# chenbinghui1/DSL

Measured on AMD Instinct MI355X. Metric: imgs/sec training step, FCOS R50-FPN 1333x800, higher is better.
Workload: dtype bf16; 1 GPU; FCOS R50-caffe-FPN supervised training step (BASELINE.json configs[1]), 2 x (3,800,1344) per GPU, synthetic COCO-shaped boxes, random-init weights; global_batch=2, parallelism=dp1, optimizer=SGD momentum 0.9 wd 1e-4

## Files before the change

dsl_amd/_lib.py:

```python
import ctypes as C
import os

import torch

HERE = os.path.dirname(os.path.abspath(__file__))
LIB_PATH = os.environ.get('DSL_HIP_LIB') or os.path.join(HERE, 'lib', 'libdsl_hip.so')
MAX_SEG = 5

if not os.path.exists(LIB_PATH):
    raise RuntimeError(
        f'{LIB_PATH} not found: the MI355X kernels are not built. Run `python -m dsl_amd.build` '
        '(needs hipcc); dsl_amd has no CPU or PyTorch fallback for its hot path.')
lib = C.CDLL(LIB_PATH)

I5 = C.c_int32 * MAX_SEG
F5 = C.c_float * MAX_SEG

CONV_RELU_OUT, CONV_RELU_IN, CONV_OUT_F32, CONV_MASK_FIRST, CONV_MASK_LAST, CONV_ADD_UPSAMPLE, \
    CONV_SMALL_C = 1, 2, 4, 8, 16, 32, 64
CONV_FP8 = 128
CONV_EPI_STAGED = 1 << 16
(OP_CONV, OP_WGRAD, OP_GN_FWD, OP_GN_BWD, OP_MAXPOOL, OP_SUM2X2, OP_COLSUM, OP_MEMSET, OP_PACK_IMAGE,
 OP_ASSIGN, OP_LOSS, OP_FORK, OP_JOIN, OP_WGRAD_GROUP, OP_RECORD, OP_WAIT) = range(1, 17)
OP_RLA = 17
# ... 8 lines not shown
MAX_MULTI = 16
SLOT_TAIL, SLOT_PREFIX = 13, 14
SLOT_PACKS = 15
SUMSQ_PARTS = 256
ACC_SET, ACC_ADD, ACC_FOLD = 0, 1, 2
SLOT_UPD = 8
SLOT_HEADW = 12
(RLA_AVGPOOL, RLA_AVGPOOL_BWD, RLA_BN_TANH, RLA_BN_TANH_BWD, RLA_BN_FOLD, RLA_BN_POST, RLA_REC_SUM, RLA_TAIL_FWD, RLA_TAIL_BWD) = range(2, 11)
MAX_GROUP = 8


class ConvDesc(C.Structure):
    _fields_ = [('nseg', C.c_int32), ('n', C.c_int32),
                ('gh', I5), ('gw', I5), ('sh', I5), ('sw', I5), ('dh', I5), ('dw', I5), ('ah', I5), ('aw', I5),
                ('cs', C.c_int32), ('cd', C.c_int32), ('cd_pad', C.c_int32),
                ('ldd', C.c_int32), ('lda', C.c_int32), ('ldm', C.c_int32),
                ('kh', C.c_int32), ('kw', C.c_int32), ('stride', C.c_int32), ('pad', C.c_int32),
                ('mode', C.c_int32), ('os', C.c_int32), ('flags', C.c_int32),
                ('src', C.c_void_p), ('wgt', C.c_void_p), ('dst', C.c_void_p),
                ('scale', C.c_void_p), ('bias', C.c_void_p), ('addend', C.c_void_p), ('mask', C.c_void_p),
                ('workspace', C.c_void_p), ('workspace_bytes', C.c_size_t), ('cs_real', C.c_int32), ('lds', C.c_int32),
                ('gn_ws', C.c_void_p), ('gn_x', C.c_void_p), ('gn_gamma', C.c_void_p), ('gn_beta', C.c_void_p),
                ('gn_stats', C.c_void_p)]


class WgradDesc(C.Structure):
    _fields_ = [('nseg', C.c_int32), ('n', C.c_int32),
                ('gh', I5), ('gw', I5), ('sh', I5), ('sw', I5),
                ('cs', C.c_int32), ('cy', C.c_int32), ('cd', C.c_int32),
                ('kh', C.c_int32), ('kw', C.c_int32), ('stride', C.c_int32), ('pad', C.c_int32),
                ('splits', C.c_int32),
                ('dy', C.c_void_p), ('x', C.c_void_p), ('scale', C.c_void_p), ('dw', C.c_void_p),
                ('db', C.c_void_p), ('workspace', C.c_void_p), ('workspace_bytes', C.c_size_t),
                ('ldx', C.c_int32), ('shared', C.c_int32), ('slots', C.c_int32), ('pad_', C.c_int32),
                ('pixtab', C.c_void_p), ('pixtab_bytes', C.c_size_t)]


class GnDesc(C.Structure):
    _fields_ = [('nseg', C.c_int32), ('n', C.c_int32), ('c', C.c_int32), ('groups', C.c_int32),
                ('h', I5), ('w', I5), ('eps', C.c_float),
                ('x', C.c_void_p), ('y', C.c_void_p), ('gamma', C.c_void_p), ('beta', C.c_void_p),
                ('stats', C.c_void_p), ('dy', C.c_void_p), ('dx', C.c_void_p), ('dgamma', C.c_void_p),
                ('dbeta', C.c_void_p), ('dbias', C.c_void_p), ('workspace', C.c_void_p), ('workspace_bytes', C.c_size_t),
                ('conv_stats', C.c_int32), ('pad_', C.c_int32), ('y8', C.c_void_p), ('y8_scale', C.c_void_p), ('y8_amax', C.c_void_p)]


class Fp8PrepItem(C.Structure):
    _fields_ = [('w', C.c_void_p), ('w8', C.c_void_p), ('comb', C.c_void_p), ('amax', C.c_void_p), ('scale', C.c_void_p),
                ('n_amax', C.c_int32), ('cout', C.c_int32)]


class FcosDesc(C.Structure):
    _fields_ = [('nlvl', C.c_int32), ('n', C.c_int32),
                ('h', I5), ('w', I5), ('stride', I5), ('range_lo', F5), ('range_hi', F5),
                ('radius', C.c_float), ('num_classes', C.c_int32),
                ('gt_boxes', C.c_void_p), ('gt_labels', C.c_void_p), ('gt_off', C.c_void_p),
                ('ig_boxes', C.c_void_p), ('ig_off', C.c_void_p),
                ('labels', C.c_void_p), ('bbox_targets', C.c_void_p), ('assign_idx', C.c_void_p),
                ('cls_weight', C.c_void_p), ('pos_weight', C.c_void_p), ('stats', C.c_void_p),
                ('loss_weight', C.c_float),
                ('cls_logits', C.c_void_p), ('regctr', C.c_void_p),
                ('ld_cls', C.c_int32), ('ld_rc', C.c_int32),
                ('scales', C.c_void_p), ('norm', C.c_void_p),
                ('g_cls', C.c_void_p), ('ld_gcls', C.c_int32), ('g_rc', C.c_void_p), ('ld_grc', C.c_int32),
                ('g_scales', C.c_void_p), ('losses', C.c_void_p),
                ('soft_weight', C.c_float), ('grad_scale', C.c_float), ('inv_world', C.c_float),
                ('workspace', C.c_void_p), ('workspace_bytes', C.c_size_t), ('logvec', C.c_void_p),
                ('head_flags', C.c_int32), ('ld_ctr', C.c_int32), ('ctr', C.c_void_p), ('g_ctr', C.c_void_p), ('ld_gctr', C.c_int32),
                ('box_kind', C.c_int32), ('box_eps', C.c_float), ('focal_gamma', C.c_float), ('focal_alpha', C.c_float),
                ('w_cls', C.c_float), ('w_bbox', C.c_float), ('w_ctr', C.c_float)]


HEAD_INSIDE_BOX, HEAD_RAW_TARGETS, HEAD_EXP_DECODE, HEAD_IOU_LOSS = 1, 2, 4, 8
HEAD_LOSS_EXT = 16
BOX_GIOU, BOX_IOU_LOG, BOX_IOU_LINEAR, BOX_DIOU, BOX_CIOU = range(5)
NMS_HARD, NMS_LINEAR, NMS_GAUSSIAN, NMS_NAIVE = range(4)
EVAL_COCO, EVAL_VOC, EVAL_MAX_THRS, EVAL_MAX_RANGES = 0, 1, 16, 4
MAX_AUG = 16


class DetDesc(C.Structure):
    _fields_ = [('nlvl', C.c_int32), ('n', C.c_int32),
                ('h', I5), ('w', I5), ('stride', I5),
                ('num_classes', C.c_int32), ('nms_pre', C.c_int32), ('max_per_img', C.c_int32),
                ('score_thr', C.c_float), ('iou_thr', C.c_float),
                ('cls_logits', C.c_void_p), ('ld_cls', C.c_int32),
                ('regctr', C.c_void_p), ('ld_rc', C.c_int32),
                ('scales', C.c_void_p), ('img_shapes', C.c_void_p), ('scale_factors', C.c_void_p),
                ('dets', C.c_void_p), ('det_labels', C.c_void_p), ('det_count', C.c_void_p),
                ('workspace', C.c_void_p), ('workspace_bytes', C.c_size_t),
                ('head_flags', C.c_int32), ('ld_ctr', C.c_int32), ('ctr', C.c_void_p),
                ('nms_method', C.c_int32), ('soft_sigma', C.c_float), ('soft_min_score', C.c_float)]


class PackItem(C.Structure):
    _fields_ = [('w', C.c_void_p), ('scale', C.c_void_p), ('out', C.c_void_p),
                ('cout', C.c_int32), ('cout_pad', C.c_int32), ('taps', C.c_int32), ('cin', C.c_int32),
                ('block_start', C.c_int32), ('tiles_ci', C.c_int32), ('tiles_co', C.c_int32), ('tapmap', C.c_int32)]


class BneckDesc(C.Structure):
    _fields_ = [('x', C.c_void_p), ('w1', C.c_void_p), ('w2', C.c_void_p), ('w3', C.c_void_p), ('idt', C.c_void_p),
                ('s1', C.c_void_p), ('b1', C.c_void_p), ('s2', C.c_void_p), ('b2', C.c_void_p), ('s3', C.c_void_p), ('b3', C.c_void_p),
                ('a1', C.c_void_p), ('a2', C.c_void_p), ('out', C.c_void_p),
                ('n', C.c_int32), ('hin', C.c_int32), ('win', C.c_int32), ('h', C.c_int32), ('w', C.c_int32),
                ('planes', C.c_int32), ('cin', C.c_int32), ('ldx', C.c_int32), ('stride', C.c_int32), ('ldi', C.c_int32), ('ldo', C.c_int32)]


class RlaDesc(C.Structure):
    _fields_ = [('kind', C.c_int32), ('i', C.c_int32 * 8), ('f', C.c_float * 2), ('rows', C.c_int64), ('p', C.c_void_p * 12)]


class BnPostItem(C.Structure):
    _fields_ = [('w', C.c_void_p), ('dw', C.c_void_p), ('dgamma', C.c_void_p), ('dbeta', C.c_void_p), ('gamma', C.c_void_p),
                ('mean', C.c_void_p), ('var', C.c_void_p), ('rows', C.c_int32), ('k', C.c_int32), ('row_start', C.c_int32),
                ('pad_', C.c_int32)]


class RecSumItem(C.Structure):
    _fields_ = [('rec', C.c_void_p), ('out_a', C.c_void_p), ('out_b', C.c_void_p), ('nrec', C.c_int32), ('pad_', C.c_int32)]


class ImagePrepItem(C.Structure):
    _fields_ = [('src', C.c_void_p), ('src_h', C.c_int32), ('src_w', C.c_int32), ('new_h', C.c_int32), ('new_w', C.c_int32),
                ('flip', C.c_int32), ('ps_mode', C.c_int32), ('ps_crop', C.c_int32), ('to_rgb', C.c_int32),
                ('mean', C.c_float * 3), ('inv_std', C.c_float * 3)]


class AugItem(C.Structure):
    _fields_ = [('h', C.c_int32), ('w', C.c_int32), ('kind', C.c_int32), ('order', C.c_int32), ('m', C.c_float * 6),
                ('roi', C.c_int32 * 4), ('cval', C.c_int32), ('f', C.c_float * 3), ('rect', (C.c_int32 * 4) * 3), ('seed', C.c_uint32)]


(AUG_COPY, AUG_AFFINE, AUG_BRIGHTNESS, AUG_CONTRAST, AUG_SATURATION, AUG_HUE, AUG_GRAY, AUG_BLUR_H, AUG_BLUR_V, AUG_ERASE,
 AUG_AUTOCONTRAST, AUG_EQUALIZE, AUG_SOLARIZE, AUG_POSTERIZE, AUG_SHARPNESS) = range(15)


class Op(C.Structure):
    _fields_ = [('kind', C.c_int32), ('i', C.c_int32 * 7), ('desc', C.c_void_p),
                ('p', C.c_void_p * 4), ('l', C.c_int64 * 2)]


lib.dsl_last_error.restype = C.c_char_p
lib.dsl_wgrad_workspace_bytes.restype = C.c_size_t
if hasattr(lib, 'dsl_wgrad_pixtab_bytes'):
    lib.dsl_wgrad_pixtab_bytes.restype = C.c_size_t
if hasattr(lib, 'dsl_wgrad_group_workspace_bytes'):
    lib.dsl_wgrad_group_workspace_bytes.restype = C.c_size_t
lib.dsl_conv2d_workspace_bytes.restype = C.c_size_t
if hasattr(lib, 'dsl_image_aug_scratch_bytes'):
    lib.dsl_image_aug_scratch_bytes.restype = C.c_size_t
if hasattr(lib, 'dsl_rla_tail_bwd_workspace_bytes'):
    lib.dsl_rla_tail_bwd_workspace_bytes.restype = C.c_size_t
for _n in ('dsl_wgrad_multi_table_bytes', 'dsl_wgrad_multi_workspace_bytes'):
    if hasattr(lib, _n):
        getattr(lib, _n).restype = C.c_size_t
if hasattr(lib, 'dsl_bn_tanh_bwd_workspace_bytes'):
    lib.dsl_bn_tanh_bwd_workspace_bytes.restype = C.c_size_t
if hasattr(lib, 'dsl_fcos_workspace_bytes'):
    lib.dsl_fcos_workspace_bytes.restype = C.c_size_t
if hasattr(lib, 'dsl_groupnorm_workspace_bytes'):
    lib.dsl_groupnorm_workspace_bytes.restype = C.c_size_t
if hasattr(lib, 'dsl_detect_workspace_bytes'):
    lib.dsl_detect_workspace_bytes.restype = C.c_size_t
if hasattr(lib, 'dsl_detect_aug_workspace_bytes'):
    lib.dsl_detect_aug_workspace_bytes.restype = C.c_size_t
if hasattr(lib, 'dsl_eval_match_workspace_bytes'):
    lib.dsl_eval_match_workspace_bytes.restype = C.c_size_t
_vp, _i, _l, _f = C.c_void_p, C.c_int, C.c_long, C.c_float
_SIGS = {
    'dsl_conv2d': [_vp, _vp], 'dsl_conv2d_workspace_bytes': [_vp], 'dsl_conv2d_gn_fusable': [_vp], 'dsl_conv2d_wgrad': [_vp, _vp], 'dsl_wgrad_splits': [_vp],
    'dsl_wgrad_workspace_bytes': [_vp], 'dsl_wgrad_pixtab_bytes': [_vp], 'dsl_wgrad_pixtab_fill': [_vp, _vp, C.c_size_t, _vp], 'dsl_wgrad_group_workspace_bytes': [_vp, _i], 'dsl_conv2d_wgrad_group': [_vp, _i, _vp],
    'dsl_wgrad_multi_config': [_vp], 'dsl_wgrad_multi_table_bytes': [], 'dsl_wgrad_multi_workspace_bytes': [_vp, _vp, _i],
    'dsl_wgrad_multi_build': [_vp, _vp, _i, _vp, C.c_size_t, _vp, C.c_size_t], 'dsl_conv2d_wgrad_multi': [_vp, _vp, _vp], 'dsl_wgrad_multi_info': [_vp, _vp, _vp, _vp, _vp, _vp],
    'dsl_wgrad_plan_probe': [_vp, _vp, _vp, _i, _i, _i, _vp, _vp],
    'dsl_image_prep': [_vp, _i, _vp, _i, _i, _vp],
    'dsl_pack_image': [_vp, _vp, _i, _i, _i, _vp], 'dsl_stem_pool': [_vp, _vp, _vp, _vp, _vp, _i, _i, _i, _i, _vp], 'dsl_stem_pool_half': [_vp, _vp, _vp, _vp, _vp, _i, _i, _i, _i, _i, _vp], 'dsl_maxpool3x3s2': [_vp, _vp, _i, _i, _i, _i, _vp],
    'dsl_maxpool3x3s2_ld': [_vp, _vp, _i, _i, _i, _i, _i, _vp],
    'dsl_avgpool2x2': [_vp, _i, _vp, _i, _i, _i, _i, _i, _vp],
    'dsl_avgpool2x2_bwd': [_vp, _i, _vp, _i, _i, _i, _i, _i, _vp],
    'dsl_bn_tanh_fwd': [_vp, _i, _vp, _vp, _vp, _i, _l, _i, _vp],
    'dsl_rla_tail_bwd': [_vp, _i, _vp, _i, _vp, _i, _vp, _vp, _vp, _vp, _f, _vp, _i, _vp, _vp, _vp, _i, _i, _i, _vp], 'dsl_rla_tail_bwd_workspace_bytes': [_i, _i, _i],
    'dsl_rla_tail_fwd': [_vp, _i, _vp, _i, _vp, _i, _vp, _vp, _vp, _i, _vp, _vp, _vp, _i, _i, _i, _i, _vp], 'dsl_bn_tanh_bwd_workspace_bytes': [_l, _i],
    'dsl_bn_tanh_bwd': [_vp, _i, _vp, _i, _vp, _i, _vp, _vp, _vp, _f, _vp, _i, _vp, _vp, _vp, _l, _i, _vp],
    'dsl_image_prep_u8': [_vp, _i, _vp, _i, _i, _vp], 'dsl_image_aug': [_vp, _i, _vp, _vp, _i, _i, _vp, _i, _vp], 'dsl_image_aug_scratch_bytes': [_i],
    'dsl_image_normalize': [_vp, _vp, _i, _vp, _i, _i, _vp],
    'dsl_quant_fp8': [_vp, _vp, _l, _i, _i, _f, _vp], 'dsl_absmax': [_vp, _l, _i, _i, _vp, _i, _vp],
    'dsl_quant_fp8_dyn': [_vp, _vp, _l, _i, _i, _vp, _i, _vp], 'dsl_fp8_comb': [_vp, _vp, _i, _vp, _i, _vp], 'dsl_fp8_prep': [_vp, _i, _i, _i, _f, _vp],
    'dsl_quant_fp8_delayed': [_vp, _vp, _l, _i, _i, _vp, _vp, _i, _vp], 'dsl_quant_fp8_weights': [_vp, _vp, _vp, _vp, _i, _i, _i, _f, _vp],
    'dsl_bn_fold': [_vp, _vp, _vp, _vp, _f, _vp, _vp, _i, _vp], 'dsl_bn_wgrad_post': [_vp, _i, _i, _f, _vp], 'dsl_rla_op': [_vp, _vp],
    'dsl_rec_sum_multi': [_vp, _i, _i, _vp],
    'dsl_groupnorm_relu_fwd': [_vp, _vp], 'dsl_groupnorm_relu_bwd': [_vp, _vp], 'dsl_groupnorm_workspace_bytes': [_vp],
    'dsl_sum2x2': [_vp, _vp, _i, _i, _i, _i, _i, _i, _vp], 'dsl_colsum': [_vp, _vp, _l, _i, _i, _vp],
    'dsl_fcos_points': [_vp, _vp, _vp], 'dsl_fcos_workspace_bytes': [_vp], 'dsl_fcos_assign': [_vp, _vp], 'dsl_fcos_loss': [_vp, _vp],
    'dsl_sumsq': [_vp, _l, _vp, _vp], 'dsl_sumsq_det': [_vp, _l, _vp, _vp, _vp],
    'dsl_sgd_step': [_vp, _vp, _vp, _vp, _vp, _l, _f, _f, _f, _f, _f, _vp, _f, _i, _vp],
    'dsl_grad_accumulate': [_vp, _vp, _l, _i, _vp],
    'dsl_ema_lerp': [_vp, _vp, _l, _f, _vp], 'dsl_ema_lerp_bf16': [_vp, _vp, _vp, _l, _f, _vp], 'dsl_cast_bf16': [_vp, _vp, _l, _vp],
    'dsl_pack_dgrad': [_vp, _vp, _vp, _i, _i, _i, _i, _vp], 'dsl_pack_dgrad_batched': [_vp, _i, _i, _vp],
    'dsl_detect_workspace_bytes': [_vp], 'dsl_fcos_detect': [_vp, _vp],
    'dsl_detect_aug_workspace_bytes': [_vp, _i], 'dsl_fcos_detect_collect': [_vp, _vp, _i, _i, _i, _vp, C.c_size_t, _vp],
    'dsl_fcos_detect_finish': [_vp, _i, _i, _vp, C.c_size_t, _vp],
    'dsl_pseudo_label_fuse': [_vp, _vp, _vp, _i, _i, _i, _f, _f, _f, _vp, _vp, _vp, _vp, _vp],
    'dsl_eval_match_workspace_bytes': [_i, _i],
    'dsl_eval_match': [_i, _i, _i, _i, _i, _i, _vp, _vp, _vp, _vp, _vp, _vp, _vp, _vp, _i, _vp, _i, _vp, _vp, _vp, _vp, C.c_size_t, _vp],
    'dsl_eval_accumulate': [_i, _i, _i, _i, _i, _i, _vp, _vp, _vp, _vp, _vp, _vp, _vp, _vp],
    'dsl_comm_unique_id': [_vp],
    'dsl_comm_init_rank': [_vp, _i, _vp, _i],
    'dsl_comm_size': [_vp],
    'dsl_comm_destroy': [_vp],
    'dsl_allreduce_bucket': [_vp, _vp, C.c_size_t, _vp],
    'dsl_allreduce_buckets': [_vp, _vp, _vp, _i, _vp],
    'dsl_allreduce_bucket_bf16': [_vp, _vp, C.c_size_t, _vp],
    'dsl_cast_f32': [_vp, _vp, _l, _vp], 'dsl_sumsq_partial': [_vp, _l, _vp, _vp], 'dsl_sumsq_fold': [_vp, _i, _vp, _vp],
    'dsl_pseudo_label_fuse_history': [_vp, _vp, _vp, _i, _i, _vp, _vp, _vp, _vp, _i, _i, _f, _f, _f, _vp, _vp, _vp, _vp, _i, _vp],
    'dsl_bottleneck_fwd': [_vp, _vp], 'dsl_bottleneck_fwd_supported': [_vp],
    'dsl_set_option': [C.c_char_p, _i], 'dsl_get_option': [C.c_char_p, _vp],
    'dsl_run_ops': [_vp, _i, _vp], 'dsl_stream_wait_slot': [_i, _vp], 'dsl_stream_record_slot': [_i, _vp], 'dsl_side_stream': [_i, _vp], 'dsl_streams_init': [_vp, _vp], 'dsl_comm_stream_queue': [], 'dsl_comm_proxy': [_vp, C.c_longlong, _i, _i, _vp], 'dsl_prof_enable': [_i], 'dsl_prof_reset': [], 'dsl_prof_read': [_vp, _vp, _vp], 'dsl_prof_read2': [_vp, _vp, _vp, _vp], 'dsl_probe_tr16': [_vp, _vp, _vp, _vp], 'dsl_probe_xcc': [_vp, _vp, _i, _vp], 'dsl_probe_cu_mask': [_vp, _i, _vp, _i],
}
MISSING = []
for _name, _args in _SIGS.items():
    try:
        getattr(lib, _name).argtypes = _args
    except AttributeError:
        MISSING.append(_name)


if 'dsl_set_option' not in MISSING:
    from . import tuning as _tuning
    _tuning.push_lib_options(lib)


def check(rc, what=''):
    if rc != 0:
        raise RuntimeError(f'libdsl_hip {what} failed ({rc}): {lib.dsl_last_error().decode()}')


def seg5(vals):
    a = I5()
    for i, v in enumerate(vals):
        a[i] = int(v)
    return a


def stream_ptr():
    import torch
    return C.c_void_p(torch.cuda.current_stream().cuda_stream)


def ptr(t):
    if t is None:
        return C.c_void_p(0)
    if isinstance(t, int):
        return C.c_void_p(t)
    return C.c_void_p(t.data_ptr())
```

dsl_amd/csrc/api.hip:

```cpp
#include <stdarg.h>
#include <stdlib.h>

#include <stdio.h>
#include <string.h>
#include <stdlib.h>

#include "common.hpp"

static thread_local char g_err[512] = "";

void dsl_set_error(const char* fmt, ...) {
  va_list ap;
  va_start(ap, fmt);
  vsnprintf(g_err, sizeof(g_err), fmt, ap);
  va_end(ap);
}

extern "C" const char* dsl_last_error(void) { return g_err; }
extern "C" int dsl_version(void) { return 100; }

namespace {
struct Option { const char* name; int value; };
Option g_options[] = {
    {"wgrad_slots", 128},
    {"stream_probe", 1},
    {"debug_sync", 0},
    {"skip_kinds", 0},
    {"rla_tail_form", 0},
    {"comm_queue", 1},
};
}
int dsl_option(const char* name) {
  for (const Option& o : g_options)
    if (!strcmp(o.name, name)) return o.value;
  return 0;
}
extern "C" int dsl_set_option(const char* name, int value) {
  DSL_CHECK(name != nullptr, "dsl_set_option: null name");
  for (Option& o : g_options)
    if (!strcmp(o.name, name)) { o.value = value; return 0; }
  dsl_set_error("dsl_set_option: unknown option '%s'", name);
  return -1;
}
extern "C" int dsl_get_option(const char* name, int* value) {
  DSL_CHECK(name != nullptr && value != nullptr, "dsl_get_option: null argument");
  for (const Option& o : g_options)
    if (!strcmp(o.name, name)) { *value = o.value; return 0; }
  dsl_set_error("dsl_get_option: unknown option '%s'", name);
  return -1;
}

namespace {
constexpr int kEvRing = 256, kSide = 3, kStreams = 6;
hipStream_t g_side[16][kStreams] = {};
hipEvent_t g_ev[16][kEvRing] = {};
int g_evpos[16] = {};
bool g_init[16] = {};
int g_probe_result[16] = {};
int g_comm_queue[16] = {};
hipEvent_t g_named[16][16] = {};
bool g_named_set[16][16] = {};

__global__ void spin_kernel(long long ticks) {
  const long long t0 = (long long)wall_clock64();
  while ((long long)wall_clock64() - t0 < ticks) __builtin_amdgcn_s_sleep(8);
}
bool streams_concurrent(hipStream_t a, hipStream_t b, hipEvent_t ea, hipEvent_t eb) {
  hipLaunchKernelGGL(spin_kernel, dim3(1), dim3(64), 0, a, 30000LL);
  hipEventRecord(ea, a);
  hipLaunchKernelGGL(spin_kernel, dim3(1), dim3(64), 0, b, 0LL);
  hipEventRecord(eb, b);
  hipEventSynchronize(eb);
  const bool a_running = hipEventQuery(ea) == hipErrorNotReady;
  hipEventSynchronize(ea);
  (void)hipGetLastError();
  return a_running;
}
void side_init(int dev, hipStream_t caller) {
  if (g_init[dev]) return;
  for (int i = 0; i < kEvRing; ++i) hipEventCreateWithFlags(&g_ev[dev][i], hipEventDisableTiming);
  for (int i = 0; i < 16; ++i) hipEventCreateWithFlags(&g_named[dev][i], hipEventDisableTiming);
  constexpr int kCand = 12, kNeed = 3;
  hipStream_t cand[kCand] = {};
  bool used[kCand] = {};
  for (int i = 0; i < kCand; ++i) {
    hipStreamCreateWithFlags(&cand[i], hipStreamNonBlocking);
    hipEventRecord(g_ev[dev][i], cand[i]);
  }
  hipStream_t chosen[kNeed] = {};
  int n = 0;
  if (dsl_option("stream_probe") != 0) {
    hipEvent_t ea = g_ev[dev][kEvRing - 1], eb = g_ev[dev][kEvRing - 2];
    for (int i = 0; i < kCand && n < kNeed; ++i) {
      bool ok = streams_concurrent(caller, cand[i], ea, eb);
      for (int j = 0; j < n && ok; ++j) ok = streams_concurrent(chosen[j], cand[i], ea, eb);
      if (ok) { chosen[n++] = cand[i]; used[i] = true; }
    }
    g_probe_result[dev] = n;
    if (n < kNeed)
      fprintf(stderr, "[libdsl_hip] stream probe: only %d of %d side streams found a hardware queue of their own (device %d); "
                      "dsl_streams_init reports the count\n", n, kNeed, dev);
  } else {
    g_probe_result[dev] = -1;
  }
  auto take = [&]() -> hipStream_t {
    for (int i = 0; i < kCand; ++i)
      if (!used[i]) { used[i] = true; return cand[i]; }
    return cand[0];
  };
  while (n < kNeed) chosen[n++] = take();
  g_side[dev][0] = chosen[0];
  g_side[dev][1] = chosen[1];
  g_side[dev][2] = chosen[1];
  g_side[dev][3] = chosen[2];
  hipStream_t comm = nullptr;
  g_comm_queue[dev] = 0;
  const int want = dsl_option("comm_queue");
  if (g_probe_result[dev] == kNeed && want >= 1 && want <= 4) {
    hipEvent_t ea = g_ev[dev][kEvRing - 1], eb = g_ev[dev][kEvRing - 2];
    hipStream_t owner = want == 4 ? caller : chosen[want - 1];
    for (int i = 0; i < kCand && !comm; ++i)
      if (!used[i] && !streams_concurrent(owner, cand[i], ea, eb)) { comm = cand[i]; used[i] = true; g_comm_queue[dev] = want; }
  }
  g_side[dev][4] = comm ? comm : take();
  g_side[dev][5] = take();
  for (int i = 0; i < kCand; ++i)
    if (!used[i]) hipStreamDestroy(cand[i]);
  g_init[dev] = true;
}
hipEvent_t next_event(int dev) {
  g_evpos[dev] = (g_evpos[dev] + 1) % kEvRing;
  return g_ev[dev][g_evpos[dev]];
}
}

void dsl_prof_phase(int cls, int end, long long flops_bits, long long bytes_bits, hipStream_t st);

extern "C" int dsl_run_ops(const dsl_op* ops, int n_ops, void* stream) {
  DSL_CHECK(ops || n_ops == 0, "dsl_run_ops: null op list");
  hipStream_t main_st = (hipStream_t)stream;
  int dev = 0;
  hipGetDevice(&dev);
  DSL_CHECK(dev >= 0 && dev < 16, "dsl_run_ops: device index %d out of range", dev);
  auto pick = [&](int id) -> hipStream_t { return id <= 0 ? main_st : g_side[dev][(id - 1) % kSide]; };
  for (int k = 0; k < n_ops; ++k) {
    const dsl_op& o = ops[k];
    int rc = 0;
    hipStream_t st = main_st;
    const bool dbg_pre = dsl_option("debug_sync") == 1;
    if (dbg_pre) {
      fprintf(stderr, "[dsl_run_ops] start op %d/%d kind %d stream %d desc %p p0 %p p1 %p\n", k, n_ops, o.kind, o.i[6], o.desc, o.p[0], o.p[1]);
      if (o.kind == DSL_OP_CONV && o.desc) {
        const dsl_conv_desc* d = (const dsl_conv_desc*)o.desc;
        fprintf(stderr, "    conv src %p wgt %p dst %p addend %p mask %p n %d nseg %d g %dx%d s %dx%d cs %d cd %d lds %d ldd %d lda %d k %d stride %d mode %d flags %d ws %p\n",
                d->src, d->wgt, d->dst, d->addend, d->mask, d->n, d->nseg, d->gh[0], d->gw[0], d->sh[0], d->sw[0], d->cs, d->cd, d->lds, d->ldd, d->lda, d->kh, d->stride, d->mode, d->flags, d->workspace);
      }
      fflush(stderr);
    }
    if (o.kind == DSL_OP_PROF) {
      dsl_prof_phase(o.i[0], o.i[1], o.l[0], o.l[1], pick(o.i[6]));
      continue;
    }
    static const unsigned skip_kinds = (unsigned)dsl_option("skip_kinds");
    if (skip_kinds && o.kind < 30 && (skip_kinds >> o.kind & 1u) && o.kind != DSL_OP_FORK && o.kind != DSL_OP_JOIN &&
        o.kind != DSL_OP_RECORD && o.kind != DSL_OP_WAIT && (!(skip_kinds >> 30 & 1u) || o.i[6] == 1))
      continue;
    if (o.kind == DSL_OP_RECORD || o.kind == DSL_OP_WAIT) {
      side_init(dev, main_st);
      DSL_CHECK(o.i[1] >= 0 && o.i[1] < 16, "dsl_run_ops: event slot %d out of range", o.i[1]);
      if (o.kind == DSL_OP_RECORD) {
        hipEventRecord(g_named[dev][o.i[1]], pick(o.i[0]));
        g_named_set[dev][o.i[1]] = true;
      } else if (g_named_set[dev][o.i[1]]) {
        hipStreamWaitEvent(pick(o.i[0]), g_named[dev][o.i[1]], 0);
      }
      continue;
    }
// ... 281 lines not shown
```

dsl_amd/csrc/wgrad.hip:

```cpp
#include <stdlib.h>
#include <algorithm>

#include <mutex>
#include <type_traits>
#include <vector>

#include "common.hpp"

namespace {
typedef __attribute__((address_space(1))) const void* gptr_t;
typedef __attribute__((address_space(3))) void* lptr_t;
__device__ __attribute__((aligned(16))) unsigned int g_zero_line[4] = {0u, 0u, 0u, 0u};

template <int N>
__device__ __forceinline__ void wait_vmcnt() {
  asm volatile("s_waitcnt vmcnt(%0)" ::"n"(N) : "memory");
}

struct WgTile {
  int bco, bci, wco, wci, ks, nst;
  bool pipe;
};
constexpr WgTile kWgTiles[] = {
    {256, 256, 2, 4, 64, 2, false}, {256, 128, 4, 2, 64, 3, false}, {128, 256, 2, 4, 64, 3, false}, {128, 128, 2, 2, 64, 2, false},
    {256, 256, 2, 4, 32, 4, true},  {256, 128, 4, 2, 32, 5, true},  {128, 256, 2, 4, 32, 5, true},
};
constexpr int kWgDescRing = 16;
constexpr bool wgrad_cfg_ok(int cfg, bool pipe) { return cfg >= 1 && cfg <= (pipe ? 3 : 4); }
constexpr int wgrad_row(int cfg, bool pipe) { return (pipe ? 4 : 0) + cfg - 1; }
constexpr const WgTile& wgrad_tile(int cfg, bool pipe) { return kWgTiles[wgrad_row(cfg, pipe)]; }
constexpr size_t wgrad_lds_bytes(int bco, int bci, int ks, int nst, bool pipe) {
  return (size_t)nst * ks * 2 * (bco + bci) + (pipe ? (size_t)kWgDescRing * ks * 8 : 0);
}
constexpr size_t wgrad_lds_bytes(const WgTile& t) { return wgrad_lds_bytes(t.bco, t.bci, t.ks, t.nst, t.pipe); }

struct WgK {
  int nseg, n;
  int gh[DSL_MAX_SEG], gw[DSL_MAX_SEG], sh[DSL_MAX_SEG], sw[DSL_MAX_SEG];
  int pxstart[DSL_MAX_SEG + 1];
  long long xoff[DSL_MAX_SEG];
  FastDiv dhw[DSL_MAX_SEG], dwd[DSL_MAX_SEG];
  int cs, cy, kh, kw, stride, pad;
  int ktiles, tiles_per_split, ctiles_per_tap;
  int dbg;
  int gx, gy, splits;
  int chunk;
  int group;
  int ldx;
  int cyp;
  const uint16_t* dyv[DSL_MAX_GROUP];
  const uint16_t* xv[DSL_MAX_GROUP];
  long long krow;
  const uint16_t* dy;
  const uint16_t* x;
  float* ws;
  int direct, cd;
  int totpx;
  float* dwv[DSL_MAX_GROUP];
  const float* scalev[DSL_MAX_GROUP];
  int dbmask;
  float* dbws;
  float* dbv[DSL_MAX_GROUP];
  const void* pixtab;
  unsigned pixtab_bytes;
  unsigned ybytes;
};

__device__ __forceinline__ u32x2 lds_tr_read_b64(unsigned addr) {
  u32x2 v;
  asm volatile("ds_read_b64_tr_b16 %0, %1" : "=v"(v) : "v"(addr) : "memory");
  return v;
}
template <int OFF>
__device__ __forceinline__ u32x2 lds_tr_read_b64_o(unsigned addr) {
  static_assert(OFF >= 0 && OFF < 65536, "DS offset field");
  u32x2 v;
  asm volatile("ds_read_b64_tr_b16 %0, %1 offset:%2" : "=v"(v) : "v"(addr), "n"(OFF) : "memory");
  return v;
}
template <int ROWB, int KK>
__device__ __forceinline__ u32x2 lds_tr_read_kh(unsigned base, int kk, int hi) {
  static_assert(KK <= 4, "k-steps per stage");
  switch (kk * 2 + hi) {
    case 0: return lds_tr_read_b64_o<0>(base);
    case 1: return lds_tr_read_b64_o<4 * ROWB>(base);
    case 2: return lds_tr_read_b64_o<16 * ROWB>(base);
    case 3: return lds_tr_read_b64_o<20 * ROWB>(base);
    case 4: return lds_tr_read_b64_o<32 * ROWB>(base);
    case 5: return lds_tr_read_b64_o<36 * ROWB>(base);
    case 6: return lds_tr_read_b64_o<48 * ROWB>(base);
    default: return lds_tr_read_b64_o<52 * ROWB>(base);
  }
}
struct Frag {
  u32x2 lo, hi;
};
__device__ __forceinline__ unsigned lds_read_b32_asm(unsigned addr) {
  unsigned v;
  asm volatile("ds_read_b32 %0, %1" : "=v"(v) : "v"(addr) : "memory");
  return v;
}
__device__ __forceinline__ void wait_lds4(unsigned& a, unsigned& b, unsigned& c, unsigned& d) {
  asm volatile("s_waitcnt lgkmcnt(0)" : "+v"(a), "+v"(b), "+v"(c), "+v"(d) : : "memory");
}
template <int CT, int IT>
__device__ __forceinline__ void wait_frags(Frag (&fa)[CT], Frag (&fb)[IT]) {
  static_assert(IT == 2 && (CT == 2 || CT == 4), "fragment shapes used by the wgrad tiles");
  if constexpr (CT == 4) {
    asm volatile("s_waitcnt lgkmcnt(0)"
                 : "+v"(fa[0].lo), "+v"(fa[0].hi), "+v"(fa[1].lo), "+v"(fa[1].hi), "+v"(fa[2].lo), "+v"(fa[2].hi),
                   "+v"(fa[3].lo), "+v"(fa[3].hi), "+v"(fb[0].lo), "+v"(fb[0].hi), "+v"(fb[1].lo), "+v"(fb[1].hi)
                 :
                 : "memory");
  } else {
    asm volatile("s_waitcnt lgkmcnt(0)"
                 : "+v"(fa[0].lo), "+v"(fa[0].hi), "+v"(fa[1].lo), "+v"(fa[1].hi), "+v"(fb[0].lo), "+v"(fb[0].hi),
                   "+v"(fb[1].lo), "+v"(fb[1].hi)
                 :
                 : "memory");
  }
  __builtin_amdgcn_sched_barrier(0);
}

struct SegSel {
  int px0;
  uint32_t m1lo, m1hi, d1, m2lo, m2hi, d2;
  int sh, sw;
  long long xoff;
};
__device__ __forceinline__ SegSel seg_select(const WgK& p, int gp) {
  SegSel r;
  r.px0 = p.pxstart[0];
  r.m1lo = (uint32_t)p.dhw[0].m; r.m1hi = (uint32_t)(p.dhw[0].m >> 32); r.d1 = p.dhw[0].d;
  r.m2lo = (uint32_t)p.dwd[0].m; r.m2hi = (uint32_t)(p.dwd[0].m >> 32); r.d2 = p.dwd[0].d;
  r.sh = p.sh[0]; r.sw = p.sw[0]; r.xoff = p.xoff[0];
#pragma unroll
  for (int s = 1; s < DSL_MAX_SEG; ++s) {
    const bool in = s < p.nseg && gp >= p.pxstart[s];
    r.px0 = in ? p.pxstart[s] : r.px0;
    r.m1lo = in ? (uint32_t)p.dhw[s].m : r.m1lo; r.m1hi = in ? (uint32_t)(p.dhw[s].m >> 32) : r.m1hi;
    r.d1 = in ? p.dhw[s].d : r.d1;
    r.m2lo = in ? (uint32_t)p.dwd[s].m : r.m2lo; r.m2hi = in ? (uint32_t)(p.dwd[s].m >> 32) : r.m2hi;
    r.d2 = in ? p.dwd[s].d : r.d2;
    r.sh = in ? p.sh[s] : r.sh; r.sw = in ? p.sw[s] : r.sw;
    r.xoff = in ? p.xoff[s] : r.xoff;
  }
  return r;
}

template <int BCO, int BCI, int WCO, int WCI, int KS, int NST>
__device__ __forceinline__ void wgrad_glds_body(const WgK& p, const int bid, unsigned char* smem) {
  constexpr int NW = WCO * WCI;
  constexpr int YB = BCO * 2, XB = BCI * 2;
  constexpr int TILE_Y = KS * YB, TILE_X = KS * XB, STAGE = TILE_Y + TILE_X;
  constexpr int NY = TILE_Y / 1024, NX = TILE_X / 1024;
  constexpr int LY = NY / NW, LX = NX / NW;
  constexpr int LPT = LY + LX;
  constexpr int CT = BCO / WCO / 32, IT = BCI / WCI / 32;
  constexpr int KK = KS / 16;
  static_assert(NY % NW == 0 && NX % NW == 0 && LY >= 1 && LX >= 1, "tile / wave mismatch");
  static_assert(YB >= 256 && XB >= 256, "64-byte-chunk swizzle needs >= 4 chunks per row");
  static_assert(KK == 2 || KK == 4, "stage depth");
  static_assert((NST - 2) * LPT <= 63 && NST >= 2 && NST <= 4, "vmcnt range");
  static_assert(wgrad_lds_bytes(BCO, BCI, KS, NST, false) == (size_t)NST * STAGE, "the host sizes the launch's LDS with wgrad_lds_bytes");

  const int tid = threadIdx.x, lane = tid & 63;
  const int wave = __builtin_amdgcn_readfirstlane(tid >> 6);
  const int wave_co = wave / WCI, wave_ci = wave % WCI;
  const int tiles_per_member = p.gx * p.gy;
  const int tiles_per_split_wg = tiles_per_member * p.group;
  const int xcd = bid & 7, jj = bid >> 3;
  const int witem = xcd * p.chunk + jj;
  if (jj >= p.chunk || witem >= tiles_per_split_wg * p.splits) return;
  const int sp = witem / tiles_per_split_wg;
  const int rem_sp = witem - sp * tiles_per_split_wg;
  const int member = rem_sp / tiles_per_member;
  const int rem_wg = rem_sp - member * tiles_per_member;
  const uint16_t* dy_p = p.dyv[0];
  const uint16_t* x_p = p.xv[0];
  float* db_p = p.dbv[0];
#pragma unroll
  for (int g = 1; g < DSL_MAX_GROUP; ++g) {
    dy_p = member == g ? p.dyv[g] : dy_p;
// ... 157 lines not shown
      for (int i = 0; i < LX; ++i) {
        const gptr_t g = gx[i] >= 0 ? (gptr_t)(x_p + gx[i] + xch[i]) : zero;
        __builtin_amdgcn_global_load_lds(g, (lptr_t)(stage + TILE_Y + (wave + NW * i) * 1024), 16, 0, 0);
      }
    }
    if (kl >= kt0) slot_i = (slot_i + 1 == NST) ? 0 : slot_i + 1;
    if (kc >= kt0) {
#ifdef DSL_ABLATE_BUILD
      if (!(p.dbg & 2))
#endif
      compute(slot_c);
      if (do_db) {
        const unsigned st = lds_base + slot_c * STAGE;
#pragma unroll
        for (int r4 = 0; r4 < DB_ROWS; r4 += 4) {
          unsigned v[4];
#pragma unroll
          for (int j = 0; j < 4; ++j) {
            const int row = db_rg * DB_ROWS + r4 + j;
            v[j] = lds_read_b32_asm(st + row * YB + ((((db_cp * 4) >> 6) ^ (row & 3)) << 6) + ((db_cp * 4) & 63));
          }
          wait_lds4(v[0], v[1], v[2], v[3]);
#pragma unroll
          for (int j = 0; j < 4; ++j) {
            db_lo += __uint_as_float(v[j] << 16);
            db_hi += __uint_as_float(v[j] & 0xffff0000u);
          }
        }
      }
      slot_c = (slot_c + 1 == NST) ? 0 : slot_c + 1;
    }
  }
#ifdef DSL_ABLATE_BUILD
  if (p.dbg & 4) return;
#endif

  if (do_db) {
    __syncthreads();
    float* red = reinterpret_cast<float*>(smem);
    red[(db_rg * DB_PAIRS + db_cp) * 2] = db_lo;
    red[(db_rg * DB_PAIRS + db_cp) * 2 + 1] = db_hi;
    __syncthreads();
    if (tid < BCO) {
      float sacc = 0.f;
#pragma unroll
      for (int r = 0; r < DB_RG; ++r) sacc += red[(r * DB_PAIRS + (tid >> 1)) * 2 + (tid & 1)];
      const int co = co0 + tid;
      if (p.direct) {
        if (co < p.cd) db_p[co] = sacc;
      } else {
        p.dbws[((long long)sp * p.group + member) * p.cyp + co] = sacc;
      }
    }
  }
  const int frow = lane & 31, fhalf = lane >> 5;
  if (p.direct) {
    float* dw_p = p.dwv[0];
    const float* sc_p = p.scalev[0];
#pragma unroll
    for (int g = 1; g < DSL_MAX_GROUP; ++g) {
      dw_p = member == g ? p.dwv[g] : dw_p;
      sc_p = member == g ? p.scalev[g] : sc_p;
    }
#pragma unroll
    for (int ct = 0; ct < CT; ++ct)
#pragma unroll
      for (int it = 0; it < IT; ++it) {
        const long long col = (long long)tap * p.cs + ci0 + wave_ci * (32 * IT) + it * 32 + frow;
#pragma unroll
        for (int j = 0; j < 16; ++j) {
          const int co = co0 + wave_co * (32 * CT) + ct * 32 + (j & 3) + 8 * (j >> 2) + 4 * fhalf;
          if (co < p.cd) dw_p[(long long)co * p.krow + col] = sc_p ? acc[ct][it][j] * sc_p[co] : acc[ct][it][j];
        }
      }
    return;
  }
#pragma unroll
  for (int ct = 0; ct < CT; ++ct)
#pragma unroll
    for (int it = 0; it < IT; ++it) {
      const long long col = (long long)tap * p.cs + ci0 + wave_ci * (32 * IT) + it * 32 + frow;
#pragma unroll
      for (int j = 0; j < 16; ++j) {
        const int co = co0 + wave_co * (32 * CT) + ct * 32 + (j & 3) + 8 * (j >> 2) + 4 * fhalf;
        p.ws[(((long long)sp * p.group + member) * p.cyp + co) * p.krow + col] = acc[ct][it][j];
      }
    }
}

template <int BCO, int BCI, int WCO, int WCI, int KS, int NST>
__global__ __launch_bounds__(64 * WCO * WCI) void wgrad_glds_kernel(const WgK p) {
  extern __shared__ __attribute__((aligned(16))) unsigned char smem[];
  wgrad_glds_body<BCO, BCI, WCO, WCI, KS, NST>(p, (int)blockIdx.x, smem);
}

struct PixDesc {
  int32_t base;
  uint32_t info;
};

__device__ __forceinline__ u32x2 lds_read_b64_asm(unsigned addr) {
  u32x2 v;
  asm volatile("ds_read_b64 %0, %1" : "=v"(v) : "v"(addr) : "memory");
  return v;
}
__device__ __forceinline__ void pin2(u32x2& a) { asm volatile("" : "+v"(a)); }
__device__ __forceinline__ void pin1(unsigned& a) { asm volatile("" : "+v"(a)); }

template <int BCO, int BCI, int WCO, int WCI, int KS, int NST>
__device__ __forceinline__ void wgrad_pipe_body(const WgK& p, const int bid, unsigned char* smem) {
  constexpr int NW = WCO * WCI;
  constexpr int YB = BCO * 2, XB = BCI * 2;
  constexpr int TILE_Y = KS * YB, TILE_X = KS * XB, STAGE = TILE_Y + TILE_X;
  constexpr int NY = TILE_Y / 1024, NX = TILE_X / 1024;
  constexpr int LY = NY / NW, LX = NX / NW;
  constexpr int NDSC = KS * 8 / 256;
  constexpr int P = NDSC + LY + LX;
  constexpr int CT = BCO / WCO / 32, IT = BCI / WCI / 32, NM = CT * IT;
  constexpr int KK = KS / 16;
  constexpr int DR = kWgDescRing;
  constexpr int DESC_BASE = NST * STAGE;
  constexpr int DLEAD = 2 * NST - 2;
  static_assert(NY % NW == 0 && NX % NW == 0 && LY >= 1 && LX >= 1, "tile / wave mismatch");
  static_assert(YB >= 256 && XB >= 256, "64-byte-chunk swizzle needs >= 4 chunks per row");
  static_assert(KK == 2 || KK == 4, "stage depth");
  static_assert(NST >= 3 && DLEAD < DR && NDSC >= 1, "ring depths");
  static_assert((NST - 1) * P + DLEAD * NDSC <= 63, "vmcnt range");
  static_assert(wgrad_lds_bytes(BCO, BCI, KS, NST, true) == (size_t)DESC_BASE + DR * KS * 8, "the host sizes the launch's LDS with wgrad_lds_bytes");

  const int tid = threadIdx.x, lane = tid & 63;
  const int wave = __builtin_amdgcn_readfirstlane(tid >> 6);
  const int wave_co = wave / WCI, wave_ci = wave % WCI;
  const int tiles_per_member = p.gx * p.gy;
  const int tiles_per_split_wg = tiles_per_member * p.group;
  const int xcd = bid & 7, jj = bid >> 3;
  const int witem = xcd * p.chunk + jj;
  if (jj >= p.chunk || witem >= tiles_per_split_wg * p.splits) return;
  const int sp = witem / tiles_per_split_wg;
  const int rem_sp = witem - sp * tiles_per_split_wg;
  const int member = rem_sp / tiles_per_member;
  const int rem_wg = rem_sp - member * tiles_per_member;
  const uint16_t* dy_p = p.dyv[0];
  const uint16_t* x_p = p.xv[0];
  float* db_p = p.dbv[0];
#pragma unroll
  for (int g = 1; g < DSL_MAX_GROUP; ++g) {
    dy_p = member == g ? p.dyv[g] : dy_p;
    x_p = member == g ? p.xv[g] : x_p;
    db_p = member == g ? p.dbv[g] : db_p;
  }
  const int co0 = (rem_wg % p.gx) * BCO;
  const int colt = rem_wg / p.gx;
  const bool do_db = colt == 0 && ((p.dbmask >> member) & 1);
  constexpr int DB_PAIRS = BCO / 2, DB_RG = 64 * NW / DB_PAIRS, DB_ROWS = KS / DB_RG;
  static_assert(DB_ROWS >= 1 && DB_ROWS <= 8 && DB_RG * DB_PAIRS == 64 * NW, "bias-gradient thread mapping");
  const int db_cp = tid % DB_PAIRS, db_rg = tid / DB_PAIRS;
  float db_lo = 0.f, db_hi = 0.f;
  const int ctiles = p.cs / BCI;
  const int tap = colt / ctiles;
  const int ci0 = (colt - tap * ctiles) * BCI;
  const int tr = tap / p.kw, ts = tap - tr * p.kw;
  const int kt0 = sp * p.tiles_per_split;
  const int kt1 = min(kt0 + p.tiles_per_split, p.ktiles);
  if (kt0 >= kt1) return;

  const __amdgpu_buffer_rsrc_t rs_y = __builtin_amdgcn_make_buffer_rsrc((void*)dy_p, 0, (int)p.ybytes, 0x00020000);
  const __amdgpu_buffer_rsrc_t rs_x = __builtin_amdgcn_make_buffer_rsrc((void*)x_p, 0, 0x7fffffff, 0x00020000);
  const __amdgpu_buffer_rsrc_t rs_t = __builtin_amdgcn_make_buffer_rsrc((void*)p.pixtab, 0, (int)p.pixtab_bytes, 0x00020000);

  unsigned yv[LY];
  unsigned xcol[LX], xdaddr[LX];
#pragma unroll
  for (int i = 0; i < LY; ++i) {
    const int off = (wave + NW * i) * 1024 + lane * 16;
    const int row = off / YB, inrow = off % YB;
    const int ch = (((inrow >> 6) ^ (row & 3)) << 5) + ((inrow & 63) >> 1);
    yv[i] = co0 + ch < p.cy ? (unsigned)(((kt0 * KS + row) * p.cy + co0 + ch) * 2) : 0x80000000u;
  }
#pragma unroll
  for (int i = 0; i < LX; ++i) {
    const int off = (wave + NW * i) * 1024 + lane * 16;
    const int row = off / XB, inrow = off % XB;
    const int ch = (((inrow >> 6) ^ (row & 3)) << 5) + ((inrow & 63) >> 1);
    xcol[i] = (unsigned)(ci0 + ch) * 2u;
    xdaddr[i] = (unsigned)(DESC_BASE + row * 8);
  }
  const unsigned y_step = (unsigned)(KS * p.cy * 2);
  const unsigned ldx2 = (unsigned)(p.ldx * 2);
  const unsigned sel = (1u << tr) | (0x100u << ts);

  f32x16 acc[CT][IT];
#pragma unroll
  for (int a = 0; a < CT; ++a)
#pragma unroll
    for (int b = 0; b < IT; ++b)
#pragma unroll
      for (int j = 0; j < 16; ++j) acc[a][b][j] = 0.f;

  const int g16 = lane >> 4, l16 = lane & 15;
  const int iblk = (g16 & 1) * 16, kblk = (g16 >> 1) * 8;
  const int krow_l = kblk + (l16 >> 2);
  const int ccol_l = iblk + 4 * (l16 & 3);
  const unsigned lds_base = (unsigned)(size_t)smem;
  unsigned a_off[CT], b_off[IT];
#pragma unroll
  for (int ct = 0; ct < CT; ++ct) {
    const int col = wave_co * (32 * CT) + ct * 32 + ccol_l;
    a_off[ct] = krow_l * YB + ((((col * 2) >> 6) ^ (krow_l & 3)) << 6) + ((col * 2) & 63);
  }
#pragma unroll
  for (int it = 0; it < IT; ++it) {
    const int col = wave_ci * (32 * IT) + it * 32 + ccol_l;
    b_off[it] = TILE_Y + krow_l * XB + ((((col * 2) >> 6) ^ (krow_l & 3)) << 6) + ((col * 2) & 63);
  }
  Frag fa[2][CT], fb[2][IT];
  constexpr int NR = 2 * (CT + IT);
  unsigned ra[CT], rb[IT];
  auto set_read_stage = [&](unsigned stage_addr) {
#pragma unroll
    for (int ct = 0; ct < CT; ++ct) ra[ct] = stage_addr + a_off[ct];
#pragma unroll
    for (int it = 0; it < IT; ++it) rb[it] = stage_addr + b_off[it];
  };
  auto rd = [&](int kk, int f, int j) {
#ifdef DSL_ABLATE_BUILD
    if (p.dbg & 8) return;
#endif
    if (j < 2 * CT) {
      const int ct = j >> 1;
      if (j & 1) fa[f][ct].hi = lds_tr_read_kh<YB, KK>(ra[ct], kk, 1); else fa[f][ct].lo = lds_tr_read_kh<YB, KK>(ra[ct], kk, 0);
    } else {
      const int it = (j - 2 * CT) >> 1;
      if (j & 1) fb[f][it].hi = lds_tr_read_kh<XB, KK>(rb[it], kk, 1); else fb[f][it].lo = lds_tr_read_kh<XB, KK>(rb[it], kk, 0);
    }
  };
  auto issue = [&](int kk, int f) {
#pragma unroll
    for (int j = 0; j < NR; ++j) rd(kk, f, j);
  };
  auto wait_lds = [&](int f) {
    asm volatile("s_waitcnt lgkmcnt(0)" ::: "memory");
#pragma unroll
    for (int ct = 0; ct < CT; ++ct) { pin2(fa[f][ct].lo); pin2(fa[f][ct].hi); }
#pragma unroll
    for (int it = 0; it < IT; ++it) { pin2(fb[f][it].lo); pin2(fb[f][it].hi); }
  };

  int t_data = kt0, t_desc = kt0, ld_slot = 0;
  unsigned xv[LX];
  u32x2 dreg[LX];
  auto piece = [&](int k) {
#ifdef DSL_ABLATE_BUILD
    if ((p.dbg & 1) && t_data >= kt0 + NST) return;
#endif
    if (k < NDSC) {
      const unsigned v = (unsigned)(t_desc * (KS * 8) + k * 256 + lane * 4);
      __builtin_amdgcn_raw_ptr_buffer_load_lds(rs_t, (lptr_t)(smem + DESC_BASE + (t_desc & (DR - 1)) * (KS * 8) + k * 256), 4, v, 0, 0, 0);
    } else if (k < NDSC + LY) {
      const int i = k - NDSC;
      const unsigned v = t_data < kt1 ? yv[i] : 0x80000000u;
      __builtin_amdgcn_raw_ptr_buffer_load_lds(rs_y, (lptr_t)(smem + ld_slot * STAGE + (wave + NW * i) * 1024), 16, v, 0, 0, 0);
    } else {
      const int i = k - NDSC - LY;
      const unsigned v = t_data < kt1 ? xv[i] : 0x80000000u;
      __builtin_amdgcn_raw_ptr_buffer_load_lds(rs_x, (lptr_t)(smem + ld_slot * STAGE + TILE_Y + (wave + NW * i) * 1024), 16, v, 0, 0, 0);
    }
  };
  auto desc_read = [&]() {
#pragma unroll
    for (int i = 0; i < LX; ++i) dreg[i] = lds_read_b64_asm(lds_base + xdaddr[i] + (unsigned)((t_data & (DR - 1)) * (KS * 8)));
  };
  auto desc_use = [&]() {
#pragma unroll
    for (int i = 0; i < LX; ++i) {
      pin2(dreg[i]);
      const unsigned info = dreg[i][1];
      const unsigned px = (unsigned)((int)dreg[i][0] + tr * (int)(info >> 16) + ts);
      xv[i] = (info & sel) == sel ? px * ldx2 + xcol[i] : 0x80000000u;
    }
  };
  auto advance = [&]() {
    ++t_data;
    ++t_desc;
    ld_slot = (ld_slot + 1 == NST) ? 0 : ld_slot + 1;
#pragma unroll
    for (int i = 0; i < LY; ++i) yv[i] += y_step;
  };
  auto block = [&](int f, int lo, int hi, int rd_kk) {
    bf16x8 a[CT], b[IT];
#pragma unroll
    for (int ct = 0; ct < CT; ++ct) {
      union { struct { u32x2 l, h; } s; bf16x8 v; } u;
      u.s.l = fa[f][ct].lo;
      u.s.h = fa[f][ct].hi;
      a[ct] = u.v;
    }
#pragma unroll
    for (int it = 0; it < IT; ++it) {
      union { struct { u32x2 l, h; } s; bf16x8 v; } u;
      u.s.l = fb[f][it].lo;
      u.s.h = fb[f][it].hi;
      b[it] = u.v;
    }
    __builtin_amdgcn_sched_barrier(0);
    int k = lo;
#pragma unroll
    for (int m = 0; m < NM; ++m) {
#ifdef DSL_ABLATE_BUILD
      if (!(p.dbg & 2))
#endif
      acc[m / IT][m % IT] = __builtin_amdgcn_mfma_f32_32x32x16_bf16(a[m / IT], b[m % IT], acc[m / IT][m % IT], 0, 0, 0);
      __builtin_amdgcn_sched_barrier(0);
#pragma unroll
      for (int j = 0; j < NR; ++j)
        if (j >= m * NR / NM && j < (m + 1) * NR / NM) rd(rd_kk, f ^ 1, j);
      if ((m & 1) == 1 && k < hi) {
        piece(k);
        ++k;
      }
      __builtin_amdgcn_sched_barrier(0);
    }
#pragma unroll
    for (int j = 0; j < P; ++j)
      if (k + j < hi) piece(k + j);
    __builtin_amdgcn_sched_barrier(0);
  };
  constexpr int PA = (KK - 1) * P / KK;

#pragma unroll
  for (int j = 0; j < NST - 1; ++j) {
#pragma unroll
    for (int k = 0; k < NDSC; ++k) piece(k);
    ++t_desc;
  }
  wait_vmcnt<0>();
  __builtin_amdgcn_s_barrier();
#pragma unroll
  for (int j = 0; j < NST - 1; ++j) {
    desc_read();
    asm volatile("s_waitcnt lgkmcnt(0)" ::: "memory");
    desc_use();
#pragma unroll
    for (int k = 0; k < P; ++k) piece(k);
    advance();
  }
  wait_vmcnt<(NST - 2) * P>();
  __builtin_amdgcn_s_barrier();
  desc_read();
  set_read_stage(lds_base);
  issue(0, 0);

  unsigned dbr[8];
  int slot_c = 0;
  for (int s = kt0; s < kt1; ++s) {
    const unsigned st = lds_base + slot_c * STAGE;
    const int nslot = (slot_c + 1 == NST) ? 0 : slot_c + 1;
#pragma unroll
    for (int kk = 0; kk < KK; ++kk) {
      const int f = kk & 1;
      wait_lds(f);
      if (kk == 0) desc_use();
      if (kk == 1 && do_db) {
#pragma unroll
        for (int j = 0; j < DB_ROWS; ++j) {
          pin1(dbr[j]);
          db_lo += __uint_as_float(dbr[j] << 16);
          db_hi += __uint_as_float(dbr[j] & 0xffff0000u);
        }
      }
      if (kk == 0 && do_db) {
#pragma unroll
        for (int j = 0; j < DB_ROWS; ++j) {
          const int row = db_rg * DB_ROWS + j;
          dbr[j] = lds_read_b32_asm(st + row * YB + ((((db_cp * 4) >> 6) ^ (row & 3)) << 6) + ((db_cp * 4) & 63));
        }
      }
      if (kk == KK - 1) {
        wait_vmcnt<(NST - 3) * P + PA>();
#ifdef DSL_ABLATE_BUILD
        if (!(p.dbg & 16))
#endif
        __builtin_amdgcn_s_barrier();
      }
      __builtin_amdgcn_sched_barrier(0);
      if (kk < KK - 1) {
        block(f, kk * P / KK, (kk + 1) * P / KK, kk + 1);
      } else {
        set_read_stage(lds_base + nslot * STAGE);
        block(f, kk * P / KK, P, 0);
      }
      if (kk == KK - 1) {
        advance();
        desc_read();
      }
    }
    slot_c = nslot;
  }
  wait_vmcnt<0>();
  asm volatile("s_waitcnt lgkmcnt(0)" ::: "memory");
#ifdef DSL_ABLATE_BUILD
  if (p.dbg & 4) return;
#endif

  if (do_db) {
    __syncthreads();
    float* red = reinterpret_cast<float*>(smem);
    red[(db_rg * DB_PAIRS + db_cp) * 2] = db_lo;
    red[(db_rg * DB_PAIRS + db_cp) * 2 + 1] = db_hi;
    __syncthreads();
    if (tid < BCO) {
      float sacc = 0.f;
#pragma unroll
      for (int r = 0; r < DB_RG; ++r) sacc += red[(r * DB_PAIRS + (tid >> 1)) * 2 + (tid & 1)];
      const int co = co0 + tid;
      if (p.direct) {
        if (co < p.cd) db_p[co] = sacc;
      } else {
        p.dbws[((long long)sp * p.group + member) * p.cyp + co] = sacc;
      }
    }
  }
  const int frow = lane & 31, fhalf = lane >> 5;
  if (p.direct) {
    float* dw_p = p.dwv[0];
    const float* sc_p = p.scalev[0];
#pragma unroll
    for (int g = 1; g < DSL_MAX_GROUP; ++g) {
      dw_p = member == g ? p.dwv[g] : dw_p;
      sc_p = member == g ? p.scalev[g] : sc_p;
    }
#pragma unroll
    for (int ct = 0; ct < CT; ++ct)
#pragma unroll
      for (int it = 0; it < IT; ++it) {
        const long long col = (long long)tap * p.cs + ci0 + wave_ci * (32 * IT) + it * 32 + frow;
#pragma unroll
        for (int j = 0; j < 16; ++j) {
          const int co = co0 + wave_co * (32 * CT) + ct * 32 + (j & 3) + 8 * (j >> 2) + 4 * fhalf;
          if (co < p.cd) dw_p[(long long)co * p.krow + col] = sc_p ? acc[ct][it][j] * sc_p[co] : acc[ct][it][j];
        }
      }
    return;
  }
#pragma unroll
  for (int ct = 0; ct < CT; ++ct)
#pragma unroll
    for (int it = 0; it < IT; ++it) {
      const long long col = (long long)tap * p.cs + ci0 + wave_ci * (32 * IT) + it * 32 + frow;
#pragma unroll
      for (int j = 0; j < 16; ++j) {
        const int co = co0 + wave_co * (32 * CT) + ct * 32 + (j & 3) + 8 * (j >> 2) + 4 * fhalf;
        p.ws[(((long long)sp * p.group + member) * p.cyp + co) * p.krow + col] = acc[ct][it][j];
      }
    }
}

template <int BCO, int BCI, int WCO, int WCI, int KS, int NST>
__global__ __launch_bounds__(64 * WCO * WCI) void wgrad_pipe_kernel(const WgK p) {
  extern __shared__ __attribute__((aligned(16))) unsigned char smem[];
  const int total = p.chunk * 8;
  for (int vb = (int)blockIdx.x; vb < total; vb += (int)gridDim.x) {
    wgrad_pipe_body<BCO, BCI, WCO, WCI, KS, NST>(p, vb, smem);
    __syncthreads();
  }
}

constexpr int kMaxMulti = DSL_MAX_MULTI;
struct WgMultiHdr {
  int nsub;
  int wg_end[kMaxMulti];
};
#define WG_MULTI_SUB(h, vb)                                    \
  int sub = 0, start = 0;                                      \
  _Pragma("unroll") for (int s = 1; s < kMaxMulti; ++s) {      \
    const bool in = s < (h).nsub && (vb) >= (h).wg_end[s - 1]; \
    sub = in ? s : sub;                                        \
    start = in ? (h).wg_end[s - 1] : start;                    \
  }

template <int BCO, int BCI, int WCO, int WCI, int KS, int NST>
__global__ __launch_bounds__(64 * WCO * WCI) void wgrad_glds_multi_kernel(const WgMultiHdr h, const WgK* __restrict__ tab) {
  extern __shared__ __attribute__((aligned(16))) unsigned char smem[];
  WG_MULTI_SUB(h, (int)blockIdx.x)
  const WgK p = tab[sub];
  wgrad_glds_body<BCO, BCI, WCO, WCI, KS, NST>(p, (int)blockIdx.x - start, smem);
}

template <int BCO, int BCI, int WCO, int WCI, int KS, int NST>
__global__ __launch_bounds__(64 * WCO * WCI) void wgrad_pipe_multi_kernel(const WgMultiHdr h, const WgK* __restrict__ tab, int total) {
  extern __shared__ __attribute__((aligned(16))) unsigned char smem[];
  for (int vb = (int)blockIdx.x; vb < total; vb += (int)gridDim.x) {
    WG_MULTI_SUB(h, vb)
    const WgK p = tab[sub];
    wgrad_pipe_body<BCO, BCI, WCO, WCI, KS, NST>(p, vb - start, smem);
    __syncthreads();
  }
}

template <int BCO, int BCI, int WCO, int WCI, int KS, int NST>
__global__ __launch_bounds__(64 * WCO * WCI) void wgrad_pipe_multi_sched_kernel(const WgMultiHdr h, const WgK* __restrict__ tab,
                                                                               const short* __restrict__ sched, int rounds) {
  extern __shared__ __attribute__((aligned(16))) unsigned char smem[];
  for (int r = 0; r < rounds; ++r) {
    const int vb = __builtin_amdgcn_readfirstlane((int)sched[r * (int)gridDim.x + (int)blockIdx.x]);
    if (vb < 0) break;
    WG_MULTI_SUB(h, vb)
    const WgK p = tab[sub];
    wgrad_pipe_body<BCO, BCI, WCO, WCI, KS, NST>(p, vb - start, smem);
    __syncthreads();
  }
}

#undef WG_MULTI_SUB

struct RedEnt {
  const float* ws;
  float* dw;
  const float* scale;
  float* db;
  const float* dbws;
  long long dbstride;
  long long krow, sstride;
  int splits, cd, blk_start, nblk;
};
__global__ void wgrad_reduce_multi_kernel(const RedEnt* __restrict__ tab, int n) {
  int e = 0;
  for (int i = 1; i < n; ++i) e = (int)blockIdx.x >= tab[i].blk_start ? i : e;
  const RedEnt r = tab[e];
  const int lb = (int)blockIdx.x - r.blk_start;
  if (lb == 0 && r.db)
    for (int c = threadIdx.x; c < r.cd; c += blockDim.x) {
      float sacc = 0.f;
      for (int sp = 0; sp < r.splits; ++sp) sacc += r.dbws[sp * r.dbstride + c];
      r.db[c] = sacc;
    }
  const long long total4 = (long long)r.cd * r.krow / 4;
  for (long long i = (long long)lb * blockDim.x + threadIdx.x; i < total4; i += (long long)r.nblk * blockDim.x) {
    const long long el = i * 4;
    const int co = (int)(el / r.krow);
    f32x4 s = {0.f, 0.f, 0.f, 0.f};
    const float* base = r.ws + el;
    int sp = 0;
    for (; sp + 4 <= r.splits; sp += 4) {
      const f32x4 a = *reinterpret_cast<const f32x4*>(base + sp * r.sstride);
      const f32x4 b = *reinterpret_cast<const f32x4*>(base + (sp + 1) * r.sstride);
      const f32x4 c = *reinterpret_cast<const f32x4*>(base + (sp + 2) * r.sstride);
      const f32x4 d = *reinterpret_cast<const f32x4*>(base + (sp + 3) * r.sstride);
      s += (a + b) + (c + d);
    }
    for (; sp < r.splits; ++sp) s += *reinterpret_cast<const f32x4*>(base + sp * r.sstride);
    if (r.scale) s *= r.scale[co];
    *reinterpret_cast<f32x4*>(r.dw + el) = s;
  }
}

struct RedK {
  float* dw[DSL_MAX_GROUP];
  const float* scale[DSL_MAX_GROUP];
  float* db[DSL_MAX_GROUP];
  const float* dbws;
};

__global__ void wgrad_reduce_kernel(const float* __restrict__ ws, const RedK r, int splits, int group, int cy, int cd,
                                    long long krow) {
  const int member = blockIdx.y;
  float* __restrict__ dw = r.dw[0];
  const float* __restrict__ scale = r.scale[0];
#pragma unroll
  for (int g = 1; g < DSL_MAX_GROUP; ++g) {
    dw = member == g ? r.dw[g] : dw;
    scale = member == g ? r.scale[g] : scale;
  }
  if (blockIdx.x == 0) {
    float* db = r.db[0];
#pragma unroll
    for (int g = 1; g < DSL_MAX_GROUP; ++g) db = member == g ? r.db[g] : db;
    if (db)
      for (int c = threadIdx.x; c < cd; c += blockDim.x) {
        float sacc = 0.f;
        if (r.dbws)
          for (int sp = 0; sp < splits; ++sp) sacc += r.dbws[((long long)sp * group + member) * cy + c];
        db[c] = sacc;
      }
  }
  const long long total4 = (long long)cd * krow / 4;
  const long long sstride = (long long)group * cy * krow;
  for (long long i = (long long)blockIdx.x * blockDim.x + threadIdx.x; i < total4;
       i += (long long)gridDim.x * blockDim.x) {
    const long long e = i * 4;
    const int co = (int)(e / krow);
    const long long k = e - (long long)co * krow;
    f32x4 s = {0.f, 0.f, 0.f, 0.f};
    const float* base = ws + ((long long)member * cy + co) * krow + k;
    int sp = 0;
    for (; sp + 4 <= splits; sp += 4) {
      const f32x4 a = *reinterpret_cast<const f32x4*>(base + sp * sstride);
      const f32x4 b = *reinterpret_cast<const f32x4*>(base + (sp + 1) * sstride);
      const f32x4 c = *reinterpret_cast<const f32x4*>(base + (sp + 2) * sstride);
      const f32x4 d = *reinterpret_cast<const f32x4*>(base + (sp + 3) * sstride);
      s += (a + b) + (c + d);
    }
    for (; sp < splits; ++sp) s += *reinterpret_cast<const f32x4*>(base + sp * sstride);
    if (scale) s *= scale[co];
    *reinterpret_cast<f32x4*>(dw + e) = s;
  }
}

}

namespace {
struct PixGeo {
  int nseg, n, stride, pad, kh, kw;
  int gh[DSL_MAX_SEG], gw[DSL_MAX_SEG], sh[DSL_MAX_SEG], sw[DSL_MAX_SEG];
  int pxstart[DSL_MAX_SEG + 1];
  long long xoff[DSL_MAX_SEG];
};
__global__ void pixtab_fill_kernel(PixDesc* __restrict__ out, PixGeo g) {
  const int i = blockIdx.x * blockDim.x + threadIdx.x;
  if (i >= g.pxstart[g.nseg]) return;
  int s = 0;
#pragma unroll
  for (int t = 1; t < DSL_MAX_SEG; ++t)
    if (t < g.nseg && i >= g.pxstart[t]) s = t;
  const int gh = g.gh[s], gw = g.gw[s], sh = g.sh[s], sw = g.sw[s];
  int r = i - g.pxstart[s];
  const int img = r / (gh * gw);
  r -= img * gh * gw;
  const int y = r / gw, x = r - y * gw;
  const int y0 = y * g.stride - g.pad, x0 = x * g.stride - g.pad;
  unsigned ym = 0, xm = 0;
  for (int a = 0; a < g.kh; ++a) if ((unsigned)(y0 + a) < (unsigned)sh) ym |= 1u << a;
  for (int c = 0; c < g.kw; ++c) if ((unsigned)(x0 + c) < (unsigned)sw) xm |= 1u << c;
  PixDesc e;
  e.base = (int32_t)(g.xoff[s] + ((long long)img * sh + y0) * sw + x0);
  e.info = ((unsigned)sw << 16) | (xm << 8) | ym;
  out[i] = e;
}

int wgrad_slots() {
  const int v = dsl_option("wgrad_slots");
  return v > 0 ? v : 128;
}
long long wgrad_px(const dsl_wgrad_desc* d) {
  long long px = 0;
  for (int s = 0; s < d->nseg; ++s) px += (long long)d->n * d->gh[s] * d->gw[s];
  return px;
}
bool wgrad_v3_ok(const dsl_wgrad_desc* d, int cfg) {
  if (!wgrad_cfg_ok(cfg, true) || d->kh > 8 || d->kw > 8) return false;
  long long xo = 0;
  for (int s = 0; s < d->nseg; ++s) {
    xo += (long long)d->n * d->sh[s] * d->sw[s];
    if (d->sw[s] >= 65536) return false;
  }
  const long long px = wgrad_px(d), ldx = d->ldx > 0 ? d->ldx : d->cs;
  return px * d->cy * 2 < 0x7fff0000LL && xo * ldx * 2 < 0x7fff0000LL && px < (1 << 20);
}
int wgrad_v3_fill(const dsl_wgrad_desc* d, WgK& k, long long px) {
  const size_t need = (size_t)px * sizeof(PixDesc);
  DSL_CHECK(d->pixtab != nullptr && d->pixtab_bytes >= need,
            "dsl_conv2d_wgrad: this geometry runs the pipelined kernel and needs dsl_wgrad_desc.pixtab (%zu bytes given, %zu needed: "
            "dsl_wgrad_pixtab_bytes / dsl_wgrad_pixtab_fill)", d->pixtab ? d->pixtab_bytes : (size_t)0, need);
  k.pixtab = d->pixtab;
  k.pixtab_bytes = (unsigned)need;
  k.ybytes = (unsigned)(px * d->cy * 2);
  return 0;
}

template <class F>
bool wgrad_dispatch(int cfg, bool pipe, F&& f) {
  if (!wgrad_cfg_ok(cfg, pipe)) return false;
  switch (wgrad_row(cfg, pipe)) {
    case 0: f(std::integral_constant<int, 0>{}); break;
    case 1: f(std::integral_constant<int, 1>{}); break;
    case 2: f(std::integral_constant<int, 2>{}); break;
    case 3: f(std::integral_constant<int, 3>{}); break;
    case 4: f(std::integral_constant<int, 4>{}); break;
    case 5: f(std::integral_constant<int, 5>{}); break;
    default: f(std::integral_constant<int, 6>{}); break;
  }
  return true;
}
static_assert(sizeof(kWgTiles) / sizeof(kWgTiles[0]) == 7, "wgrad_dispatch lists every row");
#define WG_TILE_ARGS(T) T.bco, T.bci, T.wco, T.wci, T.ks, T.nst
template <auto KERNEL, class... Args>
void wgrad_run(const WgTile& T, dim3 grid, hipStream_t st, const Args&... args) {
  const size_t lds = wgrad_lds_bytes(T);
  static bool attr_set = false;
  if (!attr_set) {
    hipFuncSetAttribute((const void*)KERNEL, hipFuncAttributeMaxDynamicSharedMemorySize, (int)lds);
    attr_set = true;
  }
  hipLaunchKernelGGL(KERNEL, grid, dim3(64 * T.wco * T.wci), lds, st, args...);
}
}

static int wgrad_pick(const dsl_wgrad_desc* d) {
  const int force = d->splits < 0 ? -d->splits : 0;
  if (force) return force - 1;
  if (d->cy % 128) return d->cs % 256 == 0 ? 3 : 4;
  if (d->cy % 256 == 0 && d->cs % 256 == 0) return 1;
  if (d->cy % 256 == 0) return 2;
  if (d->cs % 256 == 0) return 3;
  return 4;
}
static int wgrad_geometry(const dsl_wgrad_desc* d, int* ktiles, int* tiles, int* bco) {
  const int cfg = wgrad_pick(d);
  *ktiles = *tiles = *bco = 0;
  if (!wgrad_cfg_ok(cfg, false)) return cfg;
  const WgTile& t = wgrad_tile(cfg, false);
  *ktiles = (int)((wgrad_px(d) + t.ks - 1) / t.ks);
  *bco = t.bco;
  *tiles = ((d->cy + t.bco - 1) / t.bco) * (d->kh * d->kw * d->cs / t.bci);
  return cfg;
}

static int wgrad_splits_for(const dsl_wgrad_desc* d, int count) {
  int ktiles, tiles, bco;
  const int cfg = wgrad_geometry(d, &ktiles, &tiles, &bco);
  if (tiles == 0) return 0;
  tiles *= count;
  const int max_by_k = ktiles / 4 > 0 ? ktiles / 4 : 1;
  const int per_cu = cfg == 4 ? 2 : 1;
  const int slots = d->slots > 0 ? d->slots : wgrad_slots();
  int splits = slots * per_cu / tiles;
  if (splits > max_by_k) splits = max_by_k;
  if (splits < 1) splits = 1;
  if (splits > 256) splits = 256;
  {
    const int ks = wgrad_tile(cfg, wgrad_v3_ok(d, cfg)).ks;
    const int stages = (int)((wgrad_px(d) + ks - 1) / ks);
    const int tps = (stages + splits - 1) / splits;
    splits = (stages + tps - 1) / tps;
  }
  return splits;
}

extern "C" int dsl_wgrad_splits(const dsl_wgrad_desc* d) { return wgrad_splits_for(d, 1); }

extern "C" size_t dsl_wgrad_pixtab_bytes(const dsl_wgrad_desc* d) {
  if (d == nullptr || d->nseg < 1 || d->nseg > DSL_MAX_SEG) return 0;
  if (!wgrad_v3_ok(d, wgrad_pick(d))) return 0;
  return (size_t)wgrad_px(d) * sizeof(PixDesc);
}
extern "C" int dsl_wgrad_pixtab_fill(const dsl_wgrad_desc* d, void* table, size_t bytes, void* stream) {
  DSL_CHECK(d != nullptr && d->nseg >= 1 && d->nseg <= DSL_MAX_SEG, "dsl_wgrad_pixtab_fill: bad descriptor");
  const size_t need = dsl_wgrad_pixtab_bytes(d);
  if (need == 0) return 0;
  DSL_CHECK(table != nullptr && bytes >= need, "dsl_wgrad_pixtab_fill: table too small (%zu < %zu)", bytes, need);
  PixGeo g;
  memset(&g, 0, sizeof(g));
  g.nseg = d->nseg; g.n = d->n; g.stride = d->stride; g.pad = d->pad; g.kh = d->kh; g.kw = d->kw;
  int px = 0;
  long long xo = 0;
  for (int s = 0; s < d->nseg; ++s) {
    g.gh[s] = d->gh[s]; g.gw[s] = d->gw[s]; g.sh[s] = d->sh[s]; g.sw[s] = d->sw[s];
    g.pxstart[s] = px;
    g.xoff[s] = xo;
    px += d->n * d->gh[s] * d->gw[s];
    xo += (long long)d->n * d->sh[s] * d->sw[s];
  }
  for (int s = d->nseg; s <= DSL_MAX_SEG; ++s) g.pxstart[s] = px;
  hipLaunchKernelGGL(pixtab_fill_kernel, dim3((px + 255) / 256), dim3(256), 0, (hipStream_t)stream, (PixDesc*)table, g);
  DSL_CHECK(hipGetLastError() == hipSuccess, "dsl_wgrad_pixtab_fill: launch failed");
  return 0;
}

static size_t wgrad_cy_pad(const dsl_wgrad_desc* d) {
  int ktiles, tiles, bco;
  wgrad_geometry(d, &ktiles, &tiles, &bco);
  return bco ? (size_t)(d->cy + bco - 1) / bco * bco : 0;
}

extern "C" size_t dsl_wgrad_workspace_bytes(const dsl_wgrad_desc* d) {
  const int splits = d->splits > 0 ? d->splits : dsl_wgrad_splits(d);
  return (size_t)splits * wgrad_cy_pad(d) * ((size_t)d->kh * d->kw * d->cs + 1) * sizeof(float);
}

extern "C" size_t dsl_wgrad_group_workspace_bytes(const dsl_wgrad_desc* descs, int count) {
  if (!descs || count < 1) return 0;
  if (count == 1) return dsl_wgrad_workspace_bytes(descs);
  return (size_t)wgrad_splits_for(descs, count) * count * wgrad_cy_pad(descs) * ((size_t)descs->kh * descs->kw * descs->cs + 1) * sizeof(float);
}

static bool wgrad_same_geometry(const dsl_wgrad_desc* a, const dsl_wgrad_desc* b) {
  if (a->ldx != b->ldx || a->shared != b->shared) return false;
  if (a->nseg != b->nseg || a->n != b->n || a->cs != b->cs || a->cy != b->cy || a->cd != b->cd || a->kh != b->kh ||
      a->kw != b->kw || a->stride != b->stride || a->pad != b->pad)
    return false;
  for (int s = 0; s < a->nseg; ++s)
    if (a->gh[s] != b->gh[s] || a->gw[s] != b->gw[s] || a->sh[s] != b->sh[s] || a->sw[s] != b->sw[s]) return false;
  return true;
}

static int wgrad_fill_k(const dsl_wgrad_desc* descs, int count, int splits, int cfg, bool v3, WgK& k, long long* px_out, long long* xo_out) {
  const dsl_wgrad_desc* d = descs;
  memset(&k, 0, sizeof(k));
  k.nseg = d->nseg; k.n = d->n;
  int px = 0;
  long long xo = 0;
  for (int s = 0; s < d->nseg; ++s) {
    k.gh[s] = d->gh[s]; k.gw[s] = d->gw[s]; k.sh[s] = d->sh[s]; k.sw[s] = d->sw[s];
    k.pxstart[s] = px;
    k.xoff[s] = xo;
    k.dhw[s] = make_fastdiv((uint32_t)(d->gh[s] * d->gw[s]));
    k.dwd[s] = make_fastdiv((uint32_t)d->gw[s]);
    px += d->n * d->gh[s] * d->gw[s];
    xo += (long long)d->n * d->sh[s] * d->sw[s];
  }
  DSL_CHECK(px < (1 << 20), "dsl_conv2d_wgrad: %d pixels exceed the 2^20 fast-division range", px);
  const int ldx = d->ldx > 0 ? d->ldx : d->cs;
  DSL_CHECK(ldx >= d->cs && ldx % 8 == 0, "dsl_conv2d_wgrad: ldx=%d must be >= cs=%d and a multiple of 8", ldx, d->cs);
  DSL_CHECK(xo * ldx < (1LL << 31), "dsl_conv2d_wgrad: X has more than 2^31 elements");
  k.pxstart[d->nseg] = px;
  k.totpx = px;
  k.cs = d->cs; k.cy = d->cy; k.kh = d->kh; k.kw = d->kw; k.stride = d->stride; k.pad = d->pad;
  k.ctiles_per_tap = d->cs / 128;
  k.krow = (long long)d->kh * d->kw * d->cs;
  k.group = count;
  k.ldx = ldx;
  k.cyp = (int)wgrad_cy_pad(d);
  k.cd = d->cd;
  for (int g = 0; g < DSL_MAX_GROUP; ++g) {
    const dsl_wgrad_desc& m = descs[g < count ? g : 0];
    k.dyv[g] = (const uint16_t*)m.dy;
    k.xv[g] = (const uint16_t*)m.x;
    k.dwv[g] = m.dw;
    k.scalev[g] = m.scale;
    k.dbv[g] = m.db;
    if (g < count && m.db) k.dbmask |= 1 << g;
  }
  k.dy = k.dyv[0]; k.x = k.xv[0];
  const WgTile& t = wgrad_tile(cfg, v3);
  DSL_CHECK(k.cyp % t.bco == 0 && d->cs % t.bci == 0, "dsl_conv2d_wgrad: tile config %d does not divide cy=%d / cs=%d", cfg, d->cy, d->cs);
  k.gx = k.cyp / t.bco;
  k.gy = d->kh * d->kw * d->cs / t.bci;
  k.splits = splits;
  k.chunk = (k.gx * k.gy * count * splits + 7) / 8;
  k.ktiles = (px + t.ks - 1) / t.ks;
  k.tiles_per_split = (k.ktiles + splits - 1) / splits;
  if (v3)
    if (int rc = wgrad_v3_fill(d, k, px)) return rc;
  *px_out = px;
  *xo_out = xo;
  return 0;
}

static int wgrad_launch(const dsl_wgrad_desc* descs, int count, void* stream) {
  const dsl_wgrad_desc* d = descs;
  DSL_CHECK(d != nullptr && count >= 1 && count <= DSL_MAX_GROUP, "dsl_conv2d_wgrad: bad group (count=%d)", count);
  DSL_CHECK(d->nseg >= 1 && d->nseg <= DSL_MAX_SEG, "dsl_conv2d_wgrad: nseg=%d", d->nseg);
  DSL_CHECK(d->cs % 128 == 0, "dsl_conv2d_wgrad: Cin=%d must be a multiple of 128", d->cs);
  DSL_CHECK(d->cy % 64 == 0 && d->cd <= d->cy, "dsl_conv2d_wgrad: bad cy=%d cd=%d", d->cy, d->cd);
  for (int g = 0; g < count; ++g) {
    DSL_CHECK(descs[g].dy && descs[g].x && descs[g].dw, "dsl_conv2d_wgrad: null pointer (member %d)", g);
    DSL_CHECK(wgrad_same_geometry(d, &descs[g]), "dsl_conv2d_wgrad_group: member %d has a different geometry", g);
  }
  DSL_CHECK(d->workspace, "dsl_conv2d_wgrad: null workspace");
  const int cfg = wgrad_pick(d);
  DSL_CHECK(wgrad_cfg_ok(cfg, false), "dsl_conv2d_wgrad: there is no tile configuration %d (1 .. 4; the register-staged configuration 0 is gone)", cfg);
  const int splits = count == 1 ? (d->splits > 0 ? d->splits : dsl_wgrad_splits(d)) : wgrad_splits_for(d, count);
  const int cyp = (int)wgrad_cy_pad(d);
  const size_t need = (size_t)splits * count * cyp * ((size_t)d->kh * d->kw * d->cs + 1) * sizeof(float);
  DSL_CHECK(d->workspace_bytes >= need, "dsl_conv2d_wgrad: workspace too small (%zu < %zu)", d->workspace_bytes, need);
  const bool v3 = wgrad_v3_ok(d, cfg);
  WgK k;
  long long px, xo;
  if (int rc = wgrad_fill_k(descs, count, splits, cfg, v3, k, &px, &xo)) return rc;
  k.ws = (float*)d->workspace;
  k.dbws = k.ws + (size_t)splits * count * cyp * k.krow;
#ifdef DSL_ABLATE_BUILD
  { const char* e = getenv("DSL_ABLATE"); k.dbg = e ? atoi(e) : 0; }
#endif
  hipStream_t st = (hipStream_t)stream;
  const int prof = dsl_prof_active()
                       ? dsl_prof_begin(3, 2.0 * count * px * (double)d->cd * d->kh * d->kw * d->cs, st,
                                        count * ((double)px * d->cd * 2.0 + (double)xo * d->cs * 2.0 + (double)d->cd * d->kh * d->kw * d->cs * 4.0))
                       : -1;
  dim3 grid(k.chunk * 8);
  if (v3) {
    const int cap = ((d->slots > 0 ? d->slots : wgrad_slots()) + 7) / 8 * 8;
    if ((int)grid.x > cap) grid.x = cap;
  }
  wgrad_dispatch(cfg, v3, [&](auto row) {
    constexpr WgTile T = kWgTiles[decltype(row)::value];
    if constexpr (T.pipe) wgrad_run<wgrad_pipe_kernel<WG_TILE_ARGS(T)>>(T, grid, st, k);
    else wgrad_run<wgrad_glds_kernel<WG_TILE_ARGS(T)>>(T, grid, st, k);
  });
  dsl_prof_end(prof, st);
  DSL_LAUNCH_CHECK(v3 ? "wgrad_pipe_kernel" : "wgrad_glds_kernel");
  const long long total4 = (long long)d->cd * k.krow / 4;
  int rb = (int)((total4 + 255) / 256);
  if (rb > 4096 / count) rb = 4096 / count;
  RedK r;
  for (int g = 0; g < DSL_MAX_GROUP; ++g) {
    r.dw[g] = descs[g < count ? g : 0].dw;
    r.scale[g] = descs[g < count ? g : 0].scale;
    r.db[g] = g < count ? descs[g].db : nullptr;
  }
  r.dbws = k.dbws;
  if (d->shared && count > 1) {
    for (int g = 1; g < count; ++g)
      DSL_CHECK(descs[g].dw == d->dw && descs[g].scale == d->scale && !descs[g].db, "dsl_conv2d_wgrad_group: shared members must share dw / scale and have no db");
    hipLaunchKernelGGL(wgrad_reduce_kernel, dim3(rb * count, 1), dim3(256), 0, st, (const float*)d->workspace, r, splits * count, 1,
                       cyp, d->cd, k.krow);
    DSL_LAUNCH_CHECK("wgrad_reduce_kernel");
    return 0;
  }
  hipLaunchKernelGGL(wgrad_reduce_kernel, dim3(rb, count), dim3(256), 0, st, (const float*)d->workspace, r, splits, count,
                     cyp, d->cd, k.krow);
  DSL_LAUNCH_CHECK("wgrad_reduce_kernel");
  return 0;
}

namespace {
constexpr int kMaxRed = 128, kSchedMax = 8192;
struct WgMultiTable {
  int magic, cfg, nsub, total_blocks;
  WgMultiHdr hdr;
  int n_red, red_blocks, v3;
  double flops, bytes;
  WgK k[kMaxMulti];
  RedEnt red[kMaxRed];
  int sched_grid, sched_rounds;
  int plan_makespan, plan_items;
  short sched[kSchedMax];
};
constexpr int kMultiMagic = 0x574d5431;

struct PlanSub { int stages, tiles, max_sp; long long tile_elems; };
inline int plan_norm_splits(int stages, int sp) {
  if (sp < 1) sp = 1;
  const int tps = (stages + sp - 1) / sp;
  return (stages + tps - 1) / tps;
}
long long plan_simulate(const PlanSub* subs, const int* splits, int nsub, int G, int ovh, short* sched, int sched_cap, int* rounds_out,
                        int* items_out) {
  struct It { int cost, vb; };
  std::vector<It> cls[8];
  int base = 0, items = 0;
  for (int i = 0; i < nsub; ++i) {
    const int witems = subs[i].tiles * splits[i];
    const int chunk = (witems + 7) / 8;
    const int tps = (subs[i].stages + splits[i] - 1) / splits[i];
    for (int bid = 0; bid < chunk * 8; ++bid) {
      const int xcd = bid & 7, jj = bid >> 3, w = xcd * chunk + jj;
      if (jj >= chunk || w >= witems) continue;
      const int sp = w / subs[i].tiles;
      const int k0 = sp * tps, k1 = std::min(k0 + tps, subs[i].stages);
      if (k1 <= k0) continue;
      cls[xcd].push_back({ovh + (k1 - k0), base + bid});
      ++items;
    }
    base += chunk * 8;
  }
  const int per = G / 8;
  long long makespan = 0;
  int rounds = 0;
  std::vector<long long> load(G, 0);
  std::vector<std::vector<int>> mine(G);
  for (int x = 0; x < 8; ++x) {
    std::stable_sort(cls[x].begin(), cls[x].end(), [](const It& a, const It& b) { return a.cost > b.cost; });
    for (const It& it : cls[x]) {
      int best = x;
      for (int j = 1; j < per; ++j)
        if (load[x + 8 * j] < load[best]) best = x + 8 * j;
      load[best] += it.cost;
      mine[best].push_back(it.vb);
    }
  }
  for (int b = 0; b < G; ++b) {
    makespan = std::max(makespan, load[b]);
    rounds = std::max(rounds, (int)mine[b].size());
  }
  if (sched) {
    if ((long long)rounds * G > sched_cap) { rounds = 0; }
    else {
      for (int i = 0; i < rounds * G; ++i) sched[i] = -1;
      for (int b = 0; b < G; ++b)
        for (size_t r = 0; r < mine[b].size(); ++r) sched[r * G + b] = (short)mine[b][r];
    }
  }
  if (rounds_out) *rounds_out = rounds;
  if (items_out) *items_out = items;
  return makespan;
}
inline double plan_stage_us(int cfg) { return cfg == 1 ? 0.62 : 0.43; }
constexpr int kPlanOvh = 8;
struct PlanOut { int splits[kMaxMulti]; int grid, makespan, items; double us; };
void wgrad_plan(const PlanSub* subs, int nsub, int cfg, int cap, PlanOut* out) {
  long long total = 0;
  int smax = 1;
  for (int i = 0; i < nsub; ++i) { total += (long long)subs[i].stages * subs[i].tiles; smax = std::max(smax, subs[i].stages); }
  const long long bal = std::max<long long>(8, (total + cap - 1) / cap);
  std::vector<int> cand;
  cand.push_back(smax);
  for (int i = 0; i < nsub; ++i)
    for (int j = 1; j <= subs[i].max_sp; ++j) {
      const int l = (subs[i].stages + j - 1) / j;
      if (l >= bal / 3 && l <= bal * 4) cand.push_back(l);
    }
  std::sort(cand.begin(), cand.end());
  cand.erase(std::unique(cand.begin(), cand.end()), cand.end());
  double best = 1e30;
  std::vector<std::vector<int>> seen;
  for (int l : cand) {
    std::vector<int> sp(nsub);
    long long items = 0;
    for (int i = 0; i < nsub; ++i) {
      int v = (subs[i].stages + l - 1) / l;
      if (v > subs[i].max_sp) v = subs[i].max_sp;
      sp[i] = plan_norm_splits(subs[i].stages, v);
      items += (long long)sp[i] * subs[i].tiles;
    }
    if (std::find(seen.begin(), seen.end(), sp) != seen.end()) continue;
    seen.push_back(sp);
    int G = (int)std::min<long long>(cap, (items + 7) / 8 * 8);
    if (G < 8) G = 8;
    int n_items = 0;
    long long ms = plan_simulate(subs, sp.data(), nsub, cap, kPlanOvh, nullptr, 0, nullptr, &n_items);
    {
      int g = G;
      for (; g < cap; g += 8)
        if (plan_simulate(subs, sp.data(), nsub, g, kPlanOvh, nullptr, 0, nullptr, nullptr) <= ms) break;
      G = g;
    }
    double red_bytes = 0;
    for (int i = 0; i < nsub; ++i)
      if (sp[i] > 1) red_bytes += (double)(sp[i] + 1) * subs[i].tile_elems * 4.0;
    const double us = ms * plan_stage_us(cfg) + (red_bytes > 0 ? 6.0 + red_bytes / 3.0e6 : 0.0);
    if (us < best) {
      best = us;
      for (int i = 0; i < nsub; ++i) out->splits[i] = sp[i];
      out->grid = G; out->makespan = (int)ms; out->items = n_items; out->us = us;
    }
  }
}
bool wgrad_multi_v3(const dsl_wgrad_desc* descs, const int* counts, int nsub, int cfg) {
  bool v3 = true;
  int off = 0;
  for (int s = 0; s < nsub; ++s) { v3 = v3 && wgrad_v3_ok(&descs[off], cfg); off += counts[s]; }
  return v3;
}
int wgrad_multi_cap(const dsl_wgrad_desc* descs, const int* counts, int nsub) {
  int n = 0, cap = 0;
  for (int s = 0; s < nsub; ++s) n += counts[s];
  for (int i = 0; i < n; ++i) cap = std::max(cap, descs[i].slots);
  if (cap <= 0) cap = wgrad_slots();
  return (std::min(cap, 256) + 7) / 8 * 8;
}

void wgrad_plan_subs(const dsl_wgrad_desc* descs, const int* counts, int nsub, int ks, PlanSub* subs) {
  int off = 0;
  for (int s = 0; s < nsub; ++s) {
    int ktiles, tiles, bco;
    wgrad_geometry(&descs[off], &ktiles, &tiles, &bco);
    const long long px = wgrad_px(&descs[off]);
    subs[s].stages = (int)((px + ks - 1) / ks);
    subs[s].tiles = tiles * counts[s];
    subs[s].max_sp = std::max(1, subs[s].stages / (256 / ks));
    subs[s].tile_elems = (long long)counts[s] * (long long)wgrad_cy_pad(&descs[off]) * ((long long)descs[off].kh * descs[off].kw * descs[off].cs);
    off += counts[s];
  }
}

int wgrad_multi_splits(const dsl_wgrad_desc* descs, const int* counts, int nsub, int* splits) {
  const int cfg = wgrad_pick(descs);
  if (wgrad_multi_v3(descs, counts, nsub, cfg)) {
    PlanSub subs[kMaxMulti];
    wgrad_plan_subs(descs, counts, nsub, wgrad_tile(cfg, true).ks, subs);
    PlanOut po;
    wgrad_plan(subs, nsub, cfg, wgrad_multi_cap(descs, counts, nsub), &po);
    for (int s = 0; s < nsub; ++s) splits[s] = po.splits[s];
    return 0;
  }
  long long total = 0;
  int off = 0;
  for (int s = 0; s < nsub; ++s) {
    int ktiles, tiles, bco;
    wgrad_geometry(&descs[off], &ktiles, &tiles, &bco);
    total += (long long)ktiles * tiles * counts[s];
    off += counts[s];
  }
  const int slots = wgrad_multi_cap(descs, counts, nsub) * (cfg == 4 ? 2 : 1);
  long long lmax = (total + slots - 1) / slots;
  if (lmax < 4) lmax = 4;
  off = 0;
  for (int s = 0; s < nsub; ++s) {
    int ktiles, tiles, bco;
    wgrad_geometry(&descs[off], &ktiles, &tiles, &bco);
    int sp = (int)((ktiles + lmax - 1) / lmax);
    const int max_by_k = ktiles / 4 > 0 ? ktiles / 4 : 1;
    if (sp > max_by_k) sp = max_by_k;
    if (sp < 1) sp = 1;
    splits[s] = sp;
    off += counts[s];
  }
  return 0;
}

int wgrad_multi_check(const dsl_wgrad_desc* descs, const int* counts, int nsub) {
  DSL_CHECK(descs && counts && nsub >= 1 && nsub <= kMaxMulti, "dsl_wgrad_multi: bad sub-launch list (n=%d)", nsub);
  const int cfg = wgrad_pick(descs);
  DSL_CHECK(cfg >= 1 && cfg <= 4, "dsl_wgrad_multi: tile configuration %d has no multi form", cfg);
  int off = 0;
  for (int s = 0; s < nsub; ++s) {
    DSL_CHECK(counts[s] >= 1 && counts[s] <= DSL_MAX_GROUP, "dsl_wgrad_multi: sub-launch %d has %d members", s, counts[s]);
    const dsl_wgrad_desc* d = &descs[off];
    DSL_CHECK(d->nseg >= 1 && d->nseg <= DSL_MAX_SEG && d->cs % 128 == 0 && d->cy % 64 == 0 && d->cd <= d->cy,
              "dsl_wgrad_multi: bad geometry in sub-launch %d", s);
    DSL_CHECK(wgrad_pick(d) == cfg, "dsl_wgrad_multi: sub-launch %d needs tile configuration %d, the launch uses %d", s, wgrad_pick(d), cfg);
    for (int g = 0; g < counts[s]; ++g) {
      DSL_CHECK(d[g].dy && d[g].x && d[g].dw, "dsl_wgrad_multi: null pointer (sub-launch %d member %d)", s, g);
      DSL_CHECK(!d[g].shared, "dsl_wgrad_multi: shared-weight groups use dsl_conv2d_wgrad_group");
      DSL_CHECK(wgrad_same_geometry(d, &d[g]), "dsl_wgrad_multi: sub-launch %d member %d has a different geometry", s, g);
    }
    off += counts[s];
  }
  return 0;
}
}

extern "C" int dsl_wgrad_multi_config(const dsl_wgrad_desc* d) {
  DSL_CHECK(d != nullptr, "dsl_wgrad_multi_config: null descriptor");
  return d->shared ? 0 : wgrad_pick(d);
}

extern "C" size_t dsl_wgrad_multi_table_bytes(void) { return sizeof(WgMultiTable); }

extern "C" size_t dsl_wgrad_multi_workspace_bytes(const dsl_wgrad_desc* descs, const int* counts, int nsub) {
  if (wgrad_multi_check(descs, counts, nsub)) return 0;
  int splits[kMaxMulti];
  wgrad_multi_splits(descs, counts, nsub, splits);
  size_t need = 0;
  int off = 0;
  for (int s = 0; s < nsub; ++s) {
    const dsl_wgrad_desc* d = &descs[off];
    if (splits[s] > 1) need += (size_t)splits[s] * counts[s] * wgrad_cy_pad(d) * ((size_t)d->kh * d->kw * d->cs + 1) * sizeof(float);
    off += counts[s];
  }
  return need ? need : 16;
}

extern "C" int dsl_wgrad_multi_build(const dsl_wgrad_desc* descs, const int* counts, int nsub, void* workspace, size_t ws_bytes,
                                     void* table_host, size_t table_bytes) {
  if (int rc = wgrad_multi_check(descs, counts, nsub)) return rc;
  DSL_CHECK(table_host && table_bytes >= sizeof(WgMultiTable), "dsl_wgrad_multi_build: table buffer too small");
  DSL_CHECK(workspace && ws_bytes >= dsl_wgrad_multi_workspace_bytes(descs, counts, nsub), "dsl_wgrad_multi_build: workspace too small");
  WgMultiTable* t = (WgMultiTable*)table_host;
  memset(t, 0, sizeof(*t));
  t->magic = kMultiMagic;
  t->cfg = wgrad_pick(descs);
  t->nsub = nsub;
  int splits[kMaxMulti], first[kMaxMulti], order[kMaxMulti];
  wgrad_multi_splits(descs, counts, nsub, splits);
  t->v3 = wgrad_multi_v3(descs, counts, nsub, t->cfg) ? 1 : 0;
  long long per_wg[kMaxMulti];
  {
    int off = 0;
    for (int s = 0; s < nsub; ++s) {
      int ktiles, tiles, bco;
      wgrad_geometry(&descs[off], &ktiles, &tiles, &bco);
      per_wg[s] = (ktiles + splits[s] - 1) / splits[s];
      first[s] = off;
      order[s] = s;
      off += counts[s];
    }
  }
  for (int i = 1; i < nsub; ++i)
    for (int j = i; j > 0 && per_wg[order[j]] > per_wg[order[j - 1]]; --j) { const int tmp = order[j]; order[j] = order[j - 1]; order[j - 1] = tmp; }
  unsigned char* ws = (unsigned char*)workspace;
  int blocks = 0, red_blocks = 0;
  for (int i = 0; i < nsub; ++i) {
    const int s = order[i];
    const dsl_wgrad_desc* d = &descs[first[s]];
    WgK& k = t->k[i];
    long long px, xo;
    if (int rc = wgrad_fill_k(d, counts[s], splits[s], t->cfg, t->v3 != 0, k, &px, &xo)) return rc;
    k.direct = splits[s] == 1 ? 1 : 0;
    k.ws = (float*)ws;
    blocks += k.chunk * 8;
    t->hdr.wg_end[i] = blocks;
    t->flops += 2.0 * counts[s] * px * (double)d->cd * d->kh * d->kw * d->cs;
    t->bytes += counts[s] * ((double)px * d->cd * 2.0 + (double)xo * d->cs * 2.0 + (double)d->cd * d->kh * d->kw * d->cs * 4.0);
    const long long sub_elems = (long long)counts[s] * k.cyp * k.krow;
    k.dbws = (float*)ws + (size_t)splits[s] * sub_elems;
    for (int g = 0; g < counts[s]; ++g) {
      if (!k.direct) {
        DSL_CHECK(t->n_red < kMaxRed, "dsl_wgrad_multi_build: more than %d reduce entries", kMaxRed);
        RedEnt& r = t->red[t->n_red++];
        r.ws = (const float*)ws + (long long)g * k.cyp * k.krow;
        r.dw = d[g].dw; r.scale = d[g].scale; r.db = d[g].db;
        r.dbws = k.dbws + (long long)g * k.cyp; r.dbstride = (long long)counts[s] * k.cyp;
        r.krow = k.krow; r.sstride = sub_elems; r.splits = splits[s]; r.cd = d->cd;
        const long long total4 = (long long)d->cd * k.krow / 4;
        int nb = (int)((total4 + 1023) / 1024);
        if (nb > 512) nb = 512;
        if (nb < 1) nb = 1;
        r.blk_start = red_blocks; r.nblk = nb;
        red_blocks += nb;
      }
    }
    if (!k.direct) ws += (size_t)splits[s] * (sub_elems + (long long)counts[s] * k.cyp) * sizeof(float);
  }
  t->hdr.nsub = nsub;
  t->total_blocks = blocks;
  t->red_blocks = red_blocks;
  if (t->v3) {
    PlanSub subs[kMaxMulti], tsubs[kMaxMulti];
    int tsplits[kMaxMulti];
    wgrad_plan_subs(descs, counts, nsub, wgrad_tile(t->cfg, true).ks, subs);
    long long items = 0;
    for (int i = 0; i < nsub; ++i) { tsubs[i] = subs[order[i]]; tsplits[i] = splits[order[i]]; items += (long long)tsplits[i] * tsubs[i].tiles; }
    const int cap_ = wgrad_multi_cap(descs, counts, nsub);
    int G = (int)std::min<long long>(cap_, (items + 7) / 8 * 8);
    if (G < 8) G = 8;
    {
      const long long ms_cap = plan_simulate(tsubs, tsplits, nsub, cap_, kPlanOvh, nullptr, 0, nullptr, nullptr);
      for (; G < cap_; G += 8)
        if (plan_simulate(tsubs, tsplits, nsub, G, kPlanOvh, nullptr, 0, nullptr, nullptr) <= ms_cap) break;
    }
    int rounds = 0, n_items = 0;
    const long long ms = plan_simulate(tsubs, tsplits, nsub, G, kPlanOvh, t->sched, kSchedMax, &rounds, &n_items);
    if (blocks < 32767 && rounds > 0) { t->sched_grid = G; t->sched_rounds = rounds; }
    t->plan_makespan = (int)ms; t->plan_items = n_items;
  }
  return 0;
}

extern "C" int dsl_wgrad_plan_probe(const int* stages, const int* tiles, const long long* tile_elems, int nsub, int cfg, int cap,
                                    int* splits_out, int* info) {
  DSL_CHECK(stages && tiles && nsub >= 1 && nsub <= kMaxMulti && cfg >= 1 && cfg <= 3 && cap >= 8 && cap % 8 == 0, "dsl_wgrad_plan_probe: bad arguments");
  PlanSub subs[kMaxMulti];
  for (int s = 0; s < nsub; ++s) {
    subs[s].stages = stages[s]; subs[s].tiles = tiles[s]; subs[s].max_sp = std::max(1, stages[s] / 8);
    subs[s].tile_elems = tile_elems ? tile_elems[s] : 0;
  }
  PlanOut po;
  wgrad_plan(subs, nsub, cfg, cap, &po);
  for (int s = 0; s < nsub; ++s) splits_out[s] = po.splits[s];
  info[0] = po.grid; info[1] = po.makespan; info[2] = po.items;
  {
    std::vector<short> sched(kSchedMax);
    int rounds = 0, n_items = 0, total_blocks = 0;
    plan_simulate(subs, po.splits, nsub, po.grid, kPlanOvh, sched.data(), kSchedMax, &rounds, &n_items);
    for (int s = 0; s < nsub; ++s) total_blocks += (subs[s].tiles * po.splits[s] + 7) / 8 * 8;
    if (rounds > 0) {
      std::vector<int> hit(total_blocks, 0);
      int seen_items = 0;
      for (int b = 0; b < po.grid; ++b) {
        bool ended = false;
        for (int r = 0; r < rounds; ++r) {
          const int vb = sched[r * po.grid + b];
          if (vb < 0) { ended = true; continue; }
          DSL_CHECK(!ended && vb < total_blocks && (vb & 7) == (b & 7) && hit[vb]++ == 0, "dsl_wgrad_plan_probe: bad schedule entry (workgroup %d round %d block %d)", b, r, vb);
          ++seen_items;
        }
      }
      DSL_CHECK(seen_items == n_items && n_items == po.items, "dsl_wgrad_plan_probe: schedule holds %d of %d items", seen_items, n_items);
    }
  }
  long long total = 0;
  for (int s = 0; s < nsub; ++s) total += (long long)((stages[s] + 1) / 2) * tiles[s];
  long long lmax = std::max<long long>(4, (total + cap - 1) / cap);
  int osp[kMaxMulti], ord[kMaxMulti];
  for (int s = 0; s < nsub; ++s) {
    const int kt = (stages[s] + 1) / 2;
    int sp = (int)((kt + lmax - 1) / lmax);
    sp = std::max(1, std::min(sp, std::max(1, kt / 4)));
    osp[s] = sp; ord[s] = s;
  }
  for (int i = 1; i < nsub; ++i)
    for (int j = i; j > 0 && (stages[ord[j]] + osp[ord[j]] - 1) / osp[ord[j]] > (stages[ord[j - 1]] + osp[ord[j - 1]] - 1) / osp[ord[j - 1]]; --j) std::swap(ord[j], ord[j - 1]);
  std::vector<long long> load(cap, 0);
  int base = 0, oitems = 0;
  for (int i = 0; i < nsub; ++i) {
    const int s = ord[i], witems = tiles[s] * osp[s], chunk = (witems + 7) / 8, tps = (stages[s] + osp[s] - 1) / osp[s];
    for (int bid = 0; bid < chunk * 8; ++bid) {
      const int xcd = bid & 7, jj = bid >> 3, w = xcd * chunk + jj;
      if (jj >= chunk || w >= witems) continue;
      const int sp = w / tiles[s], k0 = sp * tps, k1 = std::min(k0 + tps, stages[s]);
      if (k1 > k0) { load[(base + bid) % cap] += kPlanOvh + k1 - k0; ++oitems; }
    }
    base += chunk * 8;
  }
  info[3] = (int)*std::max_element(load.begin(), load.end());
  info[4] = oitems;
  return 0;
}

extern "C" int dsl_wgrad_multi_info(const void* table_host, double* flops, double* bytes, int* blocks, int* red_blocks, int* nsub) {
  const WgMultiTable* t = (const WgMultiTable*)table_host;
  DSL_CHECK(t && t->magic == kMultiMagic, "dsl_wgrad_multi_info: not a table of dsl_wgrad_multi_build");
  if (flops) *flops = t->flops;
  if (bytes) *bytes = t->bytes;
  if (blocks) *blocks = t->total_blocks;
  if (red_blocks) *red_blocks = t->red_blocks;
  if (nsub) *nsub = t->nsub;
  return 0;
}

extern "C" int dsl_conv2d_wgrad_multi(const void* table_host, const void* table_dev, void* stream) {
  const WgMultiTable* t = (const WgMultiTable*)table_host;
  DSL_CHECK(t && table_dev && t->magic == kMultiMagic, "dsl_conv2d_wgrad_multi: not a table of dsl_wgrad_multi_build");
  const unsigned char* dev = (const unsigned char*)table_dev;
  const WgK* ktab = (const WgK*)(dev + offsetof(WgMultiTable, k));
  const RedEnt* rtab = (const RedEnt*)(dev + offsetof(WgMultiTable, red));
  const short* sched = (const short*)(dev + offsetof(WgMultiTable, sched));
  hipStream_t st = (hipStream_t)stream;
  const int prof = dsl_prof_active() ? dsl_prof_begin(3, t->flops, st, t->bytes) : -1;
  const char* name = "wgrad_glds_multi_kernel";
  const bool known = wgrad_dispatch(t->cfg, t->v3 != 0, [&](auto row) {
    constexpr WgTile T = kWgTiles[decltype(row)::value];
    if constexpr (!T.pipe) {
      wgrad_run<wgrad_glds_multi_kernel<WG_TILE_ARGS(T)>>(T, dim3(t->total_blocks), st, t->hdr, ktab);
    } else if (t->sched_rounds > 0) {
      name = "wgrad_pipe_multi_sched_kernel";
      wgrad_run<wgrad_pipe_multi_sched_kernel<WG_TILE_ARGS(T)>>(T, dim3(t->sched_grid), st, t->hdr, ktab, sched, t->sched_rounds);
    } else {
      name = "wgrad_pipe_multi_kernel";
      const int cap = (wgrad_slots() + 7) / 8 * 8;
      wgrad_run<wgrad_pipe_multi_kernel<WG_TILE_ARGS(T)>>(T, dim3(std::min(t->total_blocks, cap)), st, t->hdr, ktab, t->total_blocks);
    }
  });
  dsl_prof_end(prof, st);
  DSL_CHECK(known, "dsl_conv2d_wgrad_multi: the table names tile configuration %d, which does not exist", t->cfg);
  DSL_LAUNCH_CHECK(name);
  if (t->n_red > 0) {
    hipLaunchKernelGGL(wgrad_reduce_multi_kernel, dim3(t->red_blocks), dim3(256), 0, st, rtab, t->n_red);
    DSL_LAUNCH_CHECK("wgrad_reduce_multi_kernel");
  }
  return 0;
}
#undef WG_TILE_ARGS

extern "C" int dsl_conv2d_wgrad(const dsl_wgrad_desc* d, void* stream) {
  DSL_CHECK(d != nullptr, "dsl_conv2d_wgrad: null descriptor");
  return wgrad_launch(d, 1, stream);
}

extern "C" int dsl_conv2d_wgrad_group(const dsl_wgrad_desc* descs, int count, void* stream) {
  DSL_CHECK(descs != nullptr, "dsl_conv2d_wgrad_group: null descriptors");
  return wgrad_launch(descs, count, stream);
}
```

dsl_amd/engine.py:

```python
import ctypes as C
import os

import torch

from . import _lib as L
from . import ops
from .head_loss import FcosLossPlan
from .params import STAGE_BLOCKS, STAGE_PLANES
from .tuning import skip_items, tune, tune_int

DEFER_SLOTS = 144

BF = torch.bfloat16


class OpList:
    def __init__(self):
        self.items, self.keep, self.arr = [], [], None

    def _add(self, kind, desc=None, i=(), p=(), l=()):
        o = L.Op()
        o.kind = kind
        for k, v in enumerate(i):
            o.i[k] = int(v)
# ... 391 lines not shown
                    x, h, w = out, oh, ow
                    continue
                use_br = self.BR
                bd = None
                if fuse:
                    bd = ops.bneck_desc(x, st.w16_ptr(c1), st.w16_ptr(c2), st.w16_ptr(c3), idt, st.bn_ptrs(c1.bn), st.bn_ptrs(c2.bn),
                                        st.bn_ptrs(c3.bn), a1, a2, out, n=N, hin=h, win=w, h=oh, w=ow, planes=planes, cin=c1.cin_store,
                                        ldx=int(x.shape[-1]), stride=s)
                    if not L.lib.dsl_bottleneck_fwd_supported(C.byref(bd)):
                        bd = None
                if bd is not None:
                    if b == 0:
                        dd = self._conv(cv[p + '.downsample.0'], x, idt, N, [(h, w)], [(oh, ow)])
                        f.conv(dd)
                        if li == 1:
                            self._pp['ds'] = [(dd, 0)]
                            self._pp['c1'] = [(bd, 0)]
                    f.bneck(bd)
                    self.blocks.append(dict(prefix=p, xin=x, a1=a1, a2=a2, out=out, in_hw=(h, w), out_hw=(oh, ow), stride=s,
                                            stage=li, b=b, planes=planes))
                    x, h, w = out, oh, ow
                    continue
                if b == 0:
                    dd = self._conv(cv[p + '.downsample.0'], x, idt, N, [(h, w)], [(oh, ow)])
                    if use_br:
                        dd.workspace, dd.workspace_bytes = L.ptr(self.conv_ws_br), self.conv_ws_br.numel()
                        f.fork(self.BR)
                    f.conv(dd, side=use_br)
                if li == 1 and b == 0:
                    self._pp['ds'] = [(dd, 0)]
                d1 = self._conv(c1, x, a1, N, [(h, w)], [(oh, ow)], relu=True)
                if li == 1 and b == 0:
                    self._pp['c1'] = [(d1, 0)]
                f.conv(d1)
                f.conv(self._conv(c2, a1, a2, N, [(oh, ow)], [(oh, ow)], relu=True))
                if b == 0 and use_br:
                    f.join(self.BR)
                d3 = self._conv(c3, a2, out, N, [(oh, ow)], [(oh, ow)], relu=True, addend=idt)
                if li == 0 and b == nb - 1:
                    self._pp['c3'], self._pp['out'] = d3, out
                f.conv(d3)
                self.blocks.append(dict(prefix=p, xin=x, a1=a1, a2=a2, out=out, in_hw=(h, w), out_hw=(oh, ow), stride=s,
                                        stage=li, b=b, planes=planes))
                x, h, w = out, oh, ow
            self.stage_out.append((x, (h, w)))
            self.stage_ld.append(planes * 4)
            if li == 0:
                self._prefix_end = len(f.items)
        if split_open:
            f.join(self.BR)

    def _gn_workspace(self, key):
        ws = self._gn_ws.get(key)
        if ws is None:
            d = L.GnDesc()
            d.nseg, d.n, d.c, d.groups = len(self.level_sizes), self.N, 256, 32
            d.h, d.w = ops._segs(self.level_sizes)
            ws = torch.empty((L.lib.dsl_groupnorm_workspace_bytes(C.byref(d)) + 3) // 4, dtype=torch.float32, device=self.dev)
            self._gn_ws[key] = ws
        return ws

    def _wgrad(self, ol, spec, dy, x, n, out_hw, in_hw, cy=None, cd=None, wregion=None, bregion=None, side=False,
               emit=True, no_db=False, ldx=0, shared=0, raw=False, db_ptr=None, slots=0):
        st = self.store
        scale = st.bn_ptrs(spec.bn)[0] if (spec is not None and spec.bn and not raw) else None
        name = wregion or (spec.name + '.weight')
        db = db_ptr
        if bregion is not None:
            db = st.t32_ptr(bregion, st.grad)
        elif spec is not None and spec.bias and not no_db:
            db = st.t32_ptr(spec.name + '.bias', st.grad)
        k = 3 if spec is None else spec.k
        cs = 256 if spec is None else spec.cin_store
        d = ops.wgrad_desc(dy, x, st.t32_ptr(name, st.grad), n=n, grid=out_hw, src_hw=in_hw,
                           cs=cs, cy=cy or spec.cout_pad, cd=cd or spec.cout,
                           kh=k, kw=k, stride=1 if spec is None else spec.stride, pad=1 if spec is None else spec.pad,
                           scale=scale, db=db, workspace=self._wg_ws(n, out_hw, in_hw, spec, cy), ldx=ldx, shared=shared, slots=slots)
        if emit:
            if side and self._multi_on:
                self._wg_pending.append([d])
            else:
                ol.wgrad(d, side=side)
        return d

    def _wgrad_group(self, ol, descs, side=True, ws_name='wg_ws'):
        if not descs:
            return
        if side and self._multi_on:
            self._wg_pending.append(list(descs))
            return
        if len(descs) == 1:
            if ws_name != 'wg_ws':
                need = L.lib.dsl_wgrad_workspace_bytes(C.byref(descs[0]))
                ws = self._wg_buf(need, ws_name)
                descs[0].workspace, descs[0].workspace_bytes = L.ptr(ws), ws.numel()
            ol.wgrad(descs[0], side=side)
            return
        arr0 = (L.WgradDesc * len(descs))()
        for i, d in enumerate(descs):
            C.memmove(C.addressof(arr0[i]), C.addressof(d), C.sizeof(L.WgradDesc))
        need = L.lib.dsl_wgrad_group_workspace_bytes(arr0, len(descs))
        ol.wgrad_group(ops.wgrad_group(descs, workspace=self._wg_buf(need, ws_name)), side=side)

    def _flush_wgrads(self, ol, side=True, ws_name='wg_ws'):
        pending, self._wg_pending = self._wg_pending, []
        if not pending:
            return
        by_cfg = {}
        for sub in pending:
            by_cfg.setdefault(L.lib.dsl_wgrad_multi_config(C.byref(sub[0])), []).append(sub)
        on, self._multi_on = self._multi_on, False
        for cfg, subs in by_cfg.items():
            for lo in range(0, len(subs), L.MAX_MULTI):
                chunk = subs[lo:lo + L.MAX_MULTI]
                if cfg == 0 or len(chunk) == 1:
                    for sub in chunk:
                        self._wgrad_group(ol, sub, side=side, ws_name=ws_name)
                else:
                    ol.wgrad_multi(ops.WgradMulti(chunk, workspace=lambda need: self._wg_buf(need, ws_name)), side=side)
        self._multi_on = on

    def _wg_ws(self, n, out_hw, in_hw, spec, cy):
        need = ops.wgrad_workspace_bytes(n=n, grid=out_hw, src_hw=in_hw, cs=256 if spec is None else spec.cin_store,
                                         cy=cy or spec.cout_pad, cd=1, kh=3 if spec is None else spec.k,
                                         kw=3 if spec is None else spec.k, stride=1 if spec is None else spec.stride,
                                         pad=1 if spec is None else spec.pad)
        return self._wg_buf(need)

    def _wg_buf(self, need, name='wg_ws'):
        ws = self.bufs.get(name)
        if ws is None or ws.numel() < need:
            ws = torch.empty(max(need, 96 << 20), dtype=torch.uint8, device=self.dev)
            self.bufs.setdefault(name + '_old', []).append(self.bufs.get(name))
            self.bufs[name] = ws
        return ws

    def _dgrad(self, name, dy, dst, n, dy_hw, dst_hw, *, cs, cd, k, stride, pad, os=1, addend=None, mask=None,
               mask_first=False, mask_last=False, cs_real=0, wptr=None, cd_pad=None, ldd=None, lda=None, ldm=None):
        st = self.store
        f = (L.CONV_MASK_FIRST if mask_first else 0) | (L.CONV_MASK_LAST if mask_last else 0)
        grid = dy_hw if os > 1 else dst_hw
        return ops.conv_desc(dy, wptr if wptr is not None else st.wT_ptr(name), dst, n=n, grid=grid, src_hw=dy_hw, dst_hw=dst_hw,
                             cs=cs, cd=cd, cd_pad=cd_pad or cd, ldd=ldd or cd, kh=k, kw=k, stride=stride, pad=pad, mode=1, os=os,
                             flags=f, addend=addend, lda=lda or cd, mask=mask, ldm=ldm or cd, workspace=self.conv_ws,
                             cs_real=cs_real)

    def _build_backward(self):
        st, N, ls = self.store, self.N, self.level_sizes
        lp = self.lossplan
        reg = st.train_regions
        M = self.M
        SIDE = tune('side') != '0'
        GROUP_LAST = True
        TAIL_SLOTS = tune_int('tail_slots')
        GROUP = True
        self._multi_on = SIDE
        self._wg_pending = []
        g_feats = self.buf('g_feats', M, 256)
        PREFIX_LI = 2
        ol = OpList()
        ol.tag = 'bwd.head'
        ol.wait(L.SLOT_PACKS, stream=0)
        if PREFIX_LI == 0:
            ol.record(L.SLOT_TAIL, stream=0)
        ol.prof(5, 0, self._head_flops, self.M * 256 * 2.0 * (8 * 2 + 8 * 5 + 2))
        tower_group = []
        BT = 2 if SIDE else 0
        if BT:
            ol.fork(BT)

        def side_ws(cd_):
            cd_.workspace, cd_.workspace_bytes = L.ptr(self.conv_ws_side), self.conv_ws_side.numel()
            return cd_
        towers = (('reg_convs', BT), ('cls_convs', 0)) if BT else (('cls_convs', 0), ('reg_convs', 0))
        self._wgrad(ol, None, lp.g_cls, self.tower['cls_convs'][3]['act'], N, ls, ls, cy=st.cls_pad, cd=st.cls_rows, wregion='head.cls_w',
                    bregion='head.cls_b', side=SIDE)
        self._wgrad(ol, None, lp.g_rc, self.tower['reg_convs'][3]['act'], N, ls, ls, cy=64, cd=4 if st.ctr_on_cls else 5, wregion='head.regctr_w',
                    bregion='head.regctr_b', side=SIDE)
        g_act = {}
        gn_from_conv = set()

        def gn_records(cd_, tower, j, sd):
            lay = self.tower[tower][j]
            cd_.gn_x = L.ptr(lay['pre'])
            if L.lib.dsl_conv2d_gn_fusable(C.byref(cd_)):
                cd_.gn_ws = L.ptr(self._gn_workspace('bwd.' + tower))
                cd_.gn_gamma, cd_.gn_beta = L.ptr(st.t32_ptr(lay['gn'] + '.weight')), L.ptr(st.t32_ptr(lay['gn'] + '.bias'))
                cd_.gn_stats = L.ptr(lay['stats'])
                gn_from_conv.add((tower, j))
            else:
                cd_.gn_x = None
            return cd_
        for tower, sd in towers:
            wsf = side_ws if sd else (lambda c: c)
            g_act[tower] = self.buf(f'g_{tower}_act3', M, 256)
            if tower == 'cls_convs':
                ol.conv(gn_records(wsf(self._dgrad('head.cls', lp.g_cls, g_act[tower], N, ls, ls, cs=st.cls_pad, cd=256, k=3, stride=1, pad=1,
                                                         cs_real=st.cls_rows)),
                                   tower, 3, sd), side=sd)
            else:
                ol.conv(gn_records(wsf(self._dgrad('head.regctr', lp.g_rc, g_act[tower], N, ls, ls, cs=64, cd=256, k=3, stride=1, pad=1, cs_real=4 if st.ctr_on_cls else 5)),
                                   tower, 3, sd), side=sd)
        for i in (3, 2, 1, 0):
            g_pre = {}
            for tower, sd in towers:
                lay = self.tower[tower][i]
                base = lay['gn']
                g_pre[tower] = self.buf(f'g_{tower}_pre{i}', M, 256)
                gd = ops.gn_desc(lay['pre'], lay['act'], st.t32_ptr(base + '.weight'), st.t32_ptr(base + '.bias'),
                                 lay['stats'], self._gn_workspace('bwd.' + tower), n=N, hw=ls, dy=g_act[tower], dx=g_pre[tower],
                                 dgamma=st.t32_ptr(base + '.weight', st.grad), dbeta=st.t32_ptr(base + '.bias', st.grad),
                                 dbias=st.t32_ptr(lay['spec'].name + '.bias', st.grad) if lay['spec'].bias else None)
                gd.conv_stats = 1 if (tower, i) in gn_from_conv else 0
                ol.gn_bwd(gd, side=sd)
                tower_group.append(self._wgrad(ol, lay['spec'], g_pre[tower], lay['xin'], N, ls, ls, side=SIDE, emit=False, no_db=True,
                                               slots=DEFER_SLOTS if self.defer else tune_int('tower_slots')))
            if i == 0:
                if BT and SIDE:
                    ol.fork(1, other=BT)
                if self.defer:
                    self._deferred_towers = list(tower_group)
                else:
                    self._wgrad_group(ol, tower_group, side=SIDE)
                self._flush_wgrads(ol, side=SIDE)
                tower_group = []
            if i > 0:
                for tower, sd in towers:
                    wsf = side_ws if sd else (lambda c: c)
                    lay = self.tower[tower][i]
                    g_act[tower] = self.buf(f'g_{tower}_act{i - 1}', M, 256)
                    ol.conv(gn_records(wsf(self._dgrad(lay['spec'].name, g_pre[tower], g_act[tower], N, ls, ls, cs=256, cd=256, k=3, stride=1, pad=1)),
                                       tower, i - 1, sd), side=sd)
            else:
                cl, rl = self.tower['cls_convs'][0], self.tower['reg_convs'][0]
                ol.conv(self._dgrad(cl['spec'].name, g_pre['cls_convs'], g_feats, N, ls, ls, cs=256, cd=256, k=3, stride=1, pad=1))
                if BT:
                    ol.join(BT)
                ol.conv(self._dgrad(rl['spec'].name, g_pre['reg_convs'], g_feats, N, ls, ls, cs=256, cd=256, k=3, stride=1, pad=1, addend=g_feats))
                ol.prof(5, 1)
        self._flush_wgrads(ol, side=SIDE)
        ol.tag = 'bwd.fpn'
        cv = st.convs
        fc = [cv[f'neck.fpn_convs.{i}.conv'] for i in range(5)]
        lc = [cv[f'neck.lateral_convs.{i}.conv'] for i in range(3)]
        hw3, hw4, hw5, hw6, hw7 = ls
        gseg = [g_feats.data_ptr() + self.seg_off[i] * 256 * 2 for i in range(5)]
        lat = [self.bufs[f'lat{i}'] for i in range(3)]
        p6r = self.bufs['p6r']
        g_p6 = self.buf('g_p6', N, hw6[0], hw6[1], 256)
        g_p5 = self.buf('g_p5', N, hw5[0], hw5[1], 256)
        g_lat = [self.buf(f'g_lat{i}', N, hw[0], hw[1], 256) for i, hw in enumerate((hw3, hw4, hw5))]
        s0 = self.buf('s0', N, hw4[0], hw4[1], 256)
        s1 = self.buf('s1', N, hw5[0], hw5[1], 256)
        rla = st.backbone == 'rla'
        BB = 3 if (SIDE and not rla) else 0

        def br_ws(cd_):
            if BB:
                cd_.workspace, cd_.workspace_bytes = L.ptr(self.conv_ws_br), self.conv_ws_br.numel()
            return cd_
        if BB:
            ol.fork(BB)
        ol.conv(br_ws(self._dgrad(fc[0].name, gseg[0], g_lat[0], N, [hw3], [hw3], cs=256, cd=256, k=3, stride=1, pad=1)), side=BB)
        ol.sum2x2(g_lat[0], s0, N, hw4[0], hw4[1], hw3[0], hw3[1], 256, side=BB)
        ol.conv(br_ws(self._dgrad(fc[1].name, gseg[1], g_lat[1], N, [hw4], [hw4], cs=256, cd=256, k=3, stride=1, pad=1,
                                  addend=s0)), side=BB)
        ol.sum2x2(g_lat[1], s1, N, hw5[0], hw5[1], hw4[0], hw4[1], 256, side=BB)
        ol.conv(self._dgrad(fc[4].name, gseg[4], g_p6, N, [hw7], [hw6], cs=256, cd=256, k=3, stride=2, pad=1,
                            addend=gseg[3], mask=p6r, mask_first=True))
        ol.conv(self._dgrad(fc[3].name, g_p6, g_p5, N, [hw6], [hw5], cs=256, cd=256, k=3, stride=2, pad=1,
                            addend=gseg[2]))
        if BB:
            ol.join(BB)
        ol.conv(self._dgrad(fc[2].name, g_p5, g_lat[2], N, [hw5], [hw5], cs=256, cd=256, k=3, stride=1, pad=1,
                            addend=s1))
        self._wgrad(ol, fc[4], gseg[4], p6r, N, [hw7], [hw6], side=SIDE)
        self._wgrad(ol, fc[3], g_p6, self.feat_seg[2], N, [hw6], [hw5], side=SIDE)
        self._wgrad(ol, fc[2], g_p5, lat[2], N, [hw5], [hw5], side=SIDE)
        self._wgrad(ol, fc[1], gseg[1], lat[1], N, [hw4], [hw4], side=SIDE)
        self._wgrad(ol, fc[0], gseg[0], lat[0], N, [hw3], [hw3], side=SIDE)
        self.g_stage = {}
        self._br_pending = False
        for i, (li, hw) in ((2, (3, hw5)), (1, (2, hw4)), (0, (1, hw3))):
            cfeat = self.stage_out[li][0]
            cch = STAGE_PLANES[li] * 4
            ldc = self.stage_ld[li]
            self._wgrad(ol, lc[i], g_lat[i], cfeat, N, [hw], [hw], side=SIDE, ldx=ldc if ldc != cch else 0)
            g0b = self.buf(f'g_stage{li}_last', N, hw[0], hw[1], cch)
            self.g_stage[li] = g0b
            masked = not rla or li == 3
            sd = BB if li < 3 else 0
            if sd and not self._br_pending:
                ol.fork(BB)
                self._br_pending = True
            ol.conv(br_ws(self._dgrad(lc[i].name, g_lat[i], g0b, N, [hw], [hw], cs=256, cd=cch, k=1, stride=1, pad=0,
                                      mask=cfeat if masked else None, mask_first=masked, ldm=ldc)) if sd else
                    self._dgrad(lc[i].name, g_lat[i], g0b, N, [hw], [hw], cs=256, cd=cch, k=1, stride=1, pad=0,
                                mask=cfeat if masked else None, mask_first=masked, ldm=ldc), side=sd)
        buckets = st.grad_buckets()
        self._flush_wgrads(ol, side=SIDE)
        if self.defer:
            self.bwd_segments.append((ol, dict(bucket=None, slot=None, main=False)))
        else:
            ol.record(0)
            self.bwd_segments.append((ol, dict(bucket=buckets[0], slot=0, main=False)))
        if rla:
            from . import engine_rla
            self._multi_on = SIDE
            engine_rla.build_backward(self, buckets, SIDE)
            return
        blocks_by_stage = {li: [b for b in self.blocks if b['stage'] == li] for li in (1, 2, 3)}
        BSPLIT = tune('img_split_bwd')
        for li in (3, 2, 1):
            ol = OpList()
            ol.tag = f'bwd.l{li + 1}'
            if li == 1:
                self._multi_on = False
            blks = blocks_by_stage[li]
            hw = blks[0]['out_hw']
            planes = blks[0]['planes']
            g_pre = self.g_stage[li]
            g3, g2, g1 = [], [], []
            grp_all = GROUP and (li > 1 or GROUP_LAST)
            bsplit = bool(BB) and N >= 2 and grp_all and str(li + 1) in BSPLIT
            groups = [(0, (N + 1) // 2, 0), ((N + 1) // 2, N, BB)] if bsplit else [(0, N, 0)]
            if bsplit:
                ol.join(BB)
                ol.fork(BB)
                self._br_pending = False
            for blk in reversed(blks):
                p = blk['prefix']
                c1, c2, c3 = cv[p + '.conv1'], cv[p + '.conv2'], cv[p + '.conv3']
                gA2 = self.buf(p + '.g_a2', N, hw[0], hw[1], planes)
                gA1 = self.buf(p + '.g_a1', N, hw[0], hw[1], planes)
                grp = GROUP and (li > 1 or GROUP_LAST)
                tsl = TAIL_SLOTS if li == 1 else 0
                if bsplit:
                    g3.append(self._wgrad(ol, c3, g_pre, blk['a2'], N, [hw], [hw], side=SIDE, emit=False, slots=tsl))
                    g2.append(self._wgrad(ol, c2, gA2, blk['a1'], N, [hw], [hw], side=SIDE, emit=False, slots=tsl))
                    g_prev = self.buf(p + '.g_in', N, hw[0], hw[1], planes * 4) if blk['b'] > 0 else None
                    for g0, g1_, sd in groups:
                        wsf = br_ws if sd else (lambda d_: d_)
                        n_ = g1_ - g0
                        ol.conv(wsf(self._dgrad(c3.name, g_pre[g0:g1_], gA2[g0:g1_], n_, [hw], [hw], cs=c3.cout, cd=c3.cin, k=1, stride=1, pad=0,
                                                mask=blk['a2'][g0:g1_], mask_last=True)), side=sd)
                        ol.conv(wsf(self._dgrad(c2.name, gA2[g0:g1_], gA1[g0:g1_], n_, [hw], [hw], cs=c2.cout, cd=c2.cin, k=3, stride=1, pad=1,
                                                mask=blk['a1'][g0:g1_], mask_last=True)), side=sd)
                        if blk['b'] > 0:
                            ol.conv(wsf(self._dgrad(c1.name, gA1[g0:g1_], g_prev[g0:g1_], n_, [hw], [hw], cs=c1.cout, cd=c1.cin, k=1, stride=1,
                                                    pad=0, addend=g_pre[g0:g1_], mask=blk['xin'][g0:g1_], mask_last=True)), side=sd)
                        elif li > 1:
                            ds = cv[p + '.downsample.0']
                            tgt, ihw = self.g_stage[li - 1], blk['in_hw']
                            for spec, dy in ((ds, g_pre), (c1, gA1)):
                                ol.conv(wsf(self._dgrad(spec.name, dy[g0:g1_], tgt[g0:g1_], n_, [hw], [ihw], cs=spec.cout, cd=spec.cin, k=1,
                                                        stride=1, pad=0, os=2, addend=tgt[g0:g1_], mask=blk['xin'][g0:g1_], mask_first=True)), side=sd)
                    if blk['b'] > 0:
                        g1.append(self._wgrad(ol, c1, gA1, blk['xin'], N, [hw], [blk['in_hw']], side=SIDE, emit=False, slots=tsl))
                        g_pre = g_prev
                    else:
                        ol.join(BB)
                        d1 = self._wgrad(ol, c1, gA1, blk['xin'], N, [hw], [blk['in_hw']], side=SIDE, emit=True, slots=tsl)
                        dwd = self._wgrad(ol, cv[p + '.downsample.0'], g_pre, blk['xin'], N, [hw], [blk['in_hw']], side=SIDE, slots=tsl)
                        if li == 1:
                            self._pp['wg_c1'], self._pp['wg_ds'] = d1, dwd
                    continue
                ds_early = BB and blk['b'] == 0 and li > 1
                if ds_early:
                    ds = cv[p + '.downsample.0']
                    tgt, ihw = self.g_stage[li - 1], blk['in_hw']
                    ol.fork(BB)
                    ol.conv(br_ws(self._dgrad(ds.name, g_pre, tgt, N, [hw], [ihw], cs=ds.cout, cd=ds.cin, k=1, stride=1, pad=0,
                                              os=2, addend=tgt, mask=blk['xin'], mask_first=True)), side=BB)
                g3.append(self._wgrad(ol, c3, g_pre, blk['a2'], N, [hw], [hw], side=SIDE, emit=not grp, slots=tsl))
                ol.conv(self._dgrad(c3.name, g_pre, gA2, N, [hw], [hw], cs=c3.cout, cd=c3.cin, k=1, stride=1, pad=0,
                                    mask=blk['a2'], mask_last=True))
                g2.append(self._wgrad(ol, c2, gA2, blk['a1'], N, [hw], [hw], side=SIDE, emit=not grp, slots=tsl))
                ol.conv(self._dgrad(c2.name, gA2, gA1, N, [hw], [hw], cs=c2.cout, cd=c2.cin, k=3, stride=1, pad=1,
                                    mask=blk['a1'], mask_last=True))
                d1 = self._wgrad(ol, c1, gA1, blk['xin'], N, [hw], [blk['in_hw']], side=SIDE,
                                 emit=not (grp and blk['b'] > 0), slots=tsl)
                if li == 1 and blk['b'] == 0:
                    self._pp['wg_c1'] = d1
                if blk['b'] > 0:
                    g1.append(d1)
                if blk['b'] > 0:
                    g_prev = self.buf(p + '.g_in', N, hw[0], hw[1], planes * 4)
                    ol.conv(self._dgrad(c1.name, gA1, g_prev, N, [hw], [hw], cs=c1.cout, cd=c1.cin, k=1, stride=1,
                                        pad=0, addend=g_pre, mask=blk['xin'], mask_last=True))
                    g_pre = g_prev
                else:
                    ds = cv[p + '.downsample.0']
                    dwd = self._wgrad(ol, ds, g_pre, blk['xin'], N, [hw], [blk['in_hw']], side=SIDE, slots=tsl)
                    if li == 1:
                        self._pp['wg_ds'] = dwd
                    if li > 1:
                        tgt = self.g_stage[li - 1]
                        ihw = blk['in_hw']
                        if BB:
                            ol.join(BB)
                        for spec, dy in ((c1, gA1),) if ds_early else ((ds, g_pre), (c1, gA1)):
                            ol.conv(self._dgrad(spec.name, dy, tgt, N, [hw], [ihw], cs=spec.cout, cd=spec.cin, k=1,
                                                stride=1, pad=0, os=2, addend=tgt, mask=blk['xin'], mask_first=True))
            if li == PREFIX_LI:
                ol.record(L.SLOT_TAIL, stream=0)
            if GROUP and (li > 1 or GROUP_LAST):
                on_main = '2' if li == 1 else '0'
                order = sorted(((3, g3), (2, g2), (1, g1)), key=lambda t: str(t[0]) in on_main)
                for gi, grp_descs in order:
                    mine = str(gi) in on_main
                    self._wgrad_group(ol, grp_descs, side=SIDE and not mine, ws_name='wg_ws_main' if mine else 'wg_ws')
            self._flush_wgrads(ol, side=SIDE)
            seg = 4 - li
            ol.record(seg)
            if li == 1:
                ol.join()
            self.bwd_segments.append((ol, dict(bucket=buckets[seg], slot=seg, main=(li == 1))))
            if li == 1 and self.defer:
                dl = OpList()
                on, self._multi_on = self._multi_on, False
                self._wgrad_group(dl, self._deferred_towers, side=True)
                self._multi_on = on
                dl.record(0)
                self.bwd_segments.append((dl, dict(bucket=buckets[0], slot=0, main=False, deferred=True)))

    def _split_prefix(self):
        f, end = self.fwd, self._prefix_end
        pre, rest = OpList(), OpList()
        pre.items, rest.items = f.items[:end], f.items[end:]
        if 'prefix' in skip_items():
            pre.items = [o for o in pre.items if o.kind != L.OP_CONV]
        pre.keep = rest.keep = f.keep
        ws = torch.empty(32 << 20, dtype=torch.uint8, device=self.dev)
        for o in pre.items:
            if o.kind == L.OP_CONV and o.i[6] == 0:
                d = C.cast(o.desc, C.POINTER(L.ConvDesc)).contents
                if d.workspace:
                    d.workspace, d.workspace_bytes = ws.data_ptr(), ws.numel()
        pre.keep.append(ws)
        w0 = L.Op()
        w0.kind, w0.i[0], w0.i[1] = L.OP_WAIT, 0, L.SLOT_TAIL
        r0 = L.Op()
        r0.kind, r0.i[0], r0.i[1] = L.OP_RECORD, 0, L.SLOT_PREFIX
        pre.items = [w0] + pre.items + [r0]
        self._img_op += 1
        w1 = L.Op()
        w1.kind, w1.i[0], w1.i[1] = L.OP_WAIT, 0, L.SLOT_PREFIX
        self.fwd_inline = f
        self.fwd_rest = rest
        rest.items = [w1] + rest.items
        self.prefix = pre
        out = self._pp['out']
        self._l1out = [out, torch.empty_like(out)]
        self._parity = 0

    def set_parity(self, p):
        ptr = self._l1out[p].data_ptr()
        self._pp['c3'].dst = ptr
        for d_, off in self._pp['c1'] + self._pp['ds']:
            if isinstance(d_, L.BneckDesc):
                d_.x = ptr + off
            else:
                d_.src = ptr + off
        self._pp['wg_c1'].x = ptr
        self._pp['wg_ds'].x = ptr
        self._parity = p

    def bind_image(self, img, half_last=False):
        assert img.shape[0] == self.N - (1 if half_last else 0), (tuple(img.shape), self.N, half_last)
        if half_last and self._stem_fused is False:
            raise RuntimeError('half_last needs the fused stem kernel (DSL_STEM_FUSED=0 is set)')
        direct = img.is_cuda and img.dtype == torch.float32 and img.is_contiguous() and img.device == self.img.device
        if not direct:
            self.img[:img.shape[0]].copy_(img, non_blocking=True)
        ptr = img.data_ptr() if direct else self.img.data_ptr()
        self._img_ref = img if direct else None
        lists = [(self.fwd, self._img_op - (1 if self.prefix is not None else 0))]
        if self.prefix is not None:
            lists.append((self.prefix, self._img_op))
        for f, idx in lists:
            if f.arr is None:
                f.arr = (L.Op * len(f.items))(*f.items)
            f.arr[idx].p[0] = ptr
            if self._stem_fused:
                f.arr[idx].i[4] = 1 if half_last else 0

    def fp8_warm(self, fwd):
        if getattr(self, 'fp8_cold', False):
            self.fp8_cold = False
            fwd.run()
            fwd.run()

    def forward(self, img=None):
        if img is not None:
            self.bind_image(img)
        self.fp8_warm(self.fwd)
        self.fwd.run()


class Engine:

    MAX_PLANS = 12

    def __init__(self):
        self.plans = {}

    def plan(self, store, N, H, W, training=True, single_stream=False):
        if store.dirty:
            store.refresh()
        key = (id(store), getattr(store, 'generation', 0), bool(getattr(store, 'defer_head', False)), single_stream, N, H, W, training)
        p = self.plans.pop(key, None)
        if p is None:
            stale = [k for k in self.plans if k[0] == id(store) and k[1] != key[1]]
            while stale or len(self.plans) >= self.MAX_PLANS:
                torch.cuda.synchronize()
                self.plans.pop(stale.pop() if stale else next(iter(self.plans)))
            p = Plan(store, N, H, W, training, single_stream=single_stream)
        self.plans[key] = p
        return p
```

dsl_amd/ops.py:

```python
import ctypes as C

import torch

from . import _lib as L

lib = L.lib


def _segs(shapes):
    return L.seg5([s[0] for s in shapes]), L.seg5([s[1] for s in shapes])


def conv_desc(src, wgt, dst, *, n, grid, src_hw, dst_hw, cs, cd, cd_pad, ldd, kh, kw, stride=1, pad=0,
              mode=0, os=1, flags=0, scale=None, bias=None, addend=None, lda=0, add_hw=None, mask=None,
              ldm=0, workspace=None, cs_real=0, lds=0):
    d = L.ConvDesc()
    d.nseg, d.n = len(grid), n
    d.gh, d.gw = _segs(grid)
    d.sh, d.sw = _segs(src_hw)
    d.dh, d.dw = _segs(dst_hw)
    if add_hw is not None:
        d.ah, d.aw = _segs(add_hw)
    d.cs, d.cd, d.cd_pad, d.ldd, d.lda, d.ldm = cs, cd, cd_pad, ldd, lda, ldm
    d.kh, d.kw, d.stride, d.pad, d.mode, d.os, d.flags = kh, kw, stride, pad, mode, os, flags
# ... 25 lines not shown
    raw = lambda t: 0 if t is None else (t if isinstance(t, int) else t.data_ptr())
    out = []
    for py in (0, 1):
        for px in (0, 1):
            gh, gw = (h - py + 1) // 2, (w - px + 1) // 2
            if gh <= 0 or gw <= 0:
                continue
            k, pad, _ = s2_class(py, px)
            off = py * w + px
            d = conv_desc(dy, packs[(py, px)], raw(dst) + off * ldd * 2, n=n, grid=[(gh, gw)], src_hw=[(oh, ow)], dst_hw=[(h, w)], cs=cs, cd=cd,
                          cd_pad=cd_pad or cd, ldd=ldd, kh=k, kw=k, stride=1, pad=pad, mode=1, os=2, flags=flags,
                          addend=(raw(addend) + off * (lda or cd) * 2) if addend is not None else None, lda=lda or cd,
                          mask=(raw(mask) + off * (ldm or cd) * 2) if mask is not None else None, ldm=ldm or cd, workspace=workspace,
                          cs_real=cs_real)
            d._keep = d._keep + (dy, dst, mask, addend)
            out.append(d)
    return out


def bneck_desc(x, w1, w2, w3, idt, bn1, bn2, bn3, a1, a2, out, *, n, hin, win, h, w, planes, cin, ldx=None, stride=1, ldi=None, ldo=None):
    d = L.BneckDesc()
    raw = lambda t: 0 if t is None else (t if isinstance(t, int) else t.data_ptr())
    d.x, d.w1, d.w2, d.w3, d.idt = raw(x), raw(w1), raw(w2), raw(w3), raw(idt)
    (d.s1, d.b1), (d.s2, d.b2), (d.s3, d.b3) = [(raw(s_), raw(b_)) for s_, b_ in (bn1, bn2, bn3)]
    d.a1, d.a2, d.out = raw(a1), raw(a2), raw(out)
    d.n, d.hin, d.win, d.h, d.w = n, hin, win, h, w
    d.planes, d.cin, d.ldx, d.stride = planes, cin, ldx or cin, stride
    d.ldi, d.ldo = ldi or 4 * planes, ldo or 4 * planes
    d._keep = (x, w1, w2, w3, idt, bn1, bn2, bn3, a1, a2, out)
    return d


def bottleneck_fwd(*a, **k):
    d = bneck_desc(*a, **k)
    L.check(lib.dsl_bottleneck_fwd(C.byref(d), L.stream_ptr()), 'dsl_bottleneck_fwd')
    return d


def conv_workspace_bytes(d):
    return lib.dsl_conv2d_workspace_bytes(C.byref(d))


def conv2d(*a, **k):
    d = conv_desc(*a, **k)
    L.check(lib.dsl_conv2d(C.byref(d), L.stream_ptr()), 'dsl_conv2d')
    return d


def wgrad_desc(dy, x, dw, *, n, grid, src_hw, cs, cy, cd, kh, kw, stride=1, pad=0, scale=None, db=None,
               workspace=None, force_cfg=None, ldx=0, shared=0, slots=0):
    d = L.WgradDesc()
    d.nseg, d.n = len(grid), n
    d.gh, d.gw = _segs(grid)
    d.sh, d.sw = _segs(src_hw)
    d.cs, d.cy, d.cd, d.kh, d.kw, d.stride, d.pad = cs, cy, cd, kh, kw, stride, pad
    d.ldx, d.shared, d.slots = ldx, shared, slots
    d.splits = 0 if force_cfg is None else -(force_cfg + 1)
    if force_cfg is None:
        d.splits = lib.dsl_wgrad_splits(C.byref(d))
    d.dy, d.x, d.scale, d.dw, d.db = L.ptr(dy), L.ptr(x), L.ptr(scale), L.ptr(dw), L.ptr(db)
    need = lib.dsl_wgrad_workspace_bytes(C.byref(d))
    if workspace is None:
        workspace = torch.empty(need, dtype=torch.uint8, device=dy.device)
    assert workspace.numel() * workspace.element_size() >= need, (workspace.numel(), need)
    d.workspace, d.workspace_bytes = L.ptr(workspace), workspace.numel() * workspace.element_size()
    tab = pixtab(d, dy.device if hasattr(dy, 'device') else 'cuda')
    d._keep = (dy, x, dw, scale, db, workspace, tab)
    return d


_pixtabs = None


def pixtab(d, device='cuda'):
    global _pixtabs
    import weakref
    if _pixtabs is None:
        _pixtabs = weakref.WeakValueDictionary()
    need = lib.dsl_wgrad_pixtab_bytes(C.byref(d))
    if need == 0:
        d.pixtab, d.pixtab_bytes = None, 0
        return None
    dev = torch.device(device)
    if dev.index is None:
        dev = torch.device('cuda', torch.cuda.current_device())
    key = (dev.index, d.nseg, d.n, d.kh, d.kw, d.stride, d.pad) + tuple(d.gh) + tuple(d.gw) + tuple(d.sh) + tuple(d.sw)
    t = _pixtabs.get(key)
    if t is None:
        t = torch.empty(need, dtype=torch.uint8, device=dev)
        L.check(lib.dsl_wgrad_pixtab_fill(C.byref(d), L.ptr(t), need, L.stream_ptr()), 'dsl_wgrad_pixtab_fill')
        torch.cuda.current_stream().synchronize()
        _pixtabs[key] = t
    d.pixtab, d.pixtab_bytes = L.ptr(t), t.numel()
    return t


def wgrad_workspace_bytes(*, n, grid, src_hw, cs, cy, cd, kh, kw, stride=1, pad=0):
    d = L.WgradDesc()
    d.nseg, d.n = len(grid), n
    d.gh, d.gw = _segs(grid)
    d.sh, d.sw = _segs(src_hw)
    d.cs, d.cy, d.cd, d.kh, d.kw, d.stride, d.pad = cs, cy, cd, kh, kw, stride, pad
    d.splits = 0
    return lib.dsl_wgrad_workspace_bytes(C.byref(d))


def wgrad_group(descs, workspace=None):
    assert 1 <= len(descs) <= L.MAX_GROUP
    arr = (L.WgradDesc * len(descs))()
    for i, d in enumerate(descs):
        C.memmove(C.addressof(arr[i]), C.addressof(d), C.sizeof(L.WgradDesc))
        arr[i].splits = 0
    need = lib.dsl_wgrad_group_workspace_bytes(arr, len(descs))
    if workspace is None:
        workspace = torch.empty(need, dtype=torch.uint8, device='cuda')
    nbytes = workspace.numel() * workspace.element_size()
    assert nbytes >= need, (nbytes, need)
    arr[0].workspace, arr[0].workspace_bytes = L.ptr(workspace), nbytes
    arr._keep = (list(descs), workspace)
    return arr


class WgradMulti:

    def __init__(self, subs, workspace=None, device='cuda'):
        assert 1 <= len(subs) <= L.MAX_MULTI and all(1 <= len(g) <= L.MAX_GROUP for g in subs)
        flat = [d for g in subs for d in g]
        self.descs = (L.WgradDesc * len(flat))()
        for i, d in enumerate(flat):
            C.memmove(C.addressof(self.descs[i]), C.addressof(d), C.sizeof(L.WgradDesc))
            self.descs[i].splits = 0
        self.counts = (C.c_int * len(subs))(*[len(g) for g in subs])
        self.nsub = len(subs)
        need = lib.dsl_wgrad_multi_workspace_bytes(self.descs, self.counts, self.nsub)
        if need == 0:
            L.check(-1, 'dsl_wgrad_multi_workspace_bytes')
        self.workspace_bytes = need
        if callable(workspace):
            workspace = workspace(need)
        if workspace is None:
            workspace = torch.empty(need, dtype=torch.uint8, device=device)
        assert workspace.numel() * workspace.element_size() >= need
        nb = lib.dsl_wgrad_multi_table_bytes()
        self.host = torch.zeros(nb, dtype=torch.uint8)
        L.check(lib.dsl_wgrad_multi_build(self.descs, self.counts, self.nsub, L.ptr(workspace), workspace.numel() * workspace.element_size(),
                                          C.c_void_p(self.host.data_ptr()), nb), 'dsl_wgrad_multi_build')
        self.dev = self.host.to(device)
        self._keep = (flat, workspace)

    def run(self, stream=None):
        L.check(lib.dsl_conv2d_wgrad_multi(C.c_void_p(self.host.data_ptr()), L.ptr(self.dev), stream or L.stream_ptr()), 'dsl_conv2d_wgrad_multi')


def conv2d_wgrad_group(descs, workspace=None):
    arr = wgrad_group(descs, workspace)
    L.check(lib.dsl_conv2d_wgrad_group(arr, len(descs), L.stream_ptr()), 'dsl_conv2d_wgrad_group')
    return arr


def conv2d_wgrad(*a, **k):
    d = wgrad_desc(*a, **k)
    L.check(lib.dsl_conv2d_wgrad(C.byref(d), L.stream_ptr()), 'dsl_conv2d_wgrad')
    return d


def gn_desc(x, y, gamma, beta, stats, workspace=None, *, n, hw, c=256, groups=32, eps=1e-5, dy=None, dx=None,
            dgamma=None, dbeta=None, dbias=None, y8=None, y8_scale=None, y8_amax=None):
    d = L.GnDesc()
    d.nseg, d.n, d.c, d.groups = len(hw), n, c, groups
    d.h, d.w = _segs(hw)
    d.eps = eps
    d.x, d.y, d.gamma, d.beta, d.stats = (L.ptr(t) for t in (x, y, gamma, beta, stats))
    d.dy, d.dx, d.dgamma, d.dbeta, d.dbias = (L.ptr(t) for t in (dy, dx, dgamma, dbeta, dbias))
    need = lib.dsl_groupnorm_workspace_bytes(C.byref(d))
    if workspace is None:
        workspace = torch.empty(need, dtype=torch.uint8, device='cuda')
    nbytes = workspace.numel() * workspace.element_size()
    assert nbytes >= need, (nbytes, need)
    d.workspace, d.workspace_bytes = L.ptr(workspace), nbytes
    d.y8, d.y8_scale, d.y8_amax = (L.ptr(t) for t in (y8, y8_scale, y8_amax))
    d._keep = (x, y, gamma, beta, stats, workspace, dy, dx, dgamma, dbeta, dbias, y8, y8_scale, y8_amax)
    return d


def fcos_desc(*, n, sizes, strides, ranges, radius=1.5, num_classes=80):
    d = L.FcosDesc()
    d.nlvl, d.n = len(sizes), n
    d.h, d.w = _segs(sizes)
    d.stride = L.seg5(strides)
    for i, (lo, hi) in enumerate(ranges):
        d.range_lo[i], d.range_hi[i] = float(lo), float(hi)
    d.radius, d.num_classes = radius, num_classes
    d.loss_weight, d.soft_weight, d.grad_scale, d.inv_world = 1.0, 0.0, 1.0, 1.0
    d._keep = {}
    return d


def set_ptrs(d, **tensors):
    for k, t in tensors.items():
        setattr(d, k, L.ptr(t))
        d._keep[k] = t
    return d


def eval_match(mode, num_cats, num_imgs, det_boxes, det_off, gt_boxes, gt_area, gt_crowd, gt_ignore, gt_off, max_gt_per_cell,
               iou_thrs, area_ranges):
    M, G, T, R = det_boxes.shape[0], gt_boxes.shape[0], iou_thrs.numel(), area_ranges.shape[0]
    dev = det_off.device
    shape = (R, T, M) if mode == L.EVAL_COCO else (M,)
    out_a = torch.zeros(shape, dtype=torch.uint8, device=dev)
    out_b = torch.zeros(shape, dtype=torch.uint8, device=dev)
    npos = torch.zeros(num_cats, R, dtype=torch.int32, device=dev) if mode == L.EVAL_COCO else None
    need = int(lib.dsl_eval_match_workspace_bytes(G, int(max_gt_per_cell)))
    ws = torch.empty(need, dtype=torch.uint8, device=dev) if need else None
    L.check(lib.dsl_eval_match(mode, num_cats, num_imgs, M, G, int(max_gt_per_cell), L.ptr(det_boxes), L.ptr(det_off), L.ptr(gt_boxes),
                               L.ptr(gt_area), L.ptr(gt_crowd), L.ptr(gt_ignore), L.ptr(gt_off), L.ptr(iou_thrs), T, L.ptr(area_ranges), R,
                               L.ptr(out_a), L.ptr(out_b), L.ptr(npos), L.ptr(ws), need, L.stream_ptr()), 'dsl_eval_match')
    return out_a, out_b, npos


def eval_accumulate(num_cats, num_imgs, matched, ignored, npos, det_off, perm, rec_thrs):
    R, T, M = matched.shape
    prec = torch.empty(R, T, rec_thrs.numel(), num_cats, dtype=torch.float64, device=det_off.device)
    L.check(lib.dsl_eval_accumulate(num_cats, num_imgs, M, R, T, rec_thrs.numel(), L.ptr(matched), L.ptr(ignored), L.ptr(npos),
                                    L.ptr(det_off), L.ptr(perm), L.ptr(rec_thrs), L.ptr(prec), L.stream_ptr()), 'dsl_eval_accumulate')
    return prec
```

dsl_amd/tuning.py:

```python
import os

DEFAULTS = {
    'side': '1',
    'pipe_prefix': '1',
    'img_split': '234',
    'bneck_fwd': '2',
    'img_split_bwd': '23',
    'tower_slots': '72',
    'tail_slots': '192',
    'rla_split': '123',
    'rla_tail': '1',
    'rla_split_bwd': '',
    'check_backward_grad': '0',
    'skip': '',
    'lib.wgrad_slots': '128',
    'lib.stream_probe': '1',
    'lib.comm_queue': '1',
    'lib.rla_tail_form': '0',
    'lib.debug_sync': '0',
    'lib.skip_kinds': '0',
}

_values = dict(DEFAULTS)
_parsed = False


def _parse():
    global _parsed
    if _parsed:
        return
    _parsed = True
    for item in os.environ.get('DSL_TUNE', '').split(','):
        item = item.strip()
        if not item:
            continue
        k, _, v = item.partition('=')
        if k not in DEFAULTS:
            raise KeyError(f'DSL_TUNE: unknown key {k!r} (supported: {sorted(DEFAULTS)})')
        _values[k] = v


def tune(key):
    _parse()
    return _values[key]


def tune_int(key):
    return int(tune(key), 0)


def set_tune(key, value):
    _parse()
    if key not in DEFAULTS:
        raise KeyError(key)
    _values[key] = str(value)
    if key.startswith('lib.'):
        from . import _lib as L
        L.check(L.lib.dsl_set_option(key[4:].encode(), int(str(value), 0)), 'dsl_set_option')


def skip_items():
    return frozenset(t for t in tune('skip').split('+') if t)


def push_lib_options(lib):
    _parse()
    for k, v in _values.items():
        if k.startswith('lib.') and v != DEFAULTS[k]:
            if lib.dsl_set_option(k[4:].encode(), int(v, 0)) != 0:
                raise RuntimeError(f'dsl_set_option({k[4:]}) failed')
```

include/dsl_hip.h:

```cpp
#ifndef DSL_HIP_H
#define DSL_HIP_H
#include <stddef.h>
#include <stdint.h>

#ifdef __cplusplus
extern "C" {
#endif

#define DSL_MAX_SEG 5
#define DSL_MAX_GROUP 8

int dsl_version(void);
const char* dsl_last_error(void);
int dsl_set_option(const char* name, int value);
int dsl_get_option(const char* name, int* value);

enum {
  DSL_CONV_RELU_OUT = 1,
  DSL_CONV_RELU_IN = 2,
  DSL_CONV_OUT_F32 = 4,
  DSL_CONV_MASK_FIRST = 8,
  DSL_CONV_MASK_LAST = 16,
  DSL_CONV_ADD_UPSAMPLE = 32,
  DSL_CONV_SMALL_C = 64,
  DSL_CONV_FP8 = 128,
  DSL_CONV_EPI_STAGED = 1 << 16
};

typedef struct dsl_conv_desc {
  int32_t nseg, n;
  int32_t gh[DSL_MAX_SEG], gw[DSL_MAX_SEG];
  int32_t sh[DSL_MAX_SEG], sw[DSL_MAX_SEG];
  int32_t dh[DSL_MAX_SEG], dw[DSL_MAX_SEG];
  int32_t ah[DSL_MAX_SEG], aw[DSL_MAX_SEG];
  int32_t cs;
  int32_t cd;
  int32_t cd_pad;
  int32_t ldd, lda, ldm;
  int32_t kh, kw, stride, pad, mode, os, flags;
  const void* src;
  const void* wgt;
  void* dst;
  const float* scale;
  const float* bias;
  const void* addend;
  const void* mask;
  void* workspace;
  size_t workspace_bytes;
  int32_t cs_real;
  int32_t lds;
  void* gn_ws;
  const void* gn_x;
  const float* gn_gamma;
  const float* gn_beta;
  const float* gn_stats;
} dsl_conv_desc;

int dsl_conv2d_gn_fusable(const dsl_conv_desc* d);

size_t dsl_conv2d_workspace_bytes(const dsl_conv_desc* d);
int dsl_conv2d(const dsl_conv_desc* d, void* stream);

typedef struct dsl_wgrad_desc {
  int32_t nseg, n;
  int32_t gh[DSL_MAX_SEG], gw[DSL_MAX_SEG];
  int32_t sh[DSL_MAX_SEG], sw[DSL_MAX_SEG];
  int32_t cs;
  int32_t cy;
  int32_t cd;
  int32_t kh, kw, stride, pad;
  int32_t splits;
  const void* dy;
  const void* x;
  const float* scale;
  float* dw;
  float* db;
  void* workspace;
  size_t workspace_bytes;
  int32_t ldx;
  int32_t shared;
  int32_t slots;
  int32_t pad_;
  const void* pixtab;
  size_t pixtab_bytes;
} dsl_wgrad_desc;

int dsl_wgrad_splits(const dsl_wgrad_desc* d);
size_t dsl_wgrad_workspace_bytes(const dsl_wgrad_desc* d);
size_t dsl_wgrad_pixtab_bytes(const dsl_wgrad_desc* d);
int dsl_wgrad_pixtab_fill(const dsl_wgrad_desc* d, void* table, size_t bytes, void* stream);
int dsl_conv2d_wgrad(const dsl_wgrad_desc* d, void* stream);
size_t dsl_wgrad_group_workspace_bytes(const dsl_wgrad_desc* descs, int count);
int dsl_conv2d_wgrad_group(const dsl_wgrad_desc* descs, int count, void* stream);

#define DSL_MAX_MULTI 16
int dsl_wgrad_multi_config(const dsl_wgrad_desc* d);
size_t dsl_wgrad_multi_table_bytes(void);
size_t dsl_wgrad_multi_workspace_bytes(const dsl_wgrad_desc* descs, const int* counts, int nsub);
int dsl_wgrad_multi_build(const dsl_wgrad_desc* descs, const int* counts, int nsub, void* workspace, size_t workspace_bytes,
                          void* table_host, size_t table_bytes);
int dsl_conv2d_wgrad_multi(const void* table_host, const void* table_dev, void* stream);
int dsl_wgrad_multi_info(const void* table_host, double* flops, double* bytes, int* blocks, int* red_blocks, int* nsub);
int dsl_wgrad_plan_probe(const int* stages, const int* tiles, const long long* tile_elems, int nsub, int cfg, int cap,
                         int* splits_out, int* info);

int dsl_quant_fp8(const void* x_bf16, void* y_fp8, long rows, int c, int ld_x, float scale, void* stream);
int dsl_absmax(const void* x_bf16, long rows, int c, int ld_x, float* partials, int n_partials, void* stream);
int dsl_quant_fp8_dyn(const void* x_bf16, void* y_fp8, long rows, int c, int ld_x, const float* partials, int n_partials, void* stream);
int dsl_fp8_comb(const float* winv, float* comb, int n, const float* partials, int n_partials, void* stream);
int dsl_quant_fp8_weights(const float* w, void* w8, float* comb, const float* bn_scale, int cout, int cout_pad, int k,
                          float inv_act_scale, void* stream);
typedef struct dsl_fp8_prep_item {
  const float* w;
  void* w8;
  float* comb;
  const float* amax;
  float* scale;
  int32_t n_amax, cout;
} dsl_fp8_prep_item;
int dsl_fp8_prep(const dsl_fp8_prep_item* items_dev, int n_items, int cout_pad, int k, float margin, void* stream);
int dsl_quant_fp8_delayed(const void* x_bf16, void* y_fp8, long rows, int c, int ld_x, const float* scale_dev, float* partials,
                          int n_partials, void* stream);

typedef struct dsl_bneck_desc {
  const void* x; const void* w1; const void* w2; const void* w3; const void* idt;
  const float* s1; const float* b1; const float* s2; const float* b2; const float* s3; const float* b3;
  void* a1; void* a2; void* out;
  int32_t n, hin, win, h, w;
  int32_t planes, cin, ldx, stride, ldi, ldo;
} dsl_bneck_desc;
int dsl_bottleneck_fwd_supported(const dsl_bneck_desc* d);
int dsl_bottleneck_fwd(const dsl_bneck_desc* d, void* stream);

typedef struct dsl_image_prep_item {
  const unsigned char* src;
  int32_t src_h, src_w;
  int32_t new_h, new_w;
  int32_t flip;
  int32_t ps_mode, ps_crop;
  int32_t to_rgb;
  float mean[3], inv_std[3];
} dsl_image_prep_item;
int dsl_image_prep(const dsl_image_prep_item* items_dev, int n, float* dst, int hc, int wc, void* stream);
int dsl_image_prep_u8(const dsl_image_prep_item* items_dev, int n, unsigned char* dst_u8, int hc, int wc, void* stream);

enum { DSL_AUG_COPY = 0, DSL_AUG_AFFINE = 1, DSL_AUG_BRIGHTNESS = 2, DSL_AUG_CONTRAST = 3, DSL_AUG_SATURATION = 4, DSL_AUG_HUE = 5,
       DSL_AUG_GRAY = 6, DSL_AUG_BLUR_H = 7, DSL_AUG_BLUR_V = 8, DSL_AUG_ERASE = 9,
       DSL_AUG_AUTOCONTRAST = 10, DSL_AUG_EQUALIZE = 11, DSL_AUG_SOLARIZE = 12, DSL_AUG_POSTERIZE = 13, DSL_AUG_SHARPNESS = 14 };
typedef struct dsl_aug_item {
  int32_t h, w;
  int32_t kind;
  int32_t order;
  float m[6];
  int32_t roi[4];
  int32_t cval;
  float f[3];
  int32_t rect[3][4];
  uint32_t seed;
} dsl_aug_item;
size_t dsl_image_aug_scratch_bytes(int n);
int dsl_image_aug(const dsl_aug_item* items_dev, int n, const unsigned char* src, unsigned char* dst, int hc, int wc,
                  void* scratch, int need_stats, void* stream);
int dsl_image_normalize(const unsigned char* src_u8, const dsl_image_prep_item* items_dev, int n, float* dst, int hc, int wc,
                        void* stream);

int dsl_pack_image(const float* img_nchw, void* out_nhwc8, int n, int h, int w, void* stream);

int dsl_stem_pool(const float* img_nchw, const void* w_groups, const float* scale, const float* bias, void* out, int ld_out,
                  int n, int h, int w, void* stream);
int dsl_stem_pool_half(const float* img_nchw, const void* w_groups, const float* scale, const float* bias, void* out, int ld_out,
                       int n, int h, int w, int half_last, void* stream);

int dsl_maxpool3x3s2(const void* x, void* y, int n, int h, int w, int c, void* stream);
int dsl_maxpool3x3s2_ld(const void* x, void* y, int n, int h, int w, int c, int ldy, void* stream);

typedef struct dsl_gn_desc {
  int32_t nseg, n, c, groups;
  int32_t h[DSL_MAX_SEG], w[DSL_MAX_SEG];
  float eps;
  const void* x;
  void* y;
  const float* gamma;
  const float* beta;
  float* stats;
  const void* dy;
  void* dx;
  float* dgamma;
  float* dbeta;
  float* dbias;
  void* workspace;
  size_t workspace_bytes;
  int32_t conv_stats;
  int32_t pad_;
  void* y8;
  const float* y8_scale;
  float* y8_amax;
} dsl_gn_desc;
size_t dsl_groupnorm_workspace_bytes(const dsl_gn_desc* d);
int dsl_groupnorm_relu_fwd(const dsl_gn_desc* d, void* stream);
int dsl_groupnorm_relu_bwd(const dsl_gn_desc* d, void* stream);

int dsl_avgpool2x2(const void* x, int ldx, void* y, int ldy, int n, int h, int w, int c, void* stream);
int dsl_avgpool2x2_bwd(const void* gy, int ldgy, void* gx, int ldgx, int n, int h, int w, int c, void* stream);
int dsl_bn_tanh_fwd(const void* u, int ldu, const float* scale, const float* bias, void* t, int ldt, long rows, int c,
                    void* stream);
size_t dsl_bn_tanh_bwd_workspace_bytes(long rows, int c);
int dsl_bn_tanh_bwd(const void* gt, int ldgt, const void* t, int ldt, const void* u, int ldu, const float* scale,
                    const float* mean, const float* var, float eps, void* gu, int ldgu, float* dgamma, float* dbeta,
                    void* workspace, long rows, int c, void* stream);
typedef struct dsl_rec_sum_item {
  const float* rec; float* out_a; float* out_b;
  int32_t nrec, pad_;
} dsl_rec_sum_item;
int dsl_rec_sum_multi(const dsl_rec_sum_item* items_dev, int n, int c, void* stream);
int dsl_bn_fold(const float* gamma, const float* beta, const float* mean, const float* var, float eps, float* scale,
                float* bias, int n, void* stream);
typedef struct dsl_bn_post_item {
  const float* w; float* dw; float* dgamma; const float* dbeta; const float* gamma; const float* mean; const float* var;
  int32_t rows, k, row_start, pad_;
} dsl_bn_post_item;
int dsl_bn_wgrad_post(const dsl_bn_post_item* items_dev, int n, int total_rows, float eps, void* stream);
int dsl_rla_tail_fwd(const void* x, int ldx, const void* h_in, int ldh, const void* w_conv_out, int c4, const float* bn_scale,
                     const float* bn_bias, const void* w_recurrent, int tw, void* u, void* t, void* h_out, int ldo, int n, int h, int w,
                     void* stream);
size_t dsl_rla_tail_bwd_workspace_bytes(int n, int h, int w);
int dsl_rla_tail_bwd(const void* g_h, int ldgh, const void* wT_recurrent, int ldw, const void* t, int ldt, const void* u,
                     const float* scale, const float* mean, const float* var, float eps, void* g_u, int ldgu, float* dgamma, float* dbeta,
                     void* workspace, int n, int h, int w, void* stream);
enum { DSL_RLA_AVGPOOL = 2, DSL_RLA_AVGPOOL_BWD = 3, DSL_RLA_BN_TANH = 4, DSL_RLA_BN_TANH_BWD = 5,
       DSL_RLA_BN_FOLD = 6, DSL_RLA_BN_POST = 7, DSL_RLA_REC_SUM = 8 ,
       DSL_RLA_TAIL_FWD = 9 ,
       DSL_RLA_TAIL_BWD = 10  };
typedef struct dsl_rla_desc {
  int32_t kind;
  int32_t i[8];
  float f[2];
  int64_t rows;
  void* p[12];
} dsl_rla_desc;
int dsl_rla_op(const dsl_rla_desc* d, void* stream);

int dsl_sum2x2(const void* g, void* out, int n, int h, int w, int ch, int cw, int c, void* stream);

int dsl_colsum(const void* x, float* out, long rows, int c, int ld, void* stream);

typedef struct dsl_fcos_desc {
  int32_t nlvl, n;
  int32_t h[DSL_MAX_SEG], w[DSL_MAX_SEG], stride[DSL_MAX_SEG];
  float range_lo[DSL_MAX_SEG], range_hi[DSL_MAX_SEG];
  float radius;
  int32_t num_classes;
  const float* gt_boxes;
  const int64_t* gt_labels;
  const int32_t* gt_off;
  const float* ig_boxes;
// ... 197 lines not shown
```

Measured before the change: 448.8 imgs/s.

## Add pipelined 128x128 wgrad tile and optional batched tail wgrad reduce

Adds a pipelined (async LDS ring) variant of the 128x128 wgrad tile, which is enabled by default. It uses split units of two 32-wide k-steps and alternates the bias-gradient LDS reads across phases. The slot cap for that tile doubles. It also adds a batch wgrad path that launches each sub-group's main kernel and then one combined reduce kernel, but this path is gated behind the tail_batch tuning flag, which defaults to 0. The intent is to move 128x128 wgrad shapes off the non-pipelined kernel and cut reduce launches in the layer-1 tail. The cost is more code paths and different split and occupancy behaviour.

```diff
diff --git a/dsl_amd/_lib.py b/dsl_amd/_lib.py
--- a/dsl_amd/_lib.py
+++ b/dsl_amd/_lib.py
@@ -184,7 +184,7 @@
     lib.dsl_image_aug_scratch_bytes.restype = C.c_size_t
 if hasattr(lib, 'dsl_rla_tail_bwd_workspace_bytes'):
     lib.dsl_rla_tail_bwd_workspace_bytes.restype = C.c_size_t
-for _n in ('dsl_wgrad_multi_table_bytes', 'dsl_wgrad_multi_workspace_bytes'):
+for _n in ('dsl_wgrad_multi_table_bytes', 'dsl_wgrad_multi_workspace_bytes', 'dsl_wgrad_batch_table_bytes', 'dsl_wgrad_batch_workspace_bytes'):
     if hasattr(lib, _n):
         getattr(lib, _n).restype = C.c_size_t
 if hasattr(lib, 'dsl_bn_tanh_bwd_workspace_bytes'):
@@ -206,6 +206,7 @@
     'dsl_wgrad_multi_config': [_vp], 'dsl_wgrad_multi_table_bytes': [], 'dsl_wgrad_multi_workspace_bytes': [_vp, _vp, _i],
     'dsl_wgrad_multi_build': [_vp, _vp, _i, _vp, C.c_size_t, _vp, C.c_size_t], 'dsl_conv2d_wgrad_multi': [_vp, _vp, _vp], 'dsl_wgrad_multi_info': [_vp, _vp, _vp, _vp, _vp, _vp],
     'dsl_wgrad_plan_probe': [_vp, _vp, _vp, _i, _i, _i, _vp, _vp],
+    'dsl_wgrad_batch_table_bytes': [], 'dsl_wgrad_batch_workspace_bytes': [_vp, _vp, _i], 'dsl_wgrad_batch_build': [_vp, _vp, _i, _vp, C.c_size_t, _vp, C.c_size_t],
     'dsl_image_prep': [_vp, _i, _vp, _i, _i, _vp],
     'dsl_pack_image': [_vp, _vp, _i, _i, _i, _vp], 'dsl_stem_pool': [_vp, _vp, _vp, _vp, _vp, _i, _i, _i, _i, _vp], 'dsl_stem_pool_half': [_vp, _vp, _vp, _vp, _vp, _i, _i, _i, _i, _i, _vp], 'dsl_maxpool3x3s2': [_vp, _vp, _i, _i, _i, _i, _vp],
     'dsl_maxpool3x3s2_ld': [_vp, _vp, _i, _i, _i, _i, _i, _vp],
diff --git a/dsl_amd/csrc/api.hip b/dsl_amd/csrc/api.hip
--- a/dsl_amd/csrc/api.hip
+++ b/dsl_amd/csrc/api.hip
@@ -23,6 +23,7 @@
 struct Option { const char* name; int value; };
 Option g_options[] = {
     {"wgrad_slots", 128},
+    {"wgrad_pipe128", 1},
     {"stream_probe", 1},
     {"debug_sync", 0},
     {"skip_kinds", 0},
diff --git a/dsl_amd/csrc/wgrad.hip b/dsl_amd/csrc/wgrad.hip
--- a/dsl_amd/csrc/wgrad.hip
+++ b/dsl_amd/csrc/wgrad.hip
@@ -23,12 +23,16 @@
 };
 constexpr WgTile kWgTiles[] = {
     {256, 256, 2, 4, 64, 2, false}, {256, 128, 4, 2, 64, 3, false}, {128, 256, 2, 4, 64, 3, false}, {128, 128, 2, 2, 64, 2, false},
-    {256, 256, 2, 4, 32, 4, true},  {256, 128, 4, 2, 32, 5, true},  {128, 256, 2, 4, 32, 5, true},
+    {256, 256, 2, 4, 32, 4, true},  {256, 128, 4, 2, 32, 5, true},  {128, 256, 2, 4, 32, 5, true},  {128, 128, 2, 2, 32, 4, true},
 };
 constexpr int kWgDescRing = 16;
-constexpr bool wgrad_cfg_ok(int cfg, bool pipe) { return cfg >= 1 && cfg <= (pipe ? 3 : 4); }
+constexpr bool wgrad_cfg_ok(int cfg, bool) { return cfg >= 1 && cfg <= 4; }
 constexpr int wgrad_row(int cfg, bool pipe) { return (pipe ? 4 : 0) + cfg - 1; }
 constexpr const WgTile& wgrad_tile(int cfg, bool pipe) { return kWgTiles[wgrad_row(cfg, pipe)]; }
+constexpr int wgrad_pipe_unit(int bco, int bci) { return bco == 128 && bci == 128 ? 2 : 1; }
+constexpr int wgrad_split_unit(int cfg, bool pipe) { return cfg >= 1 && cfg <= 4 && pipe ? wgrad_pipe_unit(wgrad_tile(cfg, true).bco, wgrad_tile(cfg, true).bci) : 1; }
+static_assert(wgrad_split_unit(4, true) * wgrad_tile(4, true).ks == wgrad_tile(4, false).ks && wgrad_split_unit(1, true) == 1 &&
+              wgrad_split_unit(2, true) == 1 && wgrad_split_unit(3, true) == 1, "split unit of the pipelined rows");
 constexpr size_t wgrad_lds_bytes(int bco, int bci, int ks, int nst, bool pipe) {
   return (size_t)nst * ks * 2 * (bco + bci) + (pipe ? (size_t)kWgDescRing * ks * 8 : 0);
 }
@@ -492,8 +496,9 @@
   const int co0 = (rem_wg % p.gx) * BCO;
   const int colt = rem_wg / p.gx;
   const bool do_db = colt == 0 && ((p.dbmask >> member) & 1);
-  constexpr int DB_PAIRS = BCO / 2, DB_RG = 64 * NW / DB_PAIRS, DB_ROWS = KS / DB_RG;
-  static_assert(DB_ROWS >= 1 && DB_ROWS <= 8 && DB_RG * DB_PAIRS == 64 * NW, "bias-gradient thread mapping");
+  constexpr int DBU = wgrad_pipe_unit(BCO, BCI);
+  constexpr int DB_PAIRS = BCO / 2, DB_RG = 64 * NW / DB_PAIRS, DB_ROWS = KS * DBU / DB_RG, DB_ACT = DB_RG / DBU;
+  static_assert(DB_ROWS >= 1 && DB_ROWS <= 16 && DB_RG * DB_PAIRS == 64 * NW && DB_ACT * DBU == DB_RG && DB_ACT * DB_ROWS == KS, "bias-gradient thread mapping");
   const int db_cp = tid % DB_PAIRS, db_rg = tid / DB_PAIRS;
   float db_lo = 0.f, db_hi = 0.f;
   const int ctiles = p.cs / BCI;
@@ -690,17 +695,19 @@
   set_read_stage(lds_base);
   issue(0, 0);
 
-  unsigned dbr[8];
+  unsigned dbr[DB_ROWS];
   int slot_c = 0;
   for (int s = kt0; s < kt1; ++s) {
     const unsigned st = lds_base + slot_c * STAGE;
     const int nslot = (slot_c + 1 == NST) ? 0 : slot_c + 1;
+    const int db_ph = DBU > 1 ? (s - kt0) % DBU : 0;
+    const bool db_now = DBU > 1 ? do_db && db_rg / DB_ACT == db_ph : do_db;
 #pragma unroll
     for (int kk = 0; kk < KK; ++kk) {
       const int f = kk & 1;
       wait_lds(f);
       if (kk == 0) desc_use();
-      if (kk == 1 && do_db) {
+      if (kk == 1 && db_now) {
 #pragma unroll
         for (int j = 0; j < DB_ROWS; ++j) {
           pin1(dbr[j]);
@@ -708,10 +715,10 @@
           db_hi += __uint_as_float(dbr[j] & 0xffff0000u);
         }
       }
-      if (kk == 0 && do_db) {
+      if (kk == 0 && db_now) {
 #pragma unroll
         for (int j = 0; j < DB_ROWS; ++j) {
-          const int row = db_rg * DB_ROWS + j;
+          const int row = (db_rg - db_ph * DB_ACT) * DB_ROWS + j;
           dbr[j] = lds_read_b32_asm(st + row * YB + ((((db_cp * 4) >> 6) ^ (row & 3)) << 6) + ((db_cp * 4) & 63));
         }
       }
@@ -863,11 +870,7 @@
   long long krow, sstride;
   int splits, cd, blk_start, nblk;
 };
-__global__ void wgrad_reduce_multi_kernel(const RedEnt* __restrict__ tab, int n) {
-  int e = 0;
-  for (int i = 1; i < n; ++i) e = (int)blockIdx.x >= tab[i].blk_start ? i : e;
-  const RedEnt r = tab[e];
-  const int lb = (int)blockIdx.x - r.blk_start;
+__device__ __forceinline__ void wgrad_reduce_entry(const RedEnt& r, const int lb) {
   if (lb == 0 && r.db)
     for (int c = threadIdx.x; c < r.cd; c += blockDim.x) {
       float sacc = 0.f;
@@ -892,6 +895,23 @@
     if (r.scale) s *= r.scale[co];
     *reinterpret_cast<f32x4*>(r.dw + el) = s;
   }
+}
+__global__ void wgrad_reduce_multi_kernel(const RedEnt* __restrict__ tab, int n) {
+  int e = 0;
+  for (int i = 1; i < n; ++i) e = (int)blockIdx.x >= tab[i].blk_start ? i : e;
+  const RedEnt r = tab[e];
+  wgrad_reduce_entry(r, (int)blockIdx.x - r.blk_start);
+}
+constexpr int kMaxBatchRed = 16;
+struct RedBatch {
+  int n;
+  RedEnt e[kMaxBatchRed];
+};
+__global__ void wgrad_reduce_batch_kernel(const RedBatch b) {
+  int e = 0;
+  for (int i = 1; i < b.n; ++i) e = (int)blockIdx.x >= b.e[i].blk_start ? i : e;
+  const RedEnt r = b.e[e];
+  wgrad_reduce_entry(r, (int)blockIdx.x - r.blk_start);
 }
 
 struct RedK {
@@ -988,6 +1008,7 @@
 }
 bool wgrad_v3_ok(const dsl_wgrad_desc* d, int cfg) {
   if (!wgrad_cfg_ok(cfg, true) || d->kh > 8 || d->kw > 8) return false;
+  if (cfg == 4 && dsl_option("wgrad_pipe128") == 0) return false;
   long long xo = 0;
   for (int s = 0; s < d->nseg; ++s) {
     xo += (long long)d->n * d->sh[s] * d->sw[s];
@@ -1017,11 +1038,12 @@
     case 3: f(std::integral_constant<int, 3>{}); break;
     case 4: f(std::integral_constant<int, 4>{}); break;
     case 5: f(std::integral_constant<int, 5>{}); break;
-    default: f(std::integral_constant<int, 6>{}); break;
+    case 6: f(std::integral_constant<int, 6>{}); break;
+    default: f(std::integral_constant<int, 7>{}); break;
   }
   return true;
 }
-static_assert(sizeof(kWgTiles) / sizeof(kWgTiles[0]) == 7, "wgrad_dispatch lists every row");
+static_assert(sizeof(kWgTiles) / sizeof(kWgTiles[0]) == 8, "wgrad_dispatch lists every row");
 #define WG_TILE_ARGS(T) T.bco, T.bci, T.wco, T.wci, T.ks, T.nst
 template <auto KERNEL, class... Args>
 void wgrad_run(const WgTile& T, dim3 grid, hipStream_t st, const Args&... args) {
@@ -1068,7 +1090,8 @@
   if (splits < 1) splits = 1;
   if (splits > 256) splits = 256;
   {
-    const int ks = wgrad_tile(cfg, wgrad_v3_ok(d, cfg)).ks;
+    const bool v3 = wgrad_v3_ok(d, cfg);
+    const int ks = wgrad_tile(cfg, v3).ks * wgrad_split_unit(cfg, v3);
     const int stages = (int)((wgrad_px(d) + ks - 1) / ks);
     const int tps = (stages + splits - 1) / splits;
     splits = (stages + tps - 1) / tps;
@@ -1133,7 +1156,7 @@
   return true;
 }
 
-static int wgrad_fill_k(const dsl_wgrad_desc* descs, int count, int splits, int cfg, bool v3, WgK& k, long long* px_out, long long* xo_out) {
+static int wgrad_fill_k(const dsl_wgrad_desc* descs, int count, int splits, int cfg, bool v3, int unit, WgK& k, long long* px_out, long long* xo_out) {
   const dsl_wgrad_desc* d = descs;
   memset(&k, 0, sizeof(k));
   k.nseg = d->nseg; k.n = d->n;
@@ -1178,7 +1201,7 @@
   k.splits = splits;
   k.chunk = (k.gx * k.gy * count * splits + 7) / 8;
   k.ktiles = (px + t.ks - 1) / t.ks;
-  k.tiles_per_split = (k.ktiles + splits - 1) / splits;
+  k.tiles_per_split = unit * (((k.ktiles + unit - 1) / unit + splits - 1) / splits);
   if (v3)
     if (int rc = wgrad_v3_fill(d, k, px)) return rc;
   *px_out = px;
@@ -1186,7 +1209,19 @@
   return 0;
 }
 
-static int wgrad_launch(const dsl_wgrad_desc* descs, int count, void* stream) {
+struct WgPartials {
+  float* ws;
+  float* dbws;
+  int splits, cyp;
+  long long krow;
+};
+static size_t wgrad_launch_workspace(const dsl_wgrad_desc* d, int count, int* splits_out) {
+  const int splits = count == 1 ? (d->splits > 0 ? d->splits : dsl_wgrad_splits(d)) : wgrad_splits_for(d, count);
+  if (splits_out) *splits_out = splits;
+  return (size_t)splits * count * wgrad_cy_pad(d) * ((size_t)d->kh * d->kw * d->cs + 1) * sizeof(float);
+}
+
+static int wgrad_launch_main(const dsl_wgrad_desc* descs, int count, void* workspace, size_t workspace_bytes, void* stream, WgPartials* out) {
   const dsl_wgrad_desc* d = descs;
   DSL_CHECK(d != nullptr && count >= 1 && count <= DSL_MAX_GROUP, "dsl_conv2d_wgrad: bad group (count=%d)", count);
   DSL_CHECK(d->nseg >= 1 && d->nseg <= DSL_MAX_SEG, "dsl_conv2d_wgrad: nseg=%d", d->nseg);
@@ -1196,18 +1231,18 @@
     DSL_CHECK(descs[g].dy && descs[g].x && descs[g].dw, "dsl_conv2d_wgrad: null pointer (member %d)", g);
     DSL_CHECK(wgrad_same_geometry(d, &descs[g]), "dsl_conv2d_wgrad_group: member %d has a different geometry", g);
   }
-  DSL_CHECK(d->workspace, "dsl_conv2d_wgrad: null workspace");
+  DSL_CHECK(workspace, "dsl_conv2d_wgrad: null workspace");
   const int cfg = wgrad_pick(d);
   DSL_CHECK(wgrad_cfg_ok(cfg, false), "dsl_conv2d_wgrad: there is no tile configuration %d (1 .. 4; the register-staged configuration 0 is gone)", cfg);
-  const int splits = count == 1 ? (d->splits > 0 ? d->splits : dsl_wgrad_splits(d)) : wgrad_splits_for(d, count);
+  int splits;
+  const size_t need = wgrad_launch_workspace(d, count, &splits);
   const int cyp = (int)wgrad_cy_pad(d);
-  const size_t need = (size_t)splits * count * cyp * ((size_t)d->kh * d->kw * d->cs + 1) * sizeof(float);
-  DSL_CHECK(d->workspace_bytes >= need, "dsl_conv2d_wgrad: workspace too small (%zu < %zu)", d->workspace_bytes, need);
+  DSL_CHECK(workspace_bytes >= need, "dsl_conv2d_wgrad: workspace too small (%zu < %zu)", workspace_bytes, need);
   const bool v3 = wgrad_v3_ok(d, cfg);
   WgK k;
   long long px, xo;
-  if (int rc = wgrad_fill_k(descs, count, splits, cfg, v3, k, &px, &xo)) return rc;
-  k.ws = (float*)d->workspace;
+  if (int rc = wgrad_fill_k(descs, count, splits, cfg, v3, wgrad_split_unit(cfg, v3), k, &px, &xo)) return rc;
+  k.ws = (float*)workspace;
   k.dbws = k.ws + (size_t)splits * count * cyp * k.krow;
 #ifdef DSL_ABLATE_BUILD
   { const char* e = getenv("DSL_ABLATE"); k.dbg = e ? atoi(e) : 0; }
@@ -1219,7 +1254,7 @@
                        : -1;
   dim3 grid(k.chunk * 8);
   if (v3) {
-    const int cap = ((d->slots > 0 ? d->slots : wgrad_slots()) + 7) / 8 * 8;
+    const int cap = ((d->slots > 0 ? d->slots : wgrad_slots()) * (cfg == 4 ? 2 : 1) + 7) / 8 * 8;
     if ((int)grid.x > cap) grid.x = cap;
   }
   wgrad_dispatch(cfg, v3, [&](auto row) {
@@ -1229,6 +1264,17 @@
   });
   dsl_prof_end(prof, st);
   DSL_LAUNCH_CHECK(v3 ? "wgrad_pipe_kernel" : "wgrad_glds_kernel");
+  out->ws = k.ws; out->dbws = k.dbws; out->splits = splits; out->cyp = cyp; out->krow = k.krow;
+  return 0;
+}
+
+static int wgrad_launch(const dsl_wgrad_desc* descs, int count, void* stream) {
+  DSL_CHECK(descs != nullptr, "dsl_conv2d_wgrad: null descriptor");
+  const dsl_wgrad_desc* d = descs;
+  WgPartials k;
+  if (int rc = wgrad_launch_main(descs, count, d->workspace, d->workspace_bytes, stream, &k)) return rc;
+  const int splits = k.splits, cyp = k.cyp;
+  hipStream_t st = (hipStream_t)stream;
   const long long total4 = (long long)d->cd * k.krow / 4;
   int rb = (int)((total4 + 255) / 256);
   if (rb > 4096 / count) rb = 4096 / count;
@@ -1242,12 +1288,12 @@
   if (d->shared && count > 1) {
     for (int g = 1; g < count; ++g)
       DSL_CHECK(descs[g].dw == d->dw && descs[g].scale == d->scale && !descs[g].db, "dsl_conv2d_wgrad_group: shared members must share dw / scale and have no db");
-    hipLaunchKernelGGL(wgrad_reduce_kernel, dim3(rb * count, 1), dim3(256), 0, st, (const float*)d->workspace, r, splits * count, 1,
+    hipLaunchKernelGGL(wgrad_reduce_kernel, dim3(rb * count, 1), dim3(256), 0, st, (const float*)k.ws, r, splits * count, 1,
                        cyp, d->cd, k.krow);
     DSL_LAUNCH_CHECK("wgrad_reduce_kernel");
     return 0;
   }
-  hipLaunchKernelGGL(wgrad_reduce_kernel, dim3(rb, count), dim3(256), 0, st, (const float*)d->workspace, r, splits, count,
+  hipLaunchKernelGGL(wgrad_reduce_kernel, dim3(rb, count), dim3(256), 0, st, (const float*)k.ws, r, splits, count,
                      cyp, d->cd, k.krow);
   DSL_LAUNCH_CHECK("wgrad_reduce_kernel");
   return 0;
@@ -1516,7 +1562,7 @@
     const dsl_wgrad_desc* d = &descs[first[s]];
     WgK& k = t->k[i];
     long long px, xo;
-    if (int rc = wgrad_fill_k(d, counts[s], splits[s], t->cfg, t->v3 != 0, k, &px, &xo)) return rc;
+    if (int rc = wgrad_fill_k(d, counts[s], splits[s], t->cfg, t->v3 != 0, 1, k, &px, &xo)) return rc;
     k.direct = splits[s] == 1 ? 1 : 0;
     k.ws = (float*)ws;
     blocks += k.chunk * 8;
@@ -1629,7 +1675,118 @@
   return 0;
 }
 
+namespace {
+constexpr int kBatchMagic = 0x57424131;
+constexpr size_t kBatchAlign = 256;
+struct WgBatchTable {
+  int magic, nsub;
+  int counts[kMaxMulti];
+  const dsl_wgrad_desc* descs;
+  void* workspace;
+  size_t workspace_bytes;
+  double flops, bytes;
+  int red_blocks;
+};
+int wgrad_batch_check(const dsl_wgrad_desc* descs, const int* counts, int nsub) {
+  DSL_CHECK(descs && counts && nsub >= 1 && nsub <= kMaxMulti, "dsl_wgrad_batch: bad sub-launch list (n=%d)", nsub);
+  int off = 0;
+  for (int s = 0; s < nsub; ++s) {
+    DSL_CHECK(counts[s] >= 1 && counts[s] <= DSL_MAX_GROUP, "dsl_wgrad_batch: sub-launch %d has %d members", s, counts[s]);
+    DSL_CHECK(descs[off].nseg >= 1 && descs[off].nseg <= DSL_MAX_SEG, "dsl_wgrad_batch: bad geometry in sub-launch %d", s);
+    for (int g = 0; g < counts[s]; ++g) DSL_CHECK(!descs[off + g].shared, "dsl_wgrad_batch: shared-weight groups use dsl_conv2d_wgrad_group");
+    off += counts[s];
+  }
+  DSL_CHECK(off <= kMaxBatchRed, "dsl_wgrad_batch: %d members, at most %d", off, kMaxBatchRed);
+  return 0;
+}
+int wgrad_batch_launch(const WgBatchTable* t, void* stream) {
+  RedBatch rb;
+  memset(&rb, 0, sizeof(rb));
+  unsigned char* ws = (unsigned char*)t->workspace;
+  size_t left = t->workspace_bytes;
+  int off = 0, red_blocks = 0;
+  for (int s = 0; s < t->nsub; ++s) {
+    const dsl_wgrad_desc* d = &t->descs[off];
+    const int count = t->counts[s];
+    const size_t need = (wgrad_launch_workspace(d, count, nullptr) + kBatchAlign - 1) / kBatchAlign * kBatchAlign;
+    DSL_CHECK(left >= need, "dsl_conv2d_wgrad_multi (batch): workspace too small for sub-launch %d", s);
+    WgPartials k;
+    if (int rc = wgrad_launch_main(d, count, ws, need, stream, &k)) return rc;
+    for (int g = 0; g < count; ++g) {
+      DSL_CHECK(rb.n < kMaxBatchRed, "dsl_conv2d_wgrad_multi (batch): more than %d members", kMaxBatchRed);
+      RedEnt& r = rb.e[rb.n++];
+      r.ws = k.ws + (long long)g * k.cyp * k.krow;
+      r.dw = d[g].dw; r.scale = d[g].scale; r.db = d[g].db;
+      r.dbws = k.dbws + (long long)g * k.cyp; r.dbstride = (long long)count * k.cyp;
+      r.krow = k.krow; r.sstride = (long long)count * k.cyp * k.krow; r.splits = k.splits; r.cd = d->cd;
+      const long long total4 = (long long)d->cd * k.krow / 4;
+      int nb = (int)((total4 + 255) / 256);
+      if (nb > 512) nb = 512;
+      if (nb < 1) nb = 1;
+      r.blk_start = red_blocks; r.nblk = nb;
+      red_blocks += nb;
+    }
+    ws += need; left -= need;
+    off += count;
+  }
+  hipLaunchKernelGGL(wgrad_reduce_batch_kernel, dim3(red_blocks), dim3(256), 0, (hipStream_t)stream, rb);
+  DSL_LAUNCH_CHECK("wgrad_reduce_batch_kernel");
+  return 0;
+}
+}
+
+extern "C" size_t dsl_wgrad_batch_table_bytes(void) { return sizeof(WgBatchTable); }
+
+extern "C" size_t dsl_wgrad_batch_workspace_bytes(const dsl_wgrad_desc* descs, const int* counts, int nsub) {
+  if (wgrad_batch_check(descs, counts, nsub)) return 0;
+  size_t need = 0;
+  int off = 0;
+  for (int s = 0; s < nsub; ++s) {
+    need += (wgrad_launch_workspace(&descs[off], counts[s], nullptr) + kBatchAlign - 1) / kBatchAlign * kBatchAlign;
+    off += counts[s];
+  }
+  return need;
+}
+
+extern "C" int dsl_wgrad_batch_build(const dsl_wgrad_desc* descs, const int* counts, int nsub, void* workspace, size_t ws_bytes,
+                                     void* table_host, size_t table_bytes) {
+  if (int rc = wgrad_batch_check(descs, counts, nsub)) return rc;
+  DSL_CHECK(table_host && table_bytes >= sizeof(WgBatchTable), "dsl_wgrad_batch_build: table buffer too small");
+  DSL_CHECK(workspace && ws_bytes >= dsl_wgrad_batch_workspace_bytes(descs, counts, nsub), "dsl_wgrad_batch_build: workspace too small");
+  WgBatchTable* t = (WgBatchTable*)table_host;
+  memset(t, 0, sizeof(*t));
+  t->magic = kBatchMagic;
+  t->nsub = nsub;
+  t->descs = descs;
+  t->workspace = workspace;
+  t->workspace_bytes = ws_bytes;
+  int off = 0;
+  for (int s = 0; s < nsub; ++s) {
+    const dsl_wgrad_desc* d = &descs[off];
+    t->counts[s] = counts[s];
+    const long long px = wgrad_px(d);
+    long long xo = 0;
+    for (int i = 0; i < d->nseg; ++i) xo += (long long)d->n * d->sh[i] * d->sw[i];
+    const double krow = (double)d->kh * d->kw * d->cs;
+    t->flops += 2.0 * counts[s] * px * (double)d->cd * krow;
+    t->bytes += counts[s] * ((double)px * d->cd * 2.0 + (double)xo * d->cs * 2.0 + (double)d->cd * krow * 4.0);
+    const long long total4 = (long long)(d->cd * krow / 4);
+    t->red_blocks += counts[s] * (int)std::max<long long>(1, std::min<long long>(512, (total4 + 255) / 256));
+    off += counts[s];
+  }
+  return 0;
+}
+
 extern "C" int dsl_wgrad_multi_info(const void* table_host, double* flops, double* bytes, int* blocks, int* red_blocks, int* nsub) {
+  if (table_host && ((const WgBatchTable*)table_host)->magic == kBatchMagic) {
+    const WgBatchTable* b = (const WgBatchTable*)table_host;
+    if (flops) *flops = b->flops;
+    if (bytes) *bytes = b->bytes;
+    if (blocks) *blocks = 0;
+    if (red_blocks) *red_blocks = b->red_blocks;
+    if (nsub) *nsub = b->nsub;
+    return 0;
+  }
   const WgMultiTable* t = (const WgMultiTable*)table_host;
   DSL_CHECK(t && t->magic == kMultiMagic, "dsl_wgrad_multi_info: not a table of dsl_wgrad_multi_build");
   if (flops) *flops = t->flops;
@@ -1641,8 +1798,9 @@
 }
 
 extern "C" int dsl_conv2d_wgrad_multi(const void* table_host, const void* table_dev, void* stream) {
+  if (table_host && ((const WgBatchTable*)table_host)->magic == kBatchMagic) return wgrad_batch_launch((const WgBatchTable*)table_host, stream);
   const WgMultiTable* t = (const WgMultiTable*)table_host;
-  DSL_CHECK(t && table_dev && t->magic == kMultiMagic, "dsl_conv2d_wgrad_multi: not a table of dsl_wgrad_multi_build");
+  DSL_CHECK(t && table_dev && t->magic == kMultiMagic, "dsl_conv2d_wgrad_multi: not a table of dsl_wgrad_multi_build or dsl_wgrad_batch_build");
   const unsigned char* dev = (const unsigned char*)table_dev;
   const WgK* ktab = (const WgK*)(dev + offsetof(WgMultiTable, k));
   const RedEnt* rtab = (const RedEnt*)(dev + offsetof(WgMultiTable, red));
diff --git a/dsl_amd/engine.py b/dsl_amd/engine.py
--- a/dsl_amd/engine.py
+++ b/dsl_amd/engine.py
@@ -567,6 +567,7 @@
         M = self.M
         SIDE = tune('side') != '0'
         GROUP_LAST = True
+        TAIL_BATCH = tune('tail_batch') == '1'
         TAIL_SLOTS = tune_int('tail_slots')
         GROUP = True
         self._multi_on = SIDE
@@ -750,6 +751,7 @@
                 gA1 = self.buf(p + '.g_a1', N, hw[0], hw[1], planes)
                 grp = GROUP and (li > 1 or GROUP_LAST)
                 tsl = TAIL_SLOTS if li == 1 else 0
+                tail_batch = li == 1 and grp and TAIL_BATCH
                 if bsplit:
                     g3.append(self._wgrad(ol, c3, g_pre, blk['a2'], N, [hw], [hw], side=SIDE, emit=False, slots=tsl))
                     g2.append(self._wgrad(ol, c2, gA2, blk['a1'], N, [hw], [hw], side=SIDE, emit=False, slots=tsl))
@@ -775,8 +777,9 @@
                         g_pre = g_prev
                     else:
                         ol.join(BB)
-                        d1 = self._wgrad(ol, c1, gA1, blk['xin'], N, [hw], [blk['in_hw']], side=SIDE, emit=True, slots=tsl)
-                        dwd = self._wgrad(ol, cv[p + '.downsample.0'], g_pre, blk['xin'], N, [hw], [blk['in_hw']], side=SIDE, slots=tsl)
+                        d1 = self._wgrad(ol, c1, gA1, blk['xin'], N, [hw], [blk['in_hw']], side=SIDE, emit=not tail_batch, slots=tsl)
+                        dwd = self._wgrad(ol, cv[p + '.downsample.0'], g_pre, blk['xin'], N, [hw], [blk['in_hw']], side=SIDE,
+                                          emit=not tail_batch, slots=tsl)
                         if li == 1:
                             self._pp['wg_c1'], self._pp['wg_ds'] = d1, dwd
                     continue
@@ -794,7 +797,7 @@
                 ol.conv(self._dgrad(c2.name, gA2, gA1, N, [hw], [hw], cs=c2.cout, cd=c2.cin, k=3, stride=1, pad=1,
                                     mask=blk['a1'], mask_last=True))
                 d1 = self._wgrad(ol, c1, gA1, blk['xin'], N, [hw], [blk['in_hw']], side=SIDE,
-                                 emit=not (grp and blk['b'] > 0), slots=tsl)
+                                 emit=not (grp and blk['b'] > 0) and not tail_batch, slots=tsl)
                 if li == 1 and blk['b'] == 0:
                     self._pp['wg_c1'] = d1
                 if blk['b'] > 0:
@@ -806,7 +809,7 @@
                     g_pre = g_prev
                 else:
                     ds = cv[p + '.downsample.0']
-                    dwd = self._wgrad(ol, ds, g_pre, blk['xin'], N, [hw], [blk['in_hw']], side=SIDE, slots=tsl)
+                    dwd = self._wgrad(ol, ds, g_pre, blk['xin'], N, [hw], [blk['in_hw']], side=SIDE, emit=not tail_batch, slots=tsl)
                     if li == 1:
                         self._pp['wg_ds'] = dwd
                     if li > 1:
@@ -820,8 +823,18 @@
             if li == PREFIX_LI:
                 ol.record(L.SLOT_TAIL, stream=0)
             if GROUP and (li > 1 or GROUP_LAST):
-                on_main = '2' if li == 1 else '0'
+                on_main = tune('tail_main') if li == 1 else '0'
                 order = sorted(((3, g3), (2, g2), (1, g1)), key=lambda t: str(t[0]) in on_main)
+                if li == 1 and TAIL_BATCH:
+                    subs = [[self._pp['wg_c1']], [self._pp['wg_ds']]] + [g for gi, g in order if str(gi) not in on_main and g]
+                    batch = ops.WgradBatch(subs, workspace=lambda need: self._wg_buf(need, 'wg_ws'))
+                    ol.wgrad_multi(batch, side=SIDE)
+                    self._pp['wg_c1'], self._pp['wg_ds'] = batch.descs[0], batch.descs[1]
+                    order = [(gi, g) for gi, g in order if str(gi) in on_main and g]
+                    if len(order) > 1:
+                        ol.wgrad_multi(ops.WgradBatch([g for gi, g in order], workspace=lambda need: self._wg_buf(need, 'wg_ws_main')),
+                                       side=False)
+                        order = []
                 for gi, grp_descs in order:
                     mine = str(gi) in on_main
                     self._wgrad_group(ol, grp_descs, side=SIDE and not mine, ws_name='wg_ws_main' if mine else 'wg_ws')
diff --git a/dsl_amd/ops.py b/dsl_amd/ops.py
--- a/dsl_amd/ops.py
+++ b/dsl_amd/ops.py
@@ -201,6 +201,42 @@
         L.check(lib.dsl_conv2d_wgrad_multi(C.c_void_p(self.host.data_ptr()), L.ptr(self.dev), stream or L.stream_ptr()), 'dsl_conv2d_wgrad_multi')
 
 
+class WgradBatch(WgradMulti):
+
+    def __init__(self, subs, workspace=None, device='cuda'):
+        assert 1 <= len(subs) <= L.MAX_MULTI and all(1 <= len(g) <= L.MAX_GROUP for g in subs)
+        flat = [d for g in subs for d in g]
+        self.descs = (L.WgradDesc * len(flat))()
+        i = 0
+        for g in subs:
+            for d in g:
+                C.memmove(C.addressof(self.descs[i]), C.addressof(d), C.sizeof(L.WgradDesc))
+                if len(g) > 1:
+                    self.descs[i].splits = 0
+                i += 1
+        self.counts = (C.c_int * len(subs))(*[len(g) for g in subs])
+        self.nsub = len(subs)
+        need = lib.dsl_wgrad_batch_workspace_bytes(self.descs, self.counts, self.nsub)
+        if need == 0:
+            L.check(-1, 'dsl_wgrad_batch_workspace_bytes')
+        self.workspace_bytes = need
+        if callable(workspace):
+            workspace = workspace(need)
+        if workspace is None:
+            workspace = torch.empty(need, dtype=torch.uint8, device=device)
+        assert workspace.numel() * workspace.element_size() >= need
+        nb = lib.dsl_wgrad_batch_table_bytes()
+        self.host = torch.zeros(nb, dtype=torch.uint8)
+        L.check(lib.dsl_wgrad_batch_build(self.descs, self.counts, self.nsub, L.ptr(workspace), workspace.numel() * workspace.element_size(),
+                                          C.c_void_p(self.host.data_ptr()), nb), 'dsl_wgrad_batch_build')
+        self.dev = self.host
+        self._keep = (flat, workspace)
+
+    def run(self, stream=None):
+        p = C.c_void_p(self.host.data_ptr())
+        L.check(lib.dsl_conv2d_wgrad_multi(p, p, stream or L.stream_ptr()), 'dsl_conv2d_wgrad_multi')
+
+
 def conv2d_wgrad_group(descs, workspace=None):
     arr = wgrad_group(descs, workspace)
     L.check(lib.dsl_conv2d_wgrad_group(arr, len(descs), L.stream_ptr()), 'dsl_conv2d_wgrad_group')
diff --git a/dsl_amd/tuning.py b/dsl_amd/tuning.py
--- a/dsl_amd/tuning.py
+++ b/dsl_amd/tuning.py
@@ -8,12 +8,15 @@
     'img_split_bwd': '23',
     'tower_slots': '72',
     'tail_slots': '192',
+    'tail_batch': '0',
+    'tail_main': '2',
     'rla_split': '123',
     'rla_tail': '1',
     'rla_split_bwd': '',
     'check_backward_grad': '0',
     'skip': '',
     'lib.wgrad_slots': '128',
+    'lib.wgrad_pipe128': '1',
     'lib.stream_probe': '1',
     'lib.comm_queue': '1',
     'lib.rla_tail_form': '0',
diff --git a/include/dsl_hip.h b/include/dsl_hip.h
--- a/include/dsl_hip.h
+++ b/include/dsl_hip.h
@@ -101,6 +101,10 @@
                           void* table_host, size_t table_bytes);
 int dsl_conv2d_wgrad_multi(const void* table_host, const void* table_dev, void* stream);
 int dsl_wgrad_multi_info(const void* table_host, double* flops, double* bytes, int* blocks, int* red_blocks, int* nsub);
+size_t dsl_wgrad_batch_table_bytes(void);
+size_t dsl_wgrad_batch_workspace_bytes(const dsl_wgrad_desc* descs, const int* counts, int nsub);
+int dsl_wgrad_batch_build(const dsl_wgrad_desc* descs, const int* counts, int nsub, void* workspace, size_t workspace_bytes,
+                          void* table_host, size_t table_bytes);
 int dsl_wgrad_plan_probe(const int* stages, const int* tiles, const long long* tile_elems, int nsub, int cfg, int cap,
                          int* splits_out, int* info);
 
```

Result: no change. 451.6 imgs/s, median of 6 (+0.6%).
